# sinamalakouti/CDDMSL

Measured on AMD Instinct MI355X. Metric: images/sec (train step) VOC+Clipart RN50-C4, higher is better.
Workload: dtype bf16

## Files before the change

cddmsl_amd/csrc/conv_fwd256.hip:

```cpp
#include "gemm_common.h"
#include <type_traits>

namespace {

__device__ __forceinline__ unsigned pack4_e4m3(float a, float b, float c, float d) {
  a = __builtin_amdgcn_fmed3f(a, -448.f, 448.f); b = __builtin_amdgcn_fmed3f(b, -448.f, 448.f);
  c = __builtin_amdgcn_fmed3f(c, -448.f, 448.f); d = __builtin_amdgcn_fmed3f(d, -448.f, 448.f);
  int w = __builtin_amdgcn_cvt_pk_fp8_f32(a, b, 0, false);
  w = __builtin_amdgcn_cvt_pk_fp8_f32(c, d, w, true);
  return (unsigned)w;
}

struct fp8e4 { unsigned char v; };
template <> struct Mma<fp8e4> {
  static constexpr int ES = 2;
  __device__ static __forceinline__ void step2(f32x16& acc, const u32x4& a0, const u32x4& a1, const u32x4& b0, const u32x4& b1) {
    const i32x8 a = {(int)a0[0], (int)a0[1], (int)a0[2], (int)a0[3], (int)a1[0], (int)a1[1], (int)a1[2], (int)a1[3]};
    const i32x8 b = {(int)b0[0], (int)b0[1], (int)b0[2], (int)b0[3], (int)b1[0], (int)b1[1], (int)b1[2], (int)b1[3]};
    acc = __builtin_amdgcn_mfma_scale_f32_32x32x64_f8f6f4(a, b, acc, 0, 0, 0, 0x7f7f7f7f, 0, 0x7f7f7f7f);
  }
};
template <typename T> struct MmaQuad {
  __device__ static __forceinline__ void run(f32x16& c0, f32x16& c1, const u32x4 (*fa)[4], const u32x4* fb) {
#pragma unroll
    for (int ks = 0; ks < 4; ++ks) {
      Mma<T>::step(c0, fa[0][ks], fb[ks]);
      Mma<T>::step(c1, fa[1][ks], fb[ks]);
    }
  }
};
template <> struct MmaQuad<fp8e4> {
  __device__ static __forceinline__ void run(f32x16& c0, f32x16& c1, const u32x4 (*fa)[4], const u32x4* fb) {
#pragma unroll
    for (int s = 0; s < 2; ++s) {
      Mma<fp8e4>::step2(c0, fa[0][2 * s], fa[0][2 * s + 1], fb[2 * s], fb[2 * s + 1]);
      Mma<fp8e4>::step2(c1, fa[1][2 * s], fa[1][2 * s + 1], fb[2 * s], fb[2 * s + 1]);
    }
  }
};

__device__ __forceinline__ void blds16(__amdgpu_buffer_rsrc_t r, unsigned voff, unsigned soff, void* l) {
  __builtin_amdgcn_raw_ptr_buffer_load_lds(r, (__attribute__((address_space(3))) void*)l, 16, (int)voff, (int)soff, 0, 0);
}

template <typename T, bool RPOOL, int EPI, bool PRE = false>
__device__ __forceinline__ void tile_epilogue(const ConvArgs& p, f32x16 (&acc)[4][2], float* ep, int wr, int wc, int lane, int m0, int n0,
                                              const u32x4 (*pre)[4] = nullptr, const f32x4* sb = nullptr) {
  constexpr int ES = Mma<T>::ES;
  const int r32 = lane & 31, hh = lane >> 5;
  const int cg = lane & 7, rr = lane >> 3;
  const int n = n0 + wc * 64 + cg * 8;
  float sc[8], bi[8];
#pragma unroll
  for (int j = 0; j < 8; ++j) {
    if (sb) { sc[j] = sb[j >> 2][j & 3]; bi[j] = sb[2 + (j >> 2)][j & 3]; }
    else { sc[j] = p.scale ? p.scale[n + j] : 1.f; bi[j] = p.bias ? p.bias[n + j] : 0.f; }
  }
  const bool has_res = EPI < 0 ? p.residual != nullptr : (EPI & 1) != 0;
  const bool has_msk = EPI < 0 ? p.relu_mask != nullptr : (EPI & 2) != 0;
  const bool f32out = EPI < 0 && (ES == 4 || p.out_f32 != 0);
  const int eso = f32out ? 4 : 2;
  const float relu_floor = p.relu ? 0.f : -__builtin_inff();
  const long rows = p.M - m0;
  auto mk = [&](const char* base, long ld, int es) {
    long bytes = rows * ld * es;
    if (bytes > 0x7fffffffL) bytes = 0x7fffffffL;
    return __builtin_amdgcn_make_buffer_rsrc((void*)(base + (long)m0 * ld * es), 0, base ? (int)bytes : 0, 0x00020000);
  };
  const bool rf32 = EPI < 0 && ES == 2 && p.res_f32;
  const int esr = rf32 ? 4 : ES;
  const __amdgpu_buffer_rsrc_t ry = mk(p.y, p.ldy, eso), rmsk = mk(p.relu_mask, p.ldm, ES);
  const __amdgpu_buffer_rsrc_t rres = RPOOL ? __builtin_amdgcn_make_buffer_rsrc((void*)p.residual, 0, 0x7fffffff, 0x00020000)
                                            : mk(p.residual, p.ldr, esr);
  auto pooled_off = [&](int m) -> unsigned {
    const unsigned tq = fdiv((unsigned)m, p.dWo), ox = m - tq * p.Wo;
    const unsigned img = fdiv(tq, p.dHo), oy = tq - img * p.Ho;
    const unsigned hp = p.Ho >> 1, wp = p.Wo >> 1;
    const bool in = m < p.M && (oy >> 1) < hp && (ox >> 1) < wp;
    return in ? (unsigned)((((img * hp + (oy >> 1)) * wp + (ox >> 1)) * (unsigned)p.ldr + (unsigned)n) * ES) : 0x80000000u;
  };
  const unsigned vy = (unsigned)(((wr * 128 + rr) * p.ldy + n) * eso);
  const unsigned vr = (unsigned)(((wr * 128 + rr) * p.ldr + n) * esr), vm = (unsigned)(((wr * 128 + rr) * p.ldm + n) * ES);
  const bool emit8 = EPI < 0 && ES == 2 && p.y8 != nullptr;
  const __amdgpu_buffer_rsrc_t ry8 = mk(p.y8, p.ldy, 1);
  const unsigned vy8 = (unsigned)((wr * 128 + rr) * p.ldy + n);
  const float q8s = emit8 && p.q8 ? p.q8[0] : 1.f;
  unsigned am8 = 0u;
  constexpr int DEPTH = ES == 2 ? 2 : 1;
  char* wbase[8];
#pragma unroll
  for (int c = 0; c < 8; ++c)
    wbase[c] = (char*)ep + (hh * 4 * 64 + ((((r32 >> 3) ^ (hh << 2)) ^ c) << 3) + (r32 & 7)) * 4;
  u32x4 rresb[DEPTH][4][ES / 2], rmskb[DEPTH][4][ES / 2];
  auto fetch = [&](int a, u32x4 (*rres_)[ES / 2], u32x4 (*rmsk_)[ES / 2]) {
#pragma unroll
    for (int i = 0; i < 4; ++i)
#pragma unroll
      for (int q = 0; q < ES / 2; ++q) {
        if (RPOOL) rres_[i][q] = __builtin_amdgcn_raw_buffer_load_b128(rres, pooled_off(m0 + wr * 128 + a * 32 + rr + 8 * i), q * 16, 0);
        else if (has_res && !rf32) rres_[i][q] = __builtin_amdgcn_raw_buffer_load_b128(rres, vr, (a * 32 + 8 * i) * p.ldr * ES + q * 16, CDDMSL_LOAD_AUX);
        if (has_msk) rmsk_[i][q] = __builtin_amdgcn_raw_buffer_load_b128(rmsk, vm, (a * 32 + 8 * i) * p.ldm * ES + q * 16, CDDMSL_LOAD_AUX);
      }
  };
  if (PRE && DEPTH == 2) {
#pragma unroll
    for (int d = 0; d < 2; ++d)
#pragma unroll
      for (int i = 0; i < 4; ++i) {
        if (EPI & 1) {
          rresb[d % DEPTH][i][0] = pre[d][i];
          if (EPI & 2) rmskb[d % DEPTH][i][0] = __builtin_amdgcn_raw_buffer_load_b128(rmsk, vm, (d * 32 + 8 * i) * p.ldm * ES, CDDMSL_LOAD_AUX);
        } else rmskb[d % DEPTH][i][0] = pre[d][i];
      }
  } else if (DEPTH == 2 && !rf32) { fetch(0, rresb[0], rmskb[0]); fetch(1, rresb[DEPTH - 1], rmskb[DEPTH - 1]); }
  auto put = [&](auto A) {
    constexpr int a = decltype(A)::value;
#pragma unroll
    for (int b = 0; b < 2; ++b)
#pragma unroll
      for (int g = 0; g < 16; ++g)
        *(float*)(wbase[(b << 2) ^ (g & 3)] + ((g & 3) + 8 * (g >> 2)) * 256 + (a & 1) * 8192) = acc[a][b][g];
  };
  auto pass = [&](auto A) {
    constexpr int a = decltype(A)::value;
    if (DEPTH == 1) fetch(a, rresb[0], rmskb[0]);
    if (rf32) {
#pragma unroll
      for (int f = 0; f < 8; ++f)
        rresb[(f >> 2) % DEPTH][f & 3][0] = __builtin_amdgcn_raw_buffer_load_b128(rres, vr, (a * 32 + 8 * (f >> 1)) * p.ldr * 4 + (f & 1) * 16, 0);
    }
    u32x4 (*rres_)[ES / 2] = rresb[a % DEPTH];
    u32x4 (*rmsk_)[ES / 2] = rmskb[a % DEPTH];
    asm volatile("s_waitcnt lgkmcnt(0)" ::: "memory");
    f32x4 val[4][2];
#pragma unroll
    for (int i = 0; i < 4; ++i) {
      const int row = rr + 8 * i;
      const f32x4* src = (const f32x4*)(ep + (a & 1) * 2048 + row * 64 + ((cg ^ (row & 7)) << 3));
      val[i][0] = src[0]; val[i][1] = src[1];
    }
    asm volatile("" ::: "memory");
    if constexpr (a + 1 < 4) put(std::integral_constant<int, a + 1>{});
    asm volatile("" ::: "memory");
#pragma unroll
    for (int i = 0; i < 4; ++i) {
      const f32x4 v0 = val[i][0], v1 = val[i][1];
      float v[8] = {v0[0], v0[1], v0[2], v0[3], v1[0], v1[1], v1[2], v1[3]};
#pragma unroll
      for (int j = 0; j < 8; ++j) v[j] = affine<T>(v[j], sc[j], bi[j]);
      if (rf32) {
#pragma unroll
        for (int j = 0; j < 4; ++j) {
          v[j] += __builtin_bit_cast(f32x4, rresb[((2 * i) >> 2) % DEPTH][(2 * i) & 3][0])[j];
          v[4 + j] += __builtin_bit_cast(f32x4, rresb[((2 * i + 1) >> 2) % DEPTH][(2 * i + 1) & 3][0])[j];
        }
      } else if (RPOOL) {
        if (ES == 2) {
#pragma unroll
          for (int j = 0; j < 4; ++j) { v[2 * j] += 0.25f * bf2f(rres_[i][0][j] & 0xffff); v[2 * j + 1] += 0.25f * bf2f(rres_[i][0][j] >> 16); }
        } else {
#pragma unroll
          for (int j = 0; j < 4; ++j) {
            v[j] += 0.25f * __builtin_bit_cast(f32x4, rres_[i][0])[j]; v[4 + j] += 0.25f * __builtin_bit_cast(f32x4, rres_[i][ES / 2 - 1])[j];
          }
        }
      } else if (has_res) {
        if (ES == 2) {
#pragma unroll
          for (int j = 0; j < 4; ++j) { v[2 * j] += bf2f(rres_[i][0][j] & 0xffff); v[2 * j + 1] += bf2f(rres_[i][0][j] >> 16); }
        } else {
#pragma unroll
          for (int j = 0; j < 4; ++j) {
            v[j] += __builtin_bit_cast(f32x4, rres_[i][0])[j]; v[4 + j] += __builtin_bit_cast(f32x4, rres_[i][ES / 2 - 1])[j];
          }
        }
      }
#pragma unroll
      for (int j = 0; j < 8; ++j) asm("v_max_f32 %0, %1, %2" : "=v"(v[j]) : "v"(v[j]), "s"(relu_floor));
      if (has_msk) {
        float mv[8];
        if (ES == 2) {
#pragma unroll
          for (int j = 0; j < 4; ++j) { mv[2 * j] = bf2f(rmsk_[i][0][j] & 0xffff); mv[2 * j + 1] = bf2f(rmsk_[i][0][j] >> 16); }
        } else {
#pragma unroll
          for (int j = 0; j < 4; ++j) {
            mv[j] = __builtin_bit_cast(f32x4, rmsk_[i][0])[j]; mv[4 + j] = __builtin_bit_cast(f32x4, rmsk_[i][ES / 2 - 1])[j];
          }
        }
#pragma unroll
        for (int j = 0; j < 8; ++j) if (!(mv[j] > 0.f)) v[j] = 0.f;
      }
      const unsigned so = (unsigned)((a * 32 + 8 * i) * p.ldy * eso);
      if (emit8) {
#pragma unroll
        for (int j = 0; j < 8; ++j) am8 = absmax_bits(am8, v[j]);
        const u32x2 o8 = {pack4_e4m3(v[0] * q8s, v[1] * q8s, v[2] * q8s, v[3] * q8s), pack4_e4m3(v[4] * q8s, v[5] * q8s, v[6] * q8s, v[7] * q8s)};
        __builtin_amdgcn_raw_buffer_store_b64(o8, ry8, vy8, (unsigned)((a * 32 + 8 * i) * p.ldy), CDDMSL_STORE_AUX);
        asm volatile("s_nop 4" ::: "memory");
        asm volatile("" :: "v"(o8));
      }
      if (f32out) {
        const u32x4 o0 = {__builtin_bit_cast(unsigned, v[0]), __builtin_bit_cast(unsigned, v[1]), __builtin_bit_cast(unsigned, v[2]), __builtin_bit_cast(unsigned, v[3])};
        const u32x4 o1 = {__builtin_bit_cast(unsigned, v[4]), __builtin_bit_cast(unsigned, v[5]), __builtin_bit_cast(unsigned, v[6]), __builtin_bit_cast(unsigned, v[7])};
        __builtin_amdgcn_raw_buffer_store_b128(o0, ry, vy, so, CDDMSL_STORE_AUX);
        __builtin_amdgcn_raw_buffer_store_b128(o1, ry, vy, so + 16, CDDMSL_STORE_AUX);
        asm volatile("s_nop 4" ::: "memory");
        asm volatile("" :: "v"(o0), "v"(o1));
      } else {
        const u32x4 o = {pack2bf(v[0], v[1]), pack2bf(v[2], v[3]), pack2bf(v[4], v[5]), pack2bf(v[6], v[7])};
        if (p.nt_out) __builtin_amdgcn_raw_buffer_store_b128(o, ry, vy, so, CDDMSL_STORE_AUX);
        else __builtin_amdgcn_raw_buffer_store_b128(o, ry, vy, so, 0);
        asm volatile("s_nop 4" ::: "memory");
        asm volatile("" :: "v"(o));
      }
    }
    if (DEPTH == 2 && a + 2 < 4 && !rf32) fetch(a + 2, rresb[a % DEPTH], rmskb[a % DEPTH]);
  };
  put(std::integral_constant<int, 0>{});
  pass(std::integral_constant<int, 0>{});
  pass(std::integral_constant<int, 1>{});
  pass(std::integral_constant<int, 2>{});
  pass(std::integral_constant<int, 3>{});
  if (emit8 && p.amax8) {
    am8 = wave_max_u(am8);
    if (lane == 0) atomicMax(p.amax8 + (blockIdx.x & 63), am8);
  }
}

template <typename T, bool TAPS, bool RPOOL = false, int EPI = -1, bool PERSIST = false, bool SPLITK = false>
__global__ __launch_bounds__(512) void k_conv_fwd256(ConvArgs p) {
  __shared__ __attribute__((aligned(16))) u32x4 lds[2 * 2 * 2 * 128 * KCH];
  const int t_in = threadIdx.x;
  p.x += (long)blockIdx.y * p.bx; p.w += (long)blockIdx.y * p.bw; p.y += (long)blockIdx.y * p.by;
  const int ntn = p.Cout >> 8;
  const int ntiles = PERSIST ? (p.tile_limit ? p.tile_limit : ntn * ((p.M + 255) >> 8)) : 0;
  int lbid = PERSIST ? (int)((blockIdx.x & 7) * (gridDim.x >> 3) + (blockIdx.x >> 3))
           : SPLITK ? p.tile0 + (int)(blockIdx.x / (unsigned)p.ksplits) : xcd_remap(blockIdx.x, gridDim.x);
  const int kt0 = SPLITK ? (int)(blockIdx.x % (unsigned)p.ksplits) * p.kper : 0;
  if (PERSIST && lbid >= ntiles) return;
  for (;;) {
  int t = t_in;
  if (PERSIST) asm volatile("" : "+v"(t));
  const int lane = t & 63;
#ifdef CDDMSL_TILE_STAMPS
  const unsigned long long ts_entry = __builtin_amdgcn_s_memrealtime();
#endif
  const int wvu = __builtin_amdgcn_readfirstlane(t >> 6);
  const int wr = wvu >> 2, wc = wvu & 3;
  const int tile_n = lbid % ntn, tile_m = lbid / ntn;
  const int m0 = tile_m * 256, n0 = tile_n * 256;
  const int cl = (t & 7) ^ ((t >> 4) & 7);
  const int nkt = SPLITK ? min(p.kper, (p.Kc >> 3) - kt0) : (p.Kc >> 3);
  const int tpt = p.cpp >> 3;

  auto rowoff = [&](int m, int& iy0, int& ix0) {
    const unsigned tq = fdiv((unsigned)m, p.dWo), ox = m - tq * p.Wo;
    const unsigned img = fdiv(tq, p.dHo), oy = tq - img * p.Ho;
    iy0 = (int)oy * p.stride - p.pad; ix0 = (int)ox * p.stride - p.pad;
    return (((long)img * p.Hi + iy0) * p.Wi + ix0) * p.xrs * 16;
  };
  int iyb, ixb;
  const long base_a = rowoff(m0, iyb, ixb);
  const __amdgpu_buffer_rsrc_t ra_rsrc = __builtin_amdgcn_make_buffer_rsrc((void*)(p.x + base_a), 0, 0x7fffffff, 0x00020000);
  const __amdgpu_buffer_rsrc_t rb_rsrc = __builtin_amdgcn_make_buffer_rsrc((void*)(p.w + (long)n0 * p.wrs * 16), 0, 0x7fffffff, 0x00020000);
  unsigned va[2][2], vinv[2][2], vb[2][2];
  int iy0[2][2], ix0[2][2];
#pragma unroll
  for (int h = 0; h < 2; ++h)
#pragma unroll
    for (int i = 0; i < 2; ++i) {
      const int m = m0 + i * 128 + h * 64 + (t >> 3);
      const bool vm = m < p.M;
      const long ro = rowoff(vm ? m : m0, iy0[h][i], ix0[h][i]);
      va[h][i] = (unsigned)(ro - base_a) + cl * 16;
      if (!vm) { iy0[h][i] = -(1 << 20); if (!TAPS) va[h][i] |= 0x80000000u; }
      vinv[h][i] = 0;
      vb[h][i] = (unsigned)(((2 * i + (t >> 8)) * 64 + h * 32 + ((t >> 3) & 31)) * p.wrs + cl) * 16;
    }
  if (TAPS) {
    unsigned xm[2][2] = {{0, 0}, {0, 0}};
    for (int kx = 0; kx < p.KW; ++kx)
#pragma unroll
      for (int h = 0; h < 2; ++h)
#pragma unroll
        for (int i = 0; i < 2; ++i) xm[h][i] |= ((unsigned)(ix0[h][i] + kx) >= (unsigned)p.Wi ? 1u : 0u) << kx;
    const unsigned full = (1u << p.KW) - 1u;
    for (int ky = 0; ky < p.KH; ++ky)
#pragma unroll
      for (int h = 0; h < 2; ++h)
#pragma unroll
        for (int i = 0; i < 2; ++i) vinv[h][i] |= ((unsigned)(iy0[h][i] + ky) >= (unsigned)p.Hi ? full : xm[h][i]) << (ky * p.KW);
  }
  const int step_col = (p.xrs - (p.cpp - KCH)) * 16;
  const int step_row = ((p.Wi - (p.KW - 1)) * p.xrs - (p.cpp - KCH)) * 16;
  int left[2] = {tpt, tpt}, tap[2] = {0, 0}, kxs[2] = {0, 0};
  unsigned soa[2] = {0, 0}, sob[2] = {0, 0};
  if (SPLITK) {
    const int tap0 = TAPS ? kt0 / tpt : 0, within = TAPS ? kt0 - tap0 * tpt : kt0;
    const int ky0 = TAPS ? tap0 / p.KW : 0, kx0 = tap0 - ky0 * p.KW;
#pragma unroll
    for (int h = 0; h < 2; ++h) {
      left[h] = tpt - (TAPS ? within : 0); tap[h] = tap0; kxs[h] = kx0;
      soa[h] = (unsigned)((ky0 * p.Wi + kx0) * p.xrs * 16 + within * KCH * 16);
      sob[h] = (unsigned)(kt0 * KCH * 16);
    }
  }

  char* const L = (char*)lds;
  auto stageA = [&](auto H, int buf) {
    constexpr int h = decltype(H)::value;
    char* dst = L + (buf << 16) + (h << 14) + wvu * 1024;
#pragma unroll
    for (int i = 0; i < 2; ++i) {
      unsigned v = va[h][i];
      if (TAPS) v |= __builtin_amdgcn_ubfe(vinv[h][i], (unsigned)tap[h], 1u) << 31;
      blds16(ra_rsrc, v, soa[h], dst + i * 8192);
    }
    if (TAPS) {
      int step = KCH * 16;
      if (--left[h] == 0) {
        left[h] = tpt; ++tap[h];
        if (++kxs[h] == p.KW) { kxs[h] = 0; step = step_row; } else step = step_col;
      }
      soa[h] += step;
    } else soa[h] += KCH * 16;
  };
  auto stageB = [&](auto J, int buf) {
    constexpr int j = decltype(J)::value;
    char* dst = L + (buf << 16) + (1 << 15) + (j << 14) + wvu * 1024;
#pragma unroll
    for (int i = 0; i < 2; ++i) blds16(rb_rsrc, vb[j][i], sob[j], dst + i * 8192);
    sob[j] += KCH * 16;
  };
  using I0 = std::integral_constant<int, 0>;
  using I1 = std::integral_constant<int, 1>;

  f32x16 acc[4][2];
#pragma unroll
  for (int a = 0; a < 4; ++a)
#pragma unroll
    for (int b = 0; b < 2; ++b)
#pragma unroll
      for (int r = 0; r < 16; ++r) acc[a][b][r] = 0.f;

  const int r32 = lane & 31, hh = lane >> 5, sw = (r32 >> 1) & 7;
  unsigned ada[4], adb[4];
#pragma unroll
  for (int ks = 0; ks < 4; ++ks) {
    ada[ks] = (unsigned)(((wr * 64 + r32) * KCH + ((2 * ks + hh) ^ sw)) * 16);
    adb[ks] = (unsigned)(((wc * 32 + r32) * KCH + ((2 * ks + hh) ^ sw)) * 16 + (1 << 15));
  }
  u32x4 fa0[2][4], fa1[2][4], fb0[4], fb1[4];
  auto readA = [&](auto I, u32x4 (*fa)[4]) {
    constexpr int i = decltype(I)::value;
#pragma unroll
    for (int rt = 0; rt < 2; ++rt)
#pragma unroll
      for (int ks = 0; ks < 4; ++ks) fa[rt][ks] = *(const u32x4*)(L + ada[ks] + ((i << 14) + rt * 32 * KCH * 16));
  };
  auto readB = [&](auto J, u32x4* fb) {
    constexpr int j = decltype(J)::value;
#pragma unroll
    for (int ks = 0; ks < 4; ++ks) fb[ks] = *(const u32x4*)(L + adb[ks] + (j << 14));
  };
  auto flipA = [&]() {
#pragma unroll
    for (int ks = 0; ks < 4; ++ks) ada[ks] ^= 1u << 16;
  };
  auto flipB = [&]() {
#pragma unroll
    for (int ks = 0; ks < 4; ++ks) adb[ks] ^= 1u << 16;
  };
#define CDDMSL_MMA_QUAD(I, J, FA, FB) MmaQuad<T>::run(acc[2 * (I)][J], acc[2 * (I) + 1][J], FA, FB)
#define CDDMSL_PHASE_SYNC_IN()                                                      \
  __builtin_amdgcn_sched_barrier(0);                                                \
  __builtin_amdgcn_s_barrier();                                                     \
  asm volatile("s_waitcnt lgkmcnt(0)" ::: "memory");                                \
  __builtin_amdgcn_sched_barrier(0);                                                \
  __builtin_amdgcn_s_setprio(1);
#define CDDMSL_PHASE_SYNC_OUT(I, J)                                                 \
  asm volatile("" : "+v"(acc[2 * (I)][J]), "+v"(acc[2 * (I) + 1][J]));    \
  __builtin_amdgcn_s_setprio(0);                                                    \
  __builtin_amdgcn_sched_barrier(0);                                                \
  __builtin_amdgcn_s_barrier();                                                     \
  __builtin_amdgcn_sched_barrier(0);

  stageA(I0{}, 0); stageA(I1{}, 0); stageB(I0{}, 0); stageB(I1{}, 0);
  if (nkt > 1) {
    stageA(I0{}, 1); stageB(I0{}, 1); stageB(I1{}, 1);
    asm volatile("s_waitcnt vmcnt(6)" ::: "memory");
  } else {
    asm volatile("s_waitcnt vmcnt(0)" ::: "memory");
  }
  __builtin_amdgcn_s_barrier();
  readA(I0{}, fa0);
  if (wr == 1) __builtin_amdgcn_s_barrier();
  __builtin_amdgcn_sched_barrier(0);
#ifdef CDDMSL_TILE_STAMPS
  const unsigned long long ts_loop = __builtin_amdgcn_s_memrealtime();
#endif

  constexpr bool PREF = EPI > 0 && !RPOOL && Mma<T>::ES == 2 && !SPLITK;
  u32x4 pre[2][4];
  f32x4 sb[4];
  auto ktile = [&](int kt, auto LAST) {
    constexpr bool last = decltype(LAST)::value;
    const int d = kt & 1;
    const bool more1 = !last, more2 = !last && kt + 2 < nkt;
    readB(I0{}, fb0);
    if (more1) stageA(I1{}, d ^ 1);
    CDDMSL_PHASE_SYNC_IN();
    CDDMSL_MMA_QUAD(0, 0, fa0, fb0);
    CDDMSL_PHASE_SYNC_OUT(0, 0);
    readB(I1{}, fb1);
    flipB();
    if (more2) stageA(I0{}, d);
    CDDMSL_PHASE_SYNC_IN();
    CDDMSL_MMA_QUAD(0, 1, fa0, fb1);
    CDDMSL_PHASE_SYNC_OUT(0, 1);
    readA(I1{}, fa1);
    flipA();
    if (more2) {
      stageB(I0{}, d);
      asm volatile("s_waitcnt vmcnt(4)" ::: "memory");
    } else if (more1) {
      asm volatile("s_waitcnt vmcnt(0)" ::: "memory");
    } else if (PREF) {
      const bool is_res = (EPI & 1) != 0;
      const char* base = is_res ? p.residual : p.relu_mask;
      const int ld = is_res ? p.ldr : p.ldm;
      long bytes = ((long)p.M - m0) * ld * 2;
      if (bytes > 0x7fffffffL) bytes = 0x7fffffffL;
      const __amdgpu_buffer_rsrc_t rs = __builtin_amdgcn_make_buffer_rsrc((void*)(base + (long)m0 * ld * 2), 0, (int)bytes, 0x00020000);
      const unsigned vo = (unsigned)(((wr * 128 + (lane >> 3)) * ld + n0 + wc * 64 + (lane & 7) * 8) * 2);
#pragma unroll
      for (int a = 0; a < 2; ++a)
#pragma unroll
        for (int i = 0; i < 4; ++i) pre[a][i] = __builtin_amdgcn_raw_buffer_load_b128(rs, vo, (a * 32 + 8 * i) * ld * 2, 0);
    }
    CDDMSL_PHASE_SYNC_IN();
    CDDMSL_MMA_QUAD(1, 1, fa1, fb1);
    CDDMSL_PHASE_SYNC_OUT(1, 1);
    if (more1) readA(I0{}, fa0);
    if (more2) stageB(I1{}, d);
    if (last && !SPLITK) {
      const int n = n0 + wc * 64 + (lane & 7) * 8;
      const f32x4 one = {1.f, 1.f, 1.f, 1.f}, zero = {0.f, 0.f, 0.f, 0.f};
      sb[0] = p.scale ? *(const f32x4*)(p.scale + n) : one; sb[1] = p.scale ? *(const f32x4*)(p.scale + n + 4) : one;
      sb[2] = p.bias ? *(const f32x4*)(p.bias + n) : zero; sb[3] = p.bias ? *(const f32x4*)(p.bias + n + 4) : zero;
    }
    CDDMSL_PHASE_SYNC_IN();
    CDDMSL_MMA_QUAD(1, 0, fa1, fb0);
    CDDMSL_PHASE_SYNC_OUT(1, 0);
  };
  for (int kt = 0; kt + 1 < nkt; ++kt) ktile(kt, std::false_type{});
  ktile(nkt - 1, std::true_type{});
  if (wr == 0) __builtin_amdgcn_s_barrier();
#ifdef CDDMSL_TILE_STAMPS
  const unsigned long long ts_epi = __builtin_amdgcn_s_memrealtime();
#endif
#undef CDDMSL_MMA_QUAD
#undef CDDMSL_PHASE_SYNC_IN
#undef CDDMSL_PHASE_SYNC_OUT

  if (SPLITK) {
    store_frags((f32x4*)p.partial + (long)blockIdx.x * (8 * 32 * 64) + (wvu * 32) * 64 + lane, acc);
    return;
  }
  tile_epilogue<T, RPOOL, EPI, PREF>(p, acc, (float*)lds + wvu * 4096, wr, wc, lane, m0, n0, pre, sb);
#ifdef CDDMSL_TILE_STAMPS
  if (p.tstamps && lane == 0) {
    if (!PERSIST) asm volatile("s_waitcnt vmcnt(0)" ::: "memory");
    unsigned long long* o = p.tstamps + ((long)(PERSIST ? lbid : (int)blockIdx.x) * 8 + wvu) * 4;
    o[0] = ts_entry; o[1] = ts_loop; o[2] = ts_epi; o[3] = __builtin_amdgcn_s_memrealtime();
  }
#endif
  if (!PERSIST) break;
  lbid += gridDim.x;
  if (lbid >= ntiles) break;
  __builtin_amdgcn_s_barrier();
  }
}

template <typename T, bool TAPS, int EPI>
__global__ __launch_bounds__(256, 2) void k_conv_fwd2(ConvArgs p) {
  constexpr int SA = 256 * 64, SB = 128 * 64, SS = SA + SB, STAGES = 3;
  __shared__ __attribute__((aligned(16))) u32x4 lds[STAGES * SS / 16];
  const int t = threadIdx.x, lane = t & 63;
#ifdef CDDMSL_TILE_STAMPS
  const unsigned long long ts_entry = __builtin_amdgcn_s_memrealtime();
#endif
  p.x += (long)blockIdx.y * p.bx; p.w += (long)blockIdx.y * p.bw; p.y += (long)blockIdx.y * p.by;
  const int wvu = __builtin_amdgcn_readfirstlane(t >> 6);
  const int wr = wvu >> 1, wc = wvu & 1;
  const int ntn = p.Cout >> 7;
  const int lbid = xcd_remap(blockIdx.x, gridDim.x);
  const int tile_n = lbid % ntn, tile_m = lbid / ntn;
  const int m0 = tile_m * 256, n0 = tile_n * 128;
  const int cl = (t & 3) ^ ((t >> 3) & 3);
  const int nkt = p.Kc >> 2;
  const int tpt = p.cpp >> 2;

  auto rowoff = [&](int m, int& iy0, int& ix0) {
    const unsigned tq = fdiv((unsigned)m, p.dWo), ox = m - tq * p.Wo;
    const unsigned img = fdiv(tq, p.dHo), oy = tq - img * p.Ho;
    iy0 = (int)oy * p.stride - p.pad; ix0 = (int)ox * p.stride - p.pad;
    return (((long)img * p.Hi + iy0) * p.Wi + ix0) * p.xrs * 16;
  };
  int iyb, ixb;
  const long base_a = rowoff(m0, iyb, ixb);
  const __amdgpu_buffer_rsrc_t ra_rsrc = __builtin_amdgcn_make_buffer_rsrc((void*)(p.x + base_a), 0, 0x7fffffff, 0x00020000);
  const __amdgpu_buffer_rsrc_t rb_rsrc = __builtin_amdgcn_make_buffer_rsrc((void*)(p.w + (long)n0 * p.wrs * 16), 0, 0x7fffffff, 0x00020000);
  unsigned va[4], vinv[4], vb[2];
  int iy0[4], ix0[4];
#pragma unroll
  for (int i = 0; i < 4; ++i) {
    const int m = m0 + (t >> 2) + 64 * i;
    const bool vm = m < p.M;
    const long ro = rowoff(vm ? m : m0, iy0[i], ix0[i]);
    va[i] = (unsigned)(ro - base_a) + cl * 16;
    if (!vm) { iy0[i] = -(1 << 20); if (!TAPS) va[i] |= 0x80000000u; }
    vinv[i] = 0;
  }
#pragma unroll
  for (int i = 0; i < 2; ++i) vb[i] = (unsigned)((((t >> 2) + 64 * i) * p.wrs + cl) * 16);
  if (TAPS) {
    unsigned xm[4] = {0, 0, 0, 0};
    for (int kx = 0; kx < p.KW; ++kx)
#pragma unroll
      for (int i = 0; i < 4; ++i) xm[i] |= ((unsigned)(ix0[i] + kx) >= (unsigned)p.Wi ? 1u : 0u) << kx;
    const unsigned full = (1u << p.KW) - 1u;
    for (int ky = 0; ky < p.KH; ++ky)
#pragma unroll
      for (int i = 0; i < 4; ++i) vinv[i] |= ((unsigned)(iy0[i] + ky) >= (unsigned)p.Hi ? full : xm[i]) << (ky * p.KW);
  }
  const int step_col = (p.xrs - (p.cpp - 4)) * 16;
  const int step_row = ((p.Wi - (p.KW - 1)) * p.xrs - (p.cpp - 4)) * 16;
  int left = tpt, tap = 0, kxs = 0;
  unsigned soa = 0, sob = 0;

  char* const L = (char*)lds;
  auto stage = [&](int st) {
    char* dst = L + st * SS + wvu * 1024;
#pragma unroll
    for (int i = 0; i < 4; ++i) {
      unsigned v = va[i];
      if (TAPS) v |= __builtin_amdgcn_ubfe(vinv[i], (unsigned)tap, 1u) << 31;
      blds16(ra_rsrc, v, soa, dst + i * 4096);
    }
#pragma unroll
    for (int i = 0; i < 2; ++i) blds16(rb_rsrc, vb[i], sob, dst + SA + i * 4096);
    sob += 64;
    if (TAPS) {
      int step = 64;
      if (--left == 0) {
        left = tpt; ++tap;
        if (++kxs == p.KW) { kxs = 0; step = step_row; } else step = step_col;
      }
      soa += step;
    } else soa += 64;
  };

  f32x16 acc[4][2];
#pragma unroll
  for (int a = 0; a < 4; ++a)
#pragma unroll
    for (int b = 0; b < 2; ++b)
#pragma unroll
      for (int r = 0; r < 16; ++r) acc[a][b][r] = 0.f;

  const int r32 = lane & 31, hh = lane >> 5, sw = (r32 >> 1) & 3;
  unsigned ada[2], adb[2];
#pragma unroll
  for (int ks = 0; ks < 2; ++ks) {
    ada[ks] = (unsigned)(((wr * 128 + r32) * 4 + ((2 * ks + hh) ^ sw)) * 16);
    adb[ks] = (unsigned)(SA + ((wc * 64 + r32) * 4 + ((2 * ks + hh) ^ sw)) * 16);
  }
  u32x4 fa[2][4][2], fb[2][2][2];
  auto readf = [&](auto SET, int st) {
    constexpr int set = decltype(SET)::value;
    const char* base = L + st * SS;
#pragma unroll
    for (int rt = 0; rt < 4; ++rt)
#pragma unroll
      for (int ks = 0; ks < 2; ++ks) fa[set][rt][ks] = *(const u32x4*)(base + ada[ks] + rt * 32 * 64);
#pragma unroll
    for (int ct = 0; ct < 2; ++ct)
#pragma unroll
      for (int ks = 0; ks < 2; ++ks) fb[set][ct][ks] = *(const u32x4*)(base + adb[ks] + ct * 32 * 64);
  };
  using S0 = std::integral_constant<int, 0>;
  using S1 = std::integral_constant<int, 1>;

  stage(0);
  if (nkt > 1) stage(1);
  if (nkt > 2) stage(2);
  if (nkt > 2) asm volatile("s_waitcnt vmcnt(12)" ::: "memory");
  else if (nkt > 1) asm volatile("s_waitcnt vmcnt(6)" ::: "memory");
  else asm volatile("s_waitcnt vmcnt(0)" ::: "memory");
  __builtin_amdgcn_s_barrier();
  readf(S0{}, 0);
#ifdef CDDMSL_TILE_STAMPS
  const unsigned long long ts_loop = __builtin_amdgcn_s_memrealtime();
#endif
  int st_next = 1, st_free = 0;

  auto ktile = [&](int kt, auto SET) {
    constexpr int set = decltype(SET)::value;
    if (kt + 2 < nkt) asm volatile("s_waitcnt vmcnt(6)" ::: "memory");
    else asm volatile("s_waitcnt vmcnt(0)" ::: "memory");
    __builtin_amdgcn_s_waitcnt(0xc07f);
    __builtin_amdgcn_sched_barrier(0);
    __builtin_amdgcn_s_barrier();
    __builtin_amdgcn_sched_barrier(0);
    if (kt + 1 < nkt) readf(std::integral_constant<int, set ^ 1>{}, st_next);
    if (kt + 3 < nkt) stage(st_free);
    st_next = st_next == STAGES - 1 ? 0 : st_next + 1;
    st_free = st_free == STAGES - 1 ? 0 : st_free + 1;
    __builtin_amdgcn_sched_barrier(0);
    __builtin_amdgcn_s_setprio(1);
#pragma unroll
    for (int ks = 0; ks < 2; ++ks)
#pragma unroll
      for (int rt = 0; rt < 4; ++rt)
#pragma unroll
        for (int ct = 0; ct < 2; ++ct) Mma<T>::step(acc[rt][ct], fa[set][rt][ks], fb[set][ct][ks]);
    __builtin_amdgcn_s_setprio(0);
    __builtin_amdgcn_sched_barrier(0);
  };
  for (int kt = 0; kt < nkt; kt += 2) {
    ktile(kt, S0{});
    if (kt + 1 < nkt) ktile(kt + 1, S1{});
  }
#ifdef CDDMSL_TILE_STAMPS
  asm volatile("" : "+v"(acc[3][1]));
  const unsigned long long ts_epi = __builtin_amdgcn_s_memrealtime();
#endif
  tile_epilogue<T, false, EPI>(p, acc, (float*)lds + wvu * 4096, wr, wc, lane, m0, n0);
#ifdef CDDMSL_TILE_STAMPS
  if (p.tstamps && lane == 0) {
    asm volatile("s_waitcnt vmcnt(0)" ::: "memory");
    unsigned long long* o = p.tstamps + ((long)blockIdx.x * 4 + wvu) * 4;
    o[0] = ts_entry; o[1] = ts_loop; o[2] = ts_epi; o[3] = __builtin_amdgcn_s_memrealtime();
  }
#endif
}

__global__ __launch_bounds__(256) void k_conv_split_reduce(ConvArgs p) {
  const int tile_rel = blockIdx.x >> 6, q = (blockIdx.x & 63) * 256 + threadIdx.x;
  const f32x4* src = (const f32x4*)p.partial + (long)tile_rel * p.ksplits * 16384 + q;
  f32x4 sum = src[0];
  for (int s = 1; s < p.ksplits; ++s) sum += src[(long)s * 16384];
  const int wvu = q >> 11, j = (q >> 6) & 31, lane = q & 63, r32 = lane & 31, hh = lane >> 5;
  const int a = j >> 3, b = (j >> 2) & 1, g4 = j & 3, wr = wvu >> 2, wc = wvu & 3;
  const int ntn = p.Cout >> 8, lbid = p.tile0 + tile_rel;
  const int tile_n = lbid % ntn, tile_m = lbid / ntn;
  const int n = tile_n * 256 + wc * 64 + b * 32 + r32;
  const int mrow = tile_m * 256 + wr * 128 + a * 32 + 8 * g4 + 4 * hh;
  const float sc = p.scale ? p.scale[n] : 1.f, bi = p.bias ? p.bias[n] : 0.f;
#pragma unroll
  for (int e = 0; e < 4; ++e) {
    const long m = mrow + e;
    if (m >= p.M) break;
    float v = __builtin_fmaf(sum[e], sc, bi);
    if (p.residual) v += bf2f(*(const unsigned short*)(p.residual + (m * p.ldr + n) * 2));
    if (p.relu) v = fmaxf(v, 0.f);
    if (p.relu_mask && !(bf2f(*(const unsigned short*)(p.relu_mask + (m * p.ldm + n) * 2)) > 0.f)) v = 0.f;
    *(unsigned short*)(p.y + (m * p.ldy + n) * 2) = f2bf(v);
  }
}

static int persistent_blocks() { return env_int("CDDMSL_PERSIST", 1) ? persistent_blocks_raw() : 0; }

static int epi_of(const ConvArgs& a) { return (a.out_f32 || a.res_f32 || a.y8) ? -1 : (a.residual ? 1 : 0) | (a.relu_mask ? 2 : 0); }
template <typename F> void with_epi(int epi, F&& launch) {
  switch (epi) {
    case 0: launch(std::integral_constant<int, 0>()); break;
    case 1: launch(std::integral_constant<int, 1>()); break;
    case 2: launch(std::integral_constant<int, 2>()); break;
    default: launch(std::integral_constant<int, 3>()); break;
  }
}

template <typename T, bool TAPS> void launch_fwd2(const ConvArgs& a, dim3 grid, hipStream_t st) {
  const int epi = epi_of(a);
  if constexpr (sizeof(T) == 2) {
    if (epi >= 0) {
      with_epi(epi, [&](auto e) { hipLaunchKernelGGL((k_conv_fwd2<T, TAPS, decltype(e)::value>), grid, dim3(256), 0, st, a); });
      return;
    }
  }
  hipLaunchKernelGGL((k_conv_fwd2<T, TAPS, -1>), grid, dim3(256), 0, st, a);
}

struct TailSplit { int rem, splits, kper; };
constexpr int TAIL_FRAC_DEFAULT = 8;
static TailSplit plan_tail_split(int tiles, int ncu, int nktot, long ws_bytes) {
  const int rem = ncu > 0 ? tiles % ncu : 0;
  long frac = env_int("CDDMSL_TAIL_FRAC", TAIL_FRAC_DEFAULT);
  if (frac <= 0) frac = 8;
  if (env_int("CDDMSL_TAIL_SPLIT", 1) == 0 || tiles <= ncu || rem <= 0 || rem * frac > ncu || nktot < 16) return {};
  long S = ncu / rem;
  if (S > nktot / 2) S = nktot / 2;
  const long maxs = env_int("CDDMSL_TAIL_MAXS", S);
  if (S > maxs) S = maxs;
  const int kper = (int)((nktot + S - 1) / S);
  S = (nktot + kper - 1) / kper;
  if (S < 2 || rem * S * 65536 * 4 > ws_bytes) return {};
  return {rem, (int)S, kper};
}

template <typename T, bool TAPS> void launch256_main(const ConvArgs& a, dim3 grid, hipStream_t st, int epi) {
  if constexpr (std::is_same<T, __bf16>::value && !TAPS) {
    const int nb = persistent_blocks();
    if (nb > 0 && grid.y == 1 && (int)grid.x > nb && (a.Kc >> 3) <= env_int("CDDMSL_PERSIST_MAXKT", 8)) {
      with_epi(epi, [&](auto e) { hipLaunchKernelGGL((k_conv_fwd256<T, false, false, decltype(e)::value, true>), dim3(nb), dim3(512), 0, st, a); });
      return;
    }
  }
  with_epi(epi, [&](auto e) { hipLaunchKernelGGL((k_conv_fwd256<T, TAPS, false, decltype(e)::value>), grid, dim3(512), 0, st, a); });
}

template <typename T, bool TAPS> void launch256(const ConvArgs& a, dim3 grid, hipStream_t st, void* ws, long ws_bytes) {
  const int epi = epi_of(a);
  if (sizeof(T) == 4 || epi < 0) { hipLaunchKernelGGL((k_conv_fwd256<T, TAPS, false, -1>), grid, dim3(512), 0, st, a); return; }
  if constexpr (sizeof(T) != 4) {
    if constexpr (std::is_same<T, __bf16>::value) {
      const int tiles = (int)grid.x;
      const TailSplit ts = grid.y == 1 ? plan_tail_split(tiles, persistent_blocks_raw(), a.Kc >> 3, ws ? ws_bytes : 0) : TailSplit{};
      if (ts.splits) {
        ConvArgs m = a, t = a;
        m.tile_limit = tiles - ts.rem;
        launch256_main<T, TAPS>(m, dim3((unsigned)(tiles - ts.rem), 1), st, epi);
        t.partial = (float*)ws; t.tile0 = tiles - ts.rem; t.ksplits = ts.splits; t.kper = ts.kper;
        hipLaunchKernelGGL((k_conv_fwd256<T, TAPS, false, -1, false, true>), dim3((unsigned)(ts.rem * ts.splits)), dim3(512), 0, st, t);
        hipLaunchKernelGGL(k_conv_split_reduce, dim3((unsigned)(ts.rem * 64)), dim3(256), 0, st, t);
        return;
      }
    }
    launch256_main<T, TAPS>(a, grid, st, epi);
  }
}

template <typename T> void launch_tile256(const ConvArgs& a, const Plan& p, hipStream_t st, void* ws, long ws_bytes) {
  const dim3 grid(p.gx, p.gy);
  const bool taps = !(a.KH == 1 && a.KW == 1 && a.pad == 0);
  if constexpr (std::is_same<T, fp8e4>::value) {
    if (taps) launch256<T, true>(a, grid, st, ws, ws_bytes);
    else launch256<T, false>(a, grid, st, ws, ws_bytes);
  } else if (p.kernel == 11) {
    if (taps) launch_fwd2<T, true>(a, grid, st);
    else launch_fwd2<T, false>(a, grid, st);
  } else {
    if (a.res_pool) hipLaunchKernelGGL((k_conv_fwd256<T, false, true>), grid, dim3(512), 0, st, a);
    else if (taps) launch256<T, true>(a, grid, st, ws, ws_bytes);
    else launch256<T, false>(a, grid, st, ws, ws_bytes);
  }
}

}

void launch_fwd_tile256(const ConvArgs& a, const Plan& p, Operand op, hipStream_t st, void* ws, long ws_bytes) {
  if (op == OP_BF16) launch_tile256<__bf16>(a, p, st, ws, ws_bytes);
  else if (op == OP_F32) launch_tile256<float>(a, p, st, ws, ws_bytes);
  else launch_tile256<fp8e4>(a, p, st, ws, ws_bytes);
}
```

cddmsl_amd/csrc/gemm_common.h:

```cpp
#pragma once
#include "common.h"
#include <cstdlib>

namespace {

constexpr int BM = 128, BN = 128, KCH = 8;

struct FastDiv {
  unsigned mul, shr, d;
};
static inline FastDiv make_fastdiv(unsigned d) {
  FastDiv f;
  f.d = d;
  unsigned s = 0;
  while ((1ull << s) < d) ++s;
  f.shr = s;
  f.mul = (unsigned)(((1ull << 32) * ((1ull << s) - d)) / d + 1);
  return f;
}
__device__ __forceinline__ unsigned fdiv(unsigned n, const FastDiv& f) { return (__umulhi(n, f.mul) + n) >> f.shr; }

template <typename T> __device__ __forceinline__ float affine(float v, float sc, float bi) {
  return sizeof(T) <= 2 ? __builtin_fmaf(v, sc, bi) : v * sc + bi;
}

#ifndef CDDMSL_STORE_AUX
#define CDDMSL_STORE_AUX 2
#endif
#ifndef CDDMSL_LOAD_AUX
#define CDDMSL_LOAD_AUX 0
#endif

struct ConvArgs {
  const char* x;
  const char* w;
  char* y;
  const float* scale;
  const float* bias;
  const char* residual;
  const char* relu_mask;
  int Nimg, Hi, Wi, Cin, Ho, Wo, Cout, KH, KW, stride, pad;
  int ldy, ldr, ldm;
  int relu, out_f32, pool;
  int res_f32;
  int res_pool;
  int M, Kc, cpp;
  FastDiv dWo, dHo, dcpp, dKW;
  int xrs, wrs;
  long bx, bw, by;
  char* y8 = nullptr;
  const float* q8 = nullptr;
  unsigned* amax8 = nullptr;
  float* partial = nullptr;
  int tile0 = 0, ksplits = 1, kper = 0, tile_limit = 0;
  int pool_out = 0;
  FastDiv dWp = {}, dHp = {};
  int nt_out = 1;
#ifdef CDDMSL_TILE_STAMPS
  unsigned long long* tstamps = nullptr;
#endif
};

template <typename T> struct Mma;
template <> struct Mma<__bf16> {
  static constexpr int ES = 2;
  __device__ static __forceinline__ void step(f32x16& acc, const u32x4& a, const u32x4& b) {
    acc = __builtin_amdgcn_mfma_f32_32x32x16_bf16(__builtin_bit_cast(bf16x8, a), __builtin_bit_cast(bf16x8, b), acc, 0, 0, 0);
  }
  __device__ static __forceinline__ float load(const char* p) { return bf2f(*(const unsigned short*)p); }
  __device__ static __forceinline__ void store(char* p, float v) { *(unsigned short*)p = f2bf(v); }
};
template <> struct Mma<float> {
  static constexpr int ES = 4;
  __device__ static __forceinline__ void step(f32x16& acc, const u32x4& a, const u32x4& b) {
    const f32x4 fa = __builtin_bit_cast(f32x4, a), fb = __builtin_bit_cast(f32x4, b);
    acc = __builtin_amdgcn_mfma_f32_32x32x2f32(fa[0], fb[0], acc, 0, 0, 0);
    acc = __builtin_amdgcn_mfma_f32_32x32x2f32(fa[1], fb[1], acc, 0, 0, 0);
    acc = __builtin_amdgcn_mfma_f32_32x32x2f32(fa[2], fb[2], acc, 0, 0, 0);
    acc = __builtin_amdgcn_mfma_f32_32x32x2f32(fa[3], fb[3], acc, 0, 0, 0);
  }
  __device__ static __forceinline__ float load(const char* p) { return *(const float*)p; }
  __device__ static __forceinline__ void store(char* p, float v) { *(float*)p = v; }
};
typedef __attribute__((ext_vector_type(8))) int i32x8;

__device__ __forceinline__ int xcd_remap(int bid, int nblk) {
  const int q = nblk >> 3, rem = nblk & 7, x = bid & 7, j = bid >> 3;
  return (x < rem ? x * (q + 1) : rem * (q + 1) + (x - rem) * q) + j;
}

template <typename T> __device__ __forceinline__ u32x4 avg4(const u32x4& a, const u32x4& b, const u32x4& c, const u32x4& d);
template <> __device__ __forceinline__ u32x4 avg4<float>(const u32x4& a, const u32x4& b, const u32x4& c, const u32x4& d) {
  const f32x4 fa = __builtin_bit_cast(f32x4, a), fb = __builtin_bit_cast(f32x4, b);
  const f32x4 fc = __builtin_bit_cast(f32x4, c), fd = __builtin_bit_cast(f32x4, d);
  f32x4 r = ((fa + fb) + (fc + fd)) * 0.25f;
  return __builtin_bit_cast(u32x4, r);
}
template <> __device__ __forceinline__ u32x4 avg4<__bf16>(const u32x4& a, const u32x4& b, const u32x4& c, const u32x4& d) {
  u32x4 r;
#pragma unroll
  for (int j = 0; j < 4; ++j) {
    float lo = (bf2f(a[j] & 0xffff) + bf2f(b[j] & 0xffff)) + (bf2f(c[j] & 0xffff) + bf2f(d[j] & 0xffff));
    float hi = (bf2f(a[j] >> 16) + bf2f(b[j] >> 16)) + (bf2f(c[j] >> 16) + bf2f(d[j] >> 16));
    r[j] = pack2bf(lo * 0.25f, hi * 0.25f);
  }
  return r;
}

__device__ __attribute__((aligned(16))) unsigned int g_zero_page[4] = {0u, 0u, 0u, 0u};

__device__ __forceinline__ void glds16(const void* g, void* l) {
  __builtin_amdgcn_global_load_lds((const __attribute__((address_space(1))) void*)g,
                                   (__attribute__((address_space(3))) void*)l, 16, 0, 0);
}

struct WgradArgs {
  const char* x;
  const char* dy;
  float* dw;
  const float* scale;
  int Nimg, Hi, Wi, Cin, Ho, Wo, Cout, KH, KW, stride, pad, ldd, pool;
  int M, Kc, cpp, K, ncc;
  int mtiles_per_split;
  FastDiv dWo, dHo;
  int xrs;
  int ldo;
  int direct;
  long bx, bd, bo;
  const float* g0 = nullptr;
  const unsigned long long* mbits = nullptr;
  float* gpos = nullptr;
  float* ws = nullptr;
#ifdef CDDMSL_TILE_STAMPS
  unsigned long long* tstamps = nullptr;
#endif
};

constexpr int WM = 64;
constexpr int WROW = 16 + 4;

__device__ __forceinline__ int fsw(int row) { return ((row & 3) << 2) | ((row >> 2) & 3); }

__device__ __forceinline__ void store_frags(f32x4* dst, const f32x16 (&acc)[4][2]) {
#pragma unroll
  for (int a = 0; a < 4; ++a)
#pragma unroll
    for (int b = 0; b < 2; ++b)
#pragma unroll
      for (int g4 = 0; g4 < 4; ++g4) {
        const f32x4 v = {acc[a][b][4 * g4], acc[a][b][4 * g4 + 1], acc[a][b][4 * g4 + 2], acc[a][b][4 * g4 + 3]};
        dst[((a * 2 + b) * 4 + g4) * 64] = v;
      }
}

static long env_int(const char* name, long dflt, bool* set = nullptr) {
  const char* e = getenv(name);
  if (set) *set = e != nullptr;
  return e ? atol(e) : dflt;
}

enum Operand { OP_BF16 = 0, OP_F32 = 1, OP_FP8 = 2 };
static int elem_size(Operand op) { return op == OP_BF16 ? 2 : op == OP_F32 ? 4 : 1; }

struct Plan {
  int kernel;
  unsigned gx, gy;
  int splits;
  int mtiles_per_split;
  int bpb;
};

static int persistent_blocks_raw() {
  static int ncu = -1;
  if (ncu < 0) {
    int dev = 0, n = 0;
    if (hipGetDevice(&dev) != hipSuccess || hipDeviceGetAttribute(&n, hipDeviceAttributeMultiprocessorCount, dev) != hipSuccess) n = 0;
    ncu = (n / 8) * 8;
  }
  return ncu;
}

}

extern "C" {
__attribute__((visibility("hidden"))) void launch_fwd_tile128(const ConvArgs& a, const Plan& p, Operand op, hipStream_t st);
__attribute__((visibility("hidden"))) void launch_fwd_tile256(const ConvArgs& a, const Plan& p, Operand op, hipStream_t st, void* ws, long ws_bytes);
__attribute__((visibility("hidden"))) void launch_wgrad(WgradArgs& a, const Plan& p, Operand op, hipStream_t st, void* ws, long ws_bytes);
__attribute__((visibility("hidden"))) void launch_gemm_tn(const WgradArgs& p, Operand op, const Plan& pl, int batch, int mode, hipStream_t st);
__attribute__((visibility("hidden"))) void launch_attnpool_dx(const WgradArgs& p, unsigned gx, unsigned gy, int nbatch, int bpb, hipStream_t st);
__attribute__((visibility("hidden"))) bool record_kernel(int id);
}
```

cddmsl_amd/csrc/gemm_conv.hip:

```cpp
#include "gemm_common.h"

namespace {

template <typename T>
__device__ __forceinline__ void weight_prep_body(const float* w, const float* scale, char* wf, char* wd, int Cout, int KH, int KW, int Cin,
                                                 long first, long stride) {
  __shared__ float tile[32][33];
  const int taps = KH * KW, nit = (Cin + 31) / 32, nct = (Cout + 31) / 32;
  const long ntiles = (long)nct * taps * nit;
  const int tx = threadIdx.x & 31, ty = threadIdx.x >> 5;
  constexpr int ES = Mma<T>::ES;
  for (long tl = first; tl < ntiles; tl += stride) {
    const int it = (int)(tl % nit); const long q = tl / nit;
    const int tap = (int)(q % taps), ct = (int)(q / taps);
    const int ky = tap / KW, kx = tap % KW;
    __syncthreads();
#pragma unroll
    for (int r = 0; r < 4; ++r) {
      const int co = ct * 32 + ty + 8 * r, ci = it * 32 + tx;
      float v = 0.f;
      if (co < Cout && ci < Cin) {
        const long i = ((long)co * taps + tap) * Cin + ci;
        v = w[i];
        if (wf) Mma<T>::store(wf + i * ES, v);
        if (scale) v *= scale[co];
      }
      tile[ty + 8 * r][tx] = v;
    }
    __syncthreads();
    if (wd) {
#pragma unroll
      for (int r = 0; r < 4; ++r) {
        const int ci = it * 32 + ty + 8 * r, co = ct * 32 + tx;
        if (ci < Cin && co < Cout) {
          const long j = (((long)ci * KH + (KH - 1 - ky)) * KW + (KW - 1 - kx)) * Cout + co;
          Mma<T>::store(wd + j * ES, tile[tx][ty + 8 * r]);
        }
      }
    }
  }
}
template <typename T>
__global__ __launch_bounds__(256) void k_weight_prep(const float* w, const float* scale, char* wf, char* wd, int Cout, int KH, int KW, int Cin) {
  weight_prep_body<T>(w, scale, wf, wd, Cout, KH, KW, Cin, (long)blockIdx.x, (long)gridDim.x);
}
template <typename T>
__global__ __launch_bounds__(256) void k_weight_prep_multi(const long long* table) {
  const long long* e = table + 8 * (long)blockIdx.y;
  weight_prep_body<T>((const float*)e[0], (const float*)e[1], (char*)e[2], (char*)e[3], (int)e[4], (int)e[5], (int)e[6], (int)e[7],
                      (long)blockIdx.x, (long)gridDim.x);
}

static thread_local int g_last_kernel = 0;
static thread_local int g_plan_only = 0;


static bool gemm256_legal(const ConvArgs& a) {
  const bool vec_ok = (a.ldy % 8 == 0) && (!a.residual || a.ldr % 8 == 0) && (!a.relu_mask || a.ldm % 8 == 0);
  if (a.pool || (a.cpp & 7) || (a.Cout & 255) || !vec_ok || a.KH * a.KW > 31) return false;
  if (2 * a.pad > a.KH - 1 || 2 * a.pad > a.KW - 1) return false;
  return true;
}

static bool use_gemm256(const ConvArgs& a, int batch) {
  const long mode = env_int("CDDMSL_GEMM256", 1);
  if (mode == 0) return false;
  if (!gemm256_legal(a)) return false;
  if (mode == 2) return true;
  const long tiles = (long)((a.M + 255) / 256) * (a.Cout / 256) * batch;
  return tiles >= 160;
}

static bool fwd2_legal(const ConvArgs& a) {
  const bool vec_ok = (a.ldy % 8 == 0) && (!a.residual || a.ldr % 8 == 0) && (!a.relu_mask || a.ldm % 8 == 0);
  if (a.pool || a.res_pool || (a.cpp & 3) || (a.Cout & 127) || !vec_ok || a.KH * a.KW > 31) return false;
  if (2 * a.pad > a.KH - 1 || 2 * a.pad > a.KW - 1) return false;
  return true;
}
static bool use_fwd2(const ConvArgs& a, int batch) {
  const long mode = env_int("CDDMSL_FWD2", 1);
  if (mode == 0 || !fwd2_legal(a)) return false;
  if (mode == 2) return true;
  if (use_gemm256(a, batch) || batch != 1) return false;
  return (long)(a.Cout / 128) * ((a.M + 255) / 256) >= env_int("CDDMSL_FWD2_MIN", 256);
}

static Plan plan_fwd(const ConvArgs& a, Operand op, int batch) {
  const long tiles256 = (long)(a.Cout / 256) * ((a.M + 255) / 256);
  if (op == OP_FP8) {
    if (!gemm256_legal(a) || tiles256 > 0x7fffffffL) return {};
    return {10, (unsigned)tiles256, 1};
  }
  if (a.y8 && !use_gemm256(a, batch)) return {};
  const long tiles128 = (long)((a.Cout + BN - 1) / BN) * ((a.M + BM - 1) / BM);
  if (tiles128 > 0x7fffffffL) return {};
  const bool packed = batch == 1 && a.xrs == a.cpp && a.wrs == a.Kc;
  if (!a.pool && a.KH == 3 && a.KW == 3 && a.pad == 1 && (a.cpp == 1 || a.cpp == 4 || (a.cpp == 8 && a.Cout == 64)) &&
      (a.Cout == 32 || a.Cout == 64) && !a.residual && !a.out_f32 && packed) {
    return {8, a.cpp > 1 ? 256u * 2 : 256u * 8, 1};
  }
  if (op == OP_BF16 && !a.pool && a.KH == 1 && a.KW == 1 && a.pad == 0 && a.stride == 1 && a.Cout == 64 && (a.cpp == 8 || a.cpp == 32) &&
      !a.residual && !a.out_f32 && !a.y8 && packed && a.ldy == 64 && env_int("CDDMSL_SMALL_1X1", 1) != 0) return {8, 512, 1};
  if (use_fwd2(a, batch)) return {11, (unsigned)((long)(a.Cout / 128) * ((a.M + 255) / 256)), (unsigned)batch};
  if (use_gemm256(a, batch)) return {3, (unsigned)tiles256, (unsigned)batch};
  if (a.pool) return {2, (unsigned)tiles128, 1};
  return {1, (unsigned)tiles128, (unsigned)batch};
}

static void* g_ws = nullptr;
static long g_ws_bytes = 0;

static int run_fwd(const ConvArgs& a, Operand op, const Plan& p, void* stream) {
  if (p.kernel == 0) return CDDMSL_ERR_ARG;
  g_last_kernel = p.kernel;
  if (g_plan_only) return CDDMSL_OK;
  if (p.kernel == 3 || p.kernel == 10 || p.kernel == 11) launch_fwd_tile256(a, p, op, (hipStream_t)stream, g_ws, g_ws_bytes);
  else launch_fwd_tile128(a, p, op, (hipStream_t)stream);
  return launch_status();
}

}

#ifdef CDDMSL_TILE_STAMPS
static unsigned long long* g_tile_stamps = nullptr;
extern "C" void cddmsl_debug_tile_stamps(unsigned long long* p) { g_tile_stamps = p; }
#endif
extern "C" int cddmsl_last_kernel(void) { return g_last_kernel; }
extern "C" int cddmsl_plan_only(int on) { const int was = g_plan_only; g_plan_only = on; return was; }
bool record_kernel(int id) { g_last_kernel = id; return g_plan_only != 0; }

static int nt_out_for(long out_bytes) {
  static const long nt_min_mb = env_int("CDDMSL_NT_MIN_MB", 128);
  return out_bytes > (nt_min_mb << 20) ? 1 : 0;
}

static int fill_conv(ConvArgs& a, Operand op, const void* x, const void* w, void* y, const float* scale, const float* bias,
                     const void* residual, const void* relu_mask, int Nimg, int Hi, int Wi, int Cin, int Cout, int KH, int KW,
                     int stride, int pad, int pool, int ldy, int ldr, int ldm, int relu, int out_f32, void* y8, const float* q8,
                     float* amax8) {
  const int es = elem_size(op);
  if (Nimg < 0 || Hi <= 0 || Wi <= 0 || Cin <= 0 || Cout <= 0 || KH <= 0 || KW <= 0 || stride <= 0) return CDDMSL_ERR_ARG;
  if ((Cin * es) % 16 != 0) return CDDMSL_ERR_ARG;
  if (pool && (KH != 1 || KW != 1 || pad != 0 || stride != 1)) return CDDMSL_ERR_ARG;
  a.x = (const char*)x; a.w = (const char*)w; a.y = (char*)y; a.scale = scale; a.bias = bias;
  a.residual = (const char*)residual; a.relu_mask = (const char*)relu_mask;
  a.Nimg = Nimg; a.Hi = Hi; a.Wi = Wi; a.Cin = Cin; a.Cout = Cout; a.KH = KH; a.KW = KW; a.stride = stride; a.pad = pad;
  if (pool) { a.Ho = Hi / 2; a.Wo = Wi / 2; }
  else { a.Ho = (Hi + 2 * pad - KH) / stride + 1; a.Wo = (Wi + 2 * pad - KW) / stride + 1; }
  if (a.Ho <= 0 || a.Wo <= 0) return CDDMSL_ERR_ARG;
  if ((out_f32 & 2) && (!(out_f32 & 1) || !residual || relu_mask || pool)) return CDDMSL_ERR_ARG;
  a.ldy = ldy; a.ldr = ldr; a.ldm = ldm; a.relu = relu; a.out_f32 = out_f32 & 1; a.pool = pool;
  a.res_f32 = (op == OP_BF16 && (out_f32 & 2)) ? 1 : 0;
  a.res_pool = (out_f32 & 4) ? 1 : 0;
  if (a.res_pool && (!residual || (out_f32 & 2) || pool || KH != 1 || KW != 1 || pad != 0 || (long)Nimg * (a.Ho / 2) * (a.Wo / 2) * ldr * es >= (1L << 31) ||
                     (Cout & 7) || (ldy & 7) || (ldr & 7) || (relu_mask && (ldm & 7)))) return CDDMSL_ERR_ARG;
  if (a.res_f32 && ((Cout & 7) || (ldy & 7) || (ldr & 7))) return CDDMSL_ERR_ARG;
  long M = (long)Nimg * a.Ho * a.Wo;
  if (M > 0x7fffff00L) return CDDMSL_ERR_ARG;
  a.M = (int)M; a.cpp = Cin * es / 16; a.Kc = KH * KW * a.cpp;
  a.dWo = make_fastdiv((unsigned)a.Wo); a.dHo = make_fastdiv((unsigned)a.Ho);
  a.dcpp = make_fastdiv((unsigned)a.cpp); a.dKW = make_fastdiv((unsigned)KW);
  a.xrs = a.cpp; a.wrs = a.Kc; a.bx = a.bw = a.by = 0;
#ifdef CDDMSL_TILE_STAMPS
  a.tstamps = g_tile_stamps;
#endif
  if (a.M == 0) return CDDMSL_OK;
  a.nt_out = nt_out_for((long)a.M * Cout * 2);
  if (y8) {
    if (op == OP_F32 || (out_f32 & 1) || ldy != Cout) return CDDMSL_ERR_ARG;
    a.y8 = (char*)y8; a.q8 = q8; a.amax8 = (unsigned*)amax8;
  }
  return CDDMSL_OK;
}

static int conv_fwd_any(Operand op, const void* x, const void* w, void* y, const float* scale, const float* bias,
                        const void* residual, const void* relu_mask, int Nimg, int Hi, int Wi, int Cin,
                        int Cout, int KH, int KW, int stride, int pad, int pool, int ldy, int ldr, int ldm,
                        int relu, int out_f32, void* y8, const float* q8, float* amax8, void* stream) {
  ConvArgs a;
  const int st = fill_conv(a, op, x, w, y, scale, bias, residual, relu_mask, Nimg, Hi, Wi, Cin, Cout, KH, KW, stride, pad, pool, ldy, ldr, ldm,
                           relu, out_f32, y8, q8, amax8);
  if (st != CDDMSL_OK || a.M == 0) return st;
  return run_fwd(a, op, plan_fwd(a, op, 1), stream);
}

extern "C" int cddmsl_conv_fwd(const void* x, const void* w, void* y, const float* scale, const float* bias,
                               const void* residual, const void* relu_mask, int Nimg, int Hi, int Wi, int Cin,
                               int Cout, int KH, int KW, int stride, int pad, int pool, int ldy, int ldr, int ldm,
                               int relu, int out_f32, int dtype, void* stream) {
  if (dtype != 0 && dtype != 1) return CDDMSL_ERR_ARG;
  return conv_fwd_any((Operand)dtype, x, w, y, scale, bias, residual, relu_mask, Nimg, Hi, Wi, Cin, Cout, KH, KW, stride, pad, pool, ldy, ldr, ldm,
                      relu, out_f32, nullptr, nullptr, nullptr, stream);
}

extern "C" int cddmsl_conv3x3_pool_fwd(const void* x, const void* w, void* y, const float* scale, const float* bias, const void* relu_mask,
                                       int Nimg, int Hi, int Wi, int Cin, int Cout, int stride, int dtype, void* stream) {
  if (dtype != 0 || Cin != 32 || Cout != 64 || stride != 1 || relu_mask || !scale || !bias || Hi < 2 || Wi < 2) return CDDMSL_ERR_ARG;
  ConvArgs a;
  const int st = fill_conv(a, OP_BF16, x, w, y, scale, bias, nullptr, nullptr, Nimg, Hi, Wi, Cin, Cout, 3, 3, 1, 1, 0, Cout, 0, 0, 1, 0,
                           nullptr, nullptr, nullptr);
  if (st != CDDMSL_OK || a.M == 0) return st;
  if ((long)Nimg * Hi * Wi * Cin * 2 >= 0x7ffff000L || (long)Nimg * (a.Ho / 2) * (a.Wo / 2) * Cout * 2 >= 0x7fffffffL) return CDDMSL_ERR_ARG;
  a.pool_out = 1;
  a.dWp = make_fastdiv((unsigned)(a.Wo / 2)); a.dHp = make_fastdiv((unsigned)(a.Ho / 2));
  const Plan pl = plan_fwd(a, OP_BF16, 1);
  if (pl.kernel != 8) return CDDMSL_ERR_ARG;
  return run_fwd(a, OP_BF16, pl, stream);
}

extern "C" int cddmsl_conv_fwd_q8(const void* x, const void* w, void* y, const float* scale, const float* bias,
                                  const void* residual, const void* relu_mask, int Nimg, int Hi, int Wi, int Cin,
                                  int Cout, int KH, int KW, int stride, int pad, int relu, void* y8, const float* q8, float* amax8,
                                  void* stream) {
  if (!y8) return CDDMSL_ERR_ARG;
  return conv_fwd_any(OP_BF16, x, w, y, scale, bias, residual, relu_mask, Nimg, Hi, Wi, Cin, Cout, KH, KW, stride, pad, 0, Cout, Cout, Cout,
                      relu, 0, y8, q8, amax8, stream);
}

extern "C" int cddmsl_conv_fwd_fp8(const void* x, const void* w, void* y, const float* scale, const float* bias,
                                   const void* residual, const void* relu_mask, int Nimg, int Hi, int Wi, int Cin, int Cout, int KH,
                                   int KW, int pad, int relu, int out_f32, void* y8, const float* q8, float* amax8, void* stream) {
  if (Cin % 128 != 0 || (out_f32 & ~1)) return CDDMSL_ERR_ARG;
  return conv_fwd_any(OP_FP8, x, w, y, scale, bias, residual, relu_mask, Nimg, Hi, Wi, Cin, Cout, KH, KW, 1, pad, 0, Cout, Cout, Cout,
                      relu, out_f32, y8, q8, amax8, stream);
}

static bool wgrad256_ok(const WgradArgs& a, int batch) {
  const long mode = env_int("CDDMSL_GEMM256", 1);
  if (mode == 0) return false;
  if ((a.Cout & 255) || (a.K & 255) || (a.cpp & 7) || (a.ldd & 7)) return false;
  if (mode == 2) return true;
  return (long)(a.Cout / 256) * (a.K / 256) * batch * ((a.M + WM - 1) / WM) >= env_int("CDDMSL_WGRAD256_MIN", 4000);
}
static bool wgrad256_span_ok(int mtiles_per_split, int Wi, long row_bytes) {
  return ((long)mtiles_per_split * WM + WM + 2L * Wi + 2) * row_bytes + (1L << 20) < (1L << 31);
}

static int even_split(int total_mt, long* splits) {
  const int mps = (int)((total_mt + *splits - 1) / *splits);
  *splits = (total_mt + mps - 1) / mps;
  return mps;
}

static long split_512_rounds(long tiles, int total_mt, bool taps) {
  bool forced;
  const long target = env_int("CDDMSL_WGRAD_BLOCKS", taps ? 1024 : 512, &forced);
  const long maxs = (total_mt + 7) / 8;
  long splits = 1;
  const long r0 = (target + 511) / 512;
  double best = -1.0;
  for (long r = r0; r <= r0 + 1; ++r) {
    long c = (512 * r) / tiles;
    if (c < 1) c = 1;
    if (c > maxs) c = maxs;
    long real = c;
    even_split(total_mt, &real);
    const long blocks = tiles * real, rounds = (blocks + 511) / 512;
    const double eff = (double)blocks / (512.0 * rounds);
    if (eff > best + 0.03) { best = eff; splits = c; }
    if (c == maxs) break;
  }
  if (forced) { splits = (target + tiles - 1) / tiles; if (splits > maxs) splits = maxs; }
  return splits < 1 ? 1 : splits;
}

static long split_256_rounds(long tiles, int total_mt) {
  const long maxs = (total_mt + 15) / 16;
  long sp = 1;
  double best = -1.0;
  for (int r = 1; r <= 6; ++r) {
    long c = (256L * r) / tiles;
    if (c < 1) continue;
    if (c > maxs) c = maxs;
    const long blocks = tiles * c, rounds = (blocks + 255) / 256;
    const double eff = (double)blocks / (256.0 * rounds);
    if (eff > best + 0.02) { best = eff; sp = c; }
    if (c == maxs) break;
  }
  return sp;
}

static Plan plan_wgrad(const WgradArgs& a, Operand op, int batch) {
  const int es = elem_size(op), total_mt = (a.M + WM - 1) / WM;
  const long tiles256 = (long)(a.Cout / 256) * (a.K / 256);
  const long row_bytes = (long)a.ldd * es > a.xrs * 16L ? (long)a.ldd * es : a.xrs * 16L;
  if (op == OP_FP8) {
    long sp = split_256_rounds(tiles256, total_mt);
    const int mps = even_split(total_mt, &sp);
    if (!wgrad256_span_ok(mps, a.Wi, row_bytes)) return {};
    return {12, (unsigned)(tiles256 * sp), 1, (int)sp, mps};
  }
  const int cols = 256 / es;
  const long tiles = (long)((a.Cout + cols - 1) / cols) * ((a.K + cols - 1) / cols);
  long splits = split_512_rounds(tiles, total_mt, !(a.KH == 1 && a.KW == 1));
  const int mps = even_split(total_mt, &splits);
  if (tiles * splits > 0x7fffffffL) return {};
  const bool same = !a.pool && a.stride == 1 && a.Ho == a.Hi && a.Wo == a.Wi;
  if (same && op == OP_BF16 && wgrad256_ok(a, batch)) {
    bool forced;
    const long want = env_int("CDDMSL_WGRAD256_BLOCKS", 0, &forced);
    const long maxs = (total_mt + 15) / 16;
    long sp = forced ? (want + tiles256 - 1) / tiles256 : split_256_rounds(tiles256, total_mt);
    if (sp > maxs) sp = maxs;
    if (sp < 1) sp = 1;
    const int mps256 = even_split(total_mt, &sp);
    if (wgrad256_span_ok(mps256, a.Wi, row_bytes)) return {6, (unsigned)(tiles256 * sp), 1, (int)sp, mps256};
  }
  return {same ? 5 : 4, (unsigned)(tiles * splits), 1, (int)splits, mps};
}

extern "C" int cddmsl_set_workspace(void* ptr, long bytes) {
  if (bytes < 0 || (ptr == nullptr && bytes != 0) || ((size_t)ptr & 15)) return CDDMSL_ERR_ARG;
  g_ws = ptr; g_ws_bytes = bytes;
  return CDDMSL_OK;
}

static int run_wgrad(WgradArgs& a, Operand op, const Plan& p, void* stream) {
  if (p.kernel == 0) return CDDMSL_ERR_ARG;
  g_last_kernel = p.kernel;
  if (g_plan_only) return CDDMSL_OK;
  a.mtiles_per_split = p.mtiles_per_split;
  launch_wgrad(a, p, op, (hipStream_t)stream, g_ws, g_ws_bytes);
  return launch_status();
}

static int fill_wgrad(WgradArgs& a, Operand op, const void* x, const void* dy, float* dw, const float* scale, int Nimg, int Hi,
                      int Wi, int Cin, int Cout, int KH, int KW, int stride, int pad, int pool, int ldd) {
  const int es = elem_size(op);
  if (Nimg < 0 || Hi <= 0 || Wi <= 0 || Cin <= 0 || Cout <= 0 || KH <= 0 || KW <= 0 || stride <= 0) return CDDMSL_ERR_ARG;
  if ((Cin * es) % 16 != 0 || (Cout * es) % 16 != 0 || (ldd * es) % 16 != 0) return CDDMSL_ERR_ARG;
  if (pool && (KH != 1 || KW != 1 || pad != 0 || stride != 1)) return CDDMSL_ERR_ARG;
  a.x = (const char*)x; a.dy = (const char*)dy; a.dw = dw; a.scale = scale;
  a.Nimg = Nimg; a.Hi = Hi; a.Wi = Wi; a.Cin = Cin; a.Cout = Cout; a.KH = KH; a.KW = KW; a.stride = stride; a.pad = pad;
  a.ldd = ldd; a.pool = pool;
  if (pool) { a.Ho = Hi / 2; a.Wo = Wi / 2; }
  else { a.Ho = (Hi + 2 * pad - KH) / stride + 1; a.Wo = (Wi + 2 * pad - KW) / stride + 1; }
  if (a.Ho <= 0 || a.Wo <= 0) return CDDMSL_ERR_ARG;
  long M = (long)Nimg * a.Ho * a.Wo;
  if (M > 0x7fffff00L) return CDDMSL_ERR_ARG;
  a.M = (int)M; a.cpp = Cin * es / 16; a.Kc = KH * KW * a.cpp; a.K = KH * KW * Cin; a.ncc = Cout * es / 16;
  a.mtiles_per_split = 0;
  a.dWo = make_fastdiv((unsigned)a.Wo); a.dHo = make_fastdiv((unsigned)a.Ho);
  a.xrs = a.cpp; a.ldo = a.K; a.direct = 0; a.bx = a.bd = a.bo = 0;
#ifdef CDDMSL_TILE_STAMPS
  a.tstamps = g_tile_stamps;
#endif
  return CDDMSL_OK;
}

extern "C" int cddmsl_conv_wgrad(const void* x, const void* dy, float* dw, const float* scale, int Nimg, int Hi,
                                 int Wi, int Cin, int Cout, int KH, int KW, int stride, int pad, int pool, int ldd,
                                 int dtype, void* stream) {
  if (dtype != 0 && dtype != 1) return CDDMSL_ERR_ARG;
  WgradArgs a;
  const int st = fill_wgrad(a, (Operand)dtype, x, dy, dw, scale, Nimg, Hi, Wi, Cin, Cout, KH, KW, stride, pad, pool, ldd);
  if (st != CDDMSL_OK || a.M == 0) return st;
  return run_wgrad(a, (Operand)dtype, plan_wgrad(a, (Operand)dtype, 1), stream);
}

extern "C" int cddmsl_conv_wgrad_fp8_ok(int Cin, int Cout, int KH, int KW, int pad, int ldd) {
  return (Cin % 256 == 0 && Cout % 256 == 0 && KH == KW && (KH & 1) && 2 * pad == KH - 1 && ldd % 16 == 0) ? 1 : 0;
}
extern "C" int cddmsl_conv_wgrad_fp8(const void* x8, const void* dy8, float* dw, const float* scale, int Nimg, int Hi, int Wi, int Cin,
                                     int Cout, int KH, int KW, int pad, int ldd, void* stream) {
  if (!cddmsl_conv_wgrad_fp8_ok(Cin, Cout, KH, KW, pad, ldd) || ldd < Cout) return CDDMSL_ERR_ARG;
  WgradArgs a;
  const int st = fill_wgrad(a, OP_FP8, x8, dy8, dw, scale, Nimg, Hi, Wi, Cin, Cout, KH, KW, 1, pad, 0, ldd);
  if (st != CDDMSL_OK || a.M == 0) return st;
  return run_wgrad(a, OP_FP8, plan_wgrad(a, OP_FP8, 1), stream);
}

extern "C" int cddmsl_gemm_nt_batched(const void* a, const void* w, void* c, const float* bias, int M, int N, int K, int lda,
                                      int ldb, int ldc, int batch, long sa, long sw, long sc, int out_f32, int dtype, void* stream) {
  int es = dtype == 0 ? 2 : 4;
  if (dtype != 0 && dtype != 1) return CDDMSL_ERR_ARG;
  if (M < 0 || N <= 0 || K <= 0 || batch < 0 || batch > 65535) return CDDMSL_ERR_ARG;
  if ((K * es) % 16 || (lda * es) % 16 || (ldb * es) % 16 || (sa * es) % 16 || (sw * es) % 16) return CDDMSL_ERR_ARG;
  if (M == 0 || batch == 0) return CDDMSL_OK;
  const Operand op = (Operand)dtype;
  ConvArgs p;
  const int st = fill_conv(p, op, a, w, c, nullptr, bias, nullptr, nullptr, 1, 1, M, K, N, 1, 1, 1, 0, 0, ldc, 0, 0, 0, out_f32 ? 1 : 0,
                           nullptr, nullptr, nullptr);
  if (st != CDDMSL_OK) return st;
  p.xrs = lda * es / 16; p.wrs = ldb * es / 16;
  p.bx = sa * es; p.bw = sw * es; p.by = sc * (out_f32 ? 4 : es);
  p.nt_out = 1;
  return run_fwd(p, op, plan_fwd(p, op, batch), stream);
}

static unsigned tn_small_grid(long kt, long batch, int* bpb) {
  long b = (kt * batch + 4095) / 4096;
  if (b < 8) b = 8;
  if (b > batch) b = batch;
  *bpb = (int)b;
  return (unsigned)((batch + b - 1) / b);
}

static Plan plan_gemm_tn(const WgradArgs& p, Operand op, int batch, int mode) {
  const int cols = 256 / elem_size(op), M = p.M, N = p.Cout, K = p.K;
  const long tiles = (long)((N + cols - 1) / cols) * ((K + cols - 1) / cols);
  const int total_mt = (M + WM - 1) / WM;
  if (op == OP_BF16 && total_mt == 1 && N <= 64 && batch >= 64 && K % 128 == 0 && N % 8 == 0) {
    Plan p = {9, (unsigned)(K / 128), 0};
    p.gy = tn_small_grid(K / 128, batch, &p.bpb);
    return p;
  }
  if (total_mt <= 4 && batch >= 64) {
    long bpb = (tiles * batch + 4095) / 4096, minb = (8 + total_mt - 1) / total_mt;
    if (bpb < minb) bpb = minb;
    if (bpb > batch) bpb = batch;
    return {7, (unsigned)tiles, (unsigned)((batch + bpb - 1) / bpb), 0, 0, (int)bpb};
  }
  long splits = 1;
  if (mode == 0) {
    const long want = (2048 + tiles * batch - 1) / (tiles * batch), maxs = (total_mt + 7) / 8;
    splits = want < 1 ? 1 : (want > maxs ? maxs : want);
    if (splits < 1) splits = 1;
  }
  const int mps = even_split(total_mt, &splits);
  if (tiles * splits > 0x7fffffffL) return {};
  return {5, (unsigned)(tiles * splits), (unsigned)batch, (int)splits, mps};
}

extern "C" int cddmsl_gemm_tn_batched(const void* a, const void* b, void* out, int M, int N, int K, int lda, int ldb, int ldo,
                                      int batch, long sa, long sb, long so, int mode, int dtype, void* stream) {
  int es = dtype == 0 ? 2 : 4;
  if (dtype != 0 && dtype != 1) return CDDMSL_ERR_ARG;
  if (M <= 0 || N <= 0 || K <= 0 || batch <= 0 || batch > 65535 || mode < 0 || mode > 2) return CDDMSL_ERR_ARG;
  if ((K * es) % 16 || (N * es) % 16 || (lda * es) % 16 || (ldb * es) % 16 || (sa * es) % 16 || (sb * es) % 16) return CDDMSL_ERR_ARG;
  const Operand op = (Operand)dtype;
  WgradArgs p;
  const int fs = fill_wgrad(p, op, b, a, (float*)out, nullptr, 1, 1, M, K, N, 1, 1, 1, 0, 0, lda);
  if (fs != CDDMSL_OK) return fs;
  p.xrs = ldb * es / 16; p.ldo = ldo; p.direct = mode;
  p.bx = sb * es; p.bd = sa * es; p.bo = so * (mode == 2 ? es : 4);
  const Plan pl = plan_gemm_tn(p, op, batch, mode);
  if (pl.kernel == 0) return CDDMSL_ERR_ARG;
  g_last_kernel = pl.kernel;
  if (g_plan_only) return CDDMSL_OK;
  p.mtiles_per_split = pl.mtiles_per_split;
  launch_gemm_tn(p, op, pl, batch, mode, (hipStream_t)stream);
  return launch_status();
}

extern "C" int cddmsl_attnpool_dx(const void* pds, const void* zu, const float* g0, const unsigned long long* mbits, void* dx, float* gpos,
                                  int K, int H2, int P, int TP, int C, int dtype, void* stream) {
  if (dtype != 0 || K < 0 || P != 49 || TP != 56 || H2 <= 0 || H2 > 64 || (H2 & 7) || C <= 0 || (C & 127) || !g0 || !mbits || !dx) return CDDMSL_ERR_ARG;
  if (K == 0) return CDDMSL_OK;
  if (K > 65535 * 8) return CDDMSL_ERR_ARG;
  WgradArgs p;
  const int fs = fill_wgrad(p, OP_BF16, zu, pds, (float*)dx, nullptr, 1, 1, H2, C, TP, 1, 1, 1, 0, 0, TP);
  if (fs != CDDMSL_OK) return fs;
  p.direct = 3;
  p.bx = (long)H2 * C * 2; p.bd = (long)H2 * TP * 2; p.bo = (long)P * C * 2;
  p.g0 = g0; p.mbits = mbits; p.gpos = gpos;
  int bpb;
  const unsigned gy = tn_small_grid(C / 128, K, &bpb);
  launch_attnpool_dx(p, (unsigned)(C / 128), gy, K, bpb, (hipStream_t)stream);
  return launch_status();
}

extern "C" int cddmsl_weight_prep_multi(const long long* table, int count, int dtype, void* stream) {
  if ((dtype != 0 && dtype != 1) || count < 0 || count > 65535) return CDDMSL_ERR_ARG;
  if (count == 0) return CDDMSL_OK;
  if (dtype == 0) hipLaunchKernelGGL(k_weight_prep_multi<__bf16>, dim3(256, (unsigned)count), dim3(256), 0, (hipStream_t)stream, table);
  else hipLaunchKernelGGL(k_weight_prep_multi<float>, dim3(256, (unsigned)count), dim3(256), 0, (hipStream_t)stream, table);
  return launch_status();
}

extern "C" int cddmsl_weight_prep(const float* w, const float* scale, void* w_fwd, void* w_dgrad, int Cout, int KH,
                                  int KW, int Cin, int dtype, void* stream) {
  if (dtype != 0 && dtype != 1) return CDDMSL_ERR_ARG;
  long n = (long)Cout * KH * KW * Cin;
  if (n <= 0) return n == 0 ? CDDMSL_OK : CDDMSL_ERR_ARG;
  const long tiles = (long)((Cout + 31) / 32) * KH * KW * ((Cin + 31) / 32);
  unsigned grid = (unsigned)(tiles > 4096 ? 4096 : tiles);
  if (dtype == 0) hipLaunchKernelGGL(k_weight_prep<__bf16>, dim3(grid), dim3(256), 0, (hipStream_t)stream, w, scale, (char*)w_fwd, (char*)w_dgrad, Cout, KH, KW, Cin);
  else hipLaunchKernelGGL(k_weight_prep<float>, dim3(grid), dim3(256), 0, (hipStream_t)stream, w, scale, (char*)w_fwd, (char*)w_dgrad, Cout, KH, KW, Cin);
  return launch_status();
}
```

cddmsl_amd/hip.py:

```python
import ctypes
import math
import os
from ctypes import c_float, c_int, c_long, c_void_p

import torch

from ._lib import check, lib, ptr, require_cuda, stream_ptr

DT = {torch.bfloat16: 0, torch.float32: 1}

_sigs_done = False


def _L():
    global _sigs_done
    L = lib()
    if not _sigs_done:
        vp, ci, cf = c_void_p, c_int, c_float
        L.cddmsl_last_kernel.argtypes = []
        L.cddmsl_plan_only.argtypes = [ci]
        L.cddmsl_conv_fwd.argtypes = [vp] * 7 + [ci] * 16 + [vp]
        L.cddmsl_bottleneck64_ok.argtypes = [ci] * 4
        L.cddmsl_bottleneck64_fwd.argtypes = [vp] * 17 + [ci] * 4 + [vp]
        L.cddmsl_conv_wgrad.argtypes = [vp] * 4 + [ci] * 12 + [vp]
        L.cddmsl_set_workspace.argtypes = [vp, c_long]
        L.cddmsl_weight_prep.argtypes = [vp] * 4 + [ci] * 5 + [vp]
        L.cddmsl_weight_prep_multi.argtypes = [vp, ci, ci, vp]
        L.cddmsl_preprocess.argtypes = [vp, vp] + [ci] * 6 + [vp, vp, ci, ci, vp]
        L.cddmsl_maxpool3s2_fwd.argtypes = [vp, vp] + [ci] * 5 + [vp]
        L.cddmsl_upsample_zero2.argtypes = [vp] * 4 + [ci] * 5 + [vp]
        L.cddmsl_meanpool_fwd.argtypes = [vp, vp, c_long, ci, ci, ci, vp]
        L.cddmsl_meanpool_bwd.argtypes = [vp, vp, c_long, ci, ci, ci, vp]
        L.cddmsl_preprocess224.argtypes = [vp, vp] + [ci] * 11 + [vp, vp, ci, vp]
        L.cddmsl_preprocess_batch.argtypes = [vp, vp, vp, ci, vp, ci, ci, ci, vp, vp, ci, ci, vp]
        L.cddmsl_preprocess224_batch.argtypes = [vp, vp, vp, ci, vp] + [ci] * 8 + [vp, vp, ci, vp]
        L.cddmsl_tta_view.argtypes = [vp] + [ci] * 4 + [vp, vp, vp, ci] * 2 + [vp, ci, ci, ci] * 2 + [ci, vp, vp, ci, ci, vp]
        L.cddmsl_resize_batch_u8.argtypes = [vp, c_long, vp, c_long, vp, c_long, vp, ci, vp]
        L.cddmsl_avgpool2_fwd.argtypes = [vp, vp] + [ci] * 5 + [vp]
        L.cddmsl_avgpool2_bwd.argtypes = [vp] * 4 + [ci] * 5 + [vp]
        L.cddmsl_avgpool2_bwd_q8.argtypes = [vp] * 4 + [ci] * 4 + [vp] * 4
        L.cddmsl_avgpool2_fwd_bits.argtypes = [vp] * 3 + [ci] * 5 + [vp]
        L.cddmsl_avgpool2_bwd_bits.argtypes = [vp] * 3 + [ci] * 5 + [vp]
        L.cddmsl_conv3x3_pool_fwd.argtypes = [vp] * 6 + [ci] * 7 + [vp]
        L.cddmsl_attn_tokens_fwd.argtypes = [vp] * 3 + [ci] * 5 + [vp]
        L.cddmsl_attn_tokens_bwd.argtypes = [vp] * 4 + [ci] * 5 + [vp]
        L.cddmsl_attnpool_softmax_fwd.argtypes = [vp] * 3 + [c_long, ci, ci, ci, cf, ci, vp]
        L.cddmsl_attnpool_softmax_bwd.argtypes = [vp] * 4 + [c_long, ci, ci, ci, cf, ci, vp]
        L.cddmsl_gemm_nt_batched.argtypes = [vp] * 4 + [ci] * 7 + [c_long] * 3 + [ci, ci, vp]
        L.cddmsl_gemm_tn_batched.argtypes = [vp] * 3 + [ci] * 7 + [c_long] * 3 + [ci, ci, vp]
        L.cddmsl_relu_bwd.argtypes = [vp, vp, vp, c_long, ci, ci, vp]
        L.cddmsl_colsum.argtypes = [vp, vp, c_long, ci, ci, ci, vp]
        L.cddmsl_sgd_clip_step.argtypes = [vp] * 4 + [ci, vp] + [cf] * 4 + [ci, vp]
        L.cddmsl_roi_align_forward.argtypes = [vp] * 5 + [ci] * 7 + [cf, ci, ci, ci, vp]
        L.cddmsl_roi_align_backward.argtypes = [vp] * 7 + [ci] * 7 + [cf, ci, ci, ci, vp]
        L.cddmsl_nms_anyorder.argtypes = [vp] * 4 + [ci, cf, vp, vp, vp]
        L.cddmsl_soft_nms.argtypes = [vp] * 6 + [ci, ci, cf, cf, cf, ci, vp, vp, vp]
        L.cddmsl_openset_logits.argtypes = [vp] * 4 + [ci] * 4 + [cf, cf, vp]
        L.cddmsl_openset_select.argtypes = [vp, vp, ci, vp, ci, vp, ci, ci, cf, cf, cf] + [vp] * 6 + [ci, vp, vp, vp]
        L.cddmsl_roi_align_nchw_anyorder.argtypes = [vp] * 3 + [ci] * 7 + [cf, ci, ci, ci, vp, vp, vp]
        L.cddmsl_roi_align_backward_nchw_anyorder.argtypes = [vp] * 3 + [ci] * 7 + [cf, ci, ci, ci, vp, vp, vp]
        L.cddmsl_quantize_fp8.argtypes = [vp] * 4 + [c_long, ci, vp]
        L.cddmsl_conv_fwd_fp8.argtypes = [vp] * 7 + [ci] * 10 + [vp] * 4
        L.cddmsl_conv_wgrad_fp8_ok.argtypes = [ci] * 6
        L.cddmsl_conv_wgrad_fp8.argtypes = [vp] * 4 + [ci] * 9 + [vp]
        L.cddmsl_conv_fwd_q8.argtypes = [vp] * 7 + [ci] * 10 + [vp] * 4
        L.cddmsl_fp8_dot_nt.argtypes = [vp] * 4 + [ci] * 4 + [vp]
        L.cddmsl_roi_align_forward_affine.argtypes = [vp] * 6 + [ci] * 8 + [cf, ci, ci, ci] + [vp] * 4
        L.cddmsl_roi_align_backward_pooled.argtypes = [vp] * 7 + [ci] * 7 + [cf, ci, ci, ci, vp]
        L.cddmsl_anchors.argtypes = [vp, vp, ci, ci, ci, cf, cf, vp]
        L.cddmsl_sort_desc.argtypes = [vp] * 5 + [ci, ci, vp, vp, vp]
        L.cddmsl_rpn_decode.argtypes = [vp] * 6 + [ci] * 5 + [cf] * 8 + [vp]
        L.cddmsl_nms.argtypes = [vp] * 5 + [ci, ci, cf, ci, vp]
        L.cddmsl_iou_match.argtypes = [vp, ci, vp, ci, vp, vp, vp, ci, cf, cf, ci, ci, ci, ci, vp]
        L.cddmsl_iou_match_batched.argtypes = [vp] * 7 + [ci] * 5 + [cf, cf] + [ci] * 4 + [vp]
        L.cddmsl_l2norm_fwd.argtypes = [vp, vp, vp, c_long, ci, cf, vp]
        L.cddmsl_l2norm_bwd.argtypes = [vp, vp, vp, vp, c_long, ci, vp]
        L.cddmsl_cosine_logits_fwd.argtypes = [vp] * 4 + [c_long, ci, ci, cf, cf, vp]
        L.cddmsl_cosine_logits_bwd.argtypes = [vp] * 5 + [c_long, ci, ci, cf, ci, vp]
        L.cddmsl_layernorm_fwd.argtypes = [vp] * 6 + [c_long, ci, cf, ci, vp]
        L.cddmsl_layernorm_bwd.argtypes = [vp] * 6 + [c_long, ci, ci, ci, vp]
        L.cddmsl_layernorm_bwd_emit.argtypes = [vp] * 7 + [c_long, ci, ci, ci, ctypes.POINTER(ci), vp]
        L.cddmsl_focal_ce_fwd.argtypes = [vp] * 4 + [c_long, ci, cf, ci, cf, vp]
        L.cddmsl_focal_ce_bwd.argtypes = [vp] * 5 + [c_long, ci, cf, ci, cf, vp]
        L.cddmsl_attn_small_fwd.argtypes = [vp] * 4 + [ci] * 8 + [cf, ci, vp]
        L.cddmsl_attn_small_bwd.argtypes = [vp] * 7 + [ci] * 8 + [cf, ci, vp]
        L.cddmsl_attn_tokens_fwd_mask.argtypes = [vp] * 4 + [ci] * 5 + [vp]
        L.cddmsl_attnpool_dx.argtypes = [vp] * 6 + [ci] * 6 + [vp]
        L.cddmsl_rpn_losses.argtypes = [vp, vp, vp, ci, vp, ci, vp, vp, vp, vp, c_long, cf, cf, cf, cf, cf, vp, vp, vp, vp, vp]
        L.cddmsl_box_l1.argtypes = [vp, ci, vp, ci, vp, vp, vp, cf, cf, cf, cf, cf, vp, vp, vp, vp]
        L.cddmsl_rpn_losses_reg.argtypes = [vp, vp, vp, ci, vp, ci, vp, vp, vp, vp, c_long, cf, cf, cf, cf, cf, ci, cf, cf, vp, vp, vp, vp, vp]
        L.cddmsl_box_reg_loss.argtypes = [vp, ci, vp, ci, vp, vp, vp, cf, cf, cf, cf, cf, ci, cf, cf, vp, vp, vp, vp]
        L.cddmsl_attn_last_fwd.argtypes = [vp] * 4 + [ci] * 8 + [cf, ci, vp]
        L.cddmsl_attn_last_bwd.argtypes = [vp] * 6 + [ci] * 8 + [cf, ci, vp]
        L.cddmsl_contrastive_fwd.argtypes = [vp] * 4 + [ci, ci, vp]
        L.cddmsl_contrastive_bwd.argtypes = [vp] * 5 + [ci, ci, vp]
        L.cddmsl_instance_boxes.argtypes = [vp] + [ci] * 4 + [vp, ci, vp, vp, vp, vp]
        L.cddmsl_text_embed.argtypes = [vp] * 4 + [c_long, ci, ci, ci, ci, vp]
        L.cddmsl_attn_causal_fwd.argtypes = [vp, vp] + [ci] * 6 + [cf, ci, vp]
        L.cddmsl_quick_gelu.argtypes = [vp, c_long, ci, vp]
        L.cddmsl_text_pool.argtypes = [vp] * 5 + [c_long, ci, ci, ci, cf, ci, vp]
        L.cddmsl_skinny_gemm_workspace.argtypes = [ci] * 3
        L.cddmsl_skinny_gemm.argtypes = [vp] * 6 + [c_long] + [ci] * 4 + [vp]
        L.cddmsl_lm_head_workspace.argtypes = [ci, ci]
        L.cddmsl_lm_head_argmax.argtypes = [vp, vp, vp, ci, vp, vp, c_long, ci, ci, ci, vp]
        L.cddmsl_decode_attn.argtypes = [vp] * 4 + [ci] * 6 + [cf, ci, vp]
        L.cddmsl_pos_embed.argtypes = [vp, ci] + [vp] * 4 + [c_long] + [ci] * 6 + [vp]
        L.cddmsl_gelu_new.argtypes = [vp, c_long, ci, vp]
        L.cddmsl_lm_head_topk_workspace.argtypes = [ci, ci]
        L.cddmsl_lm_head_topk.argtypes = [vp] * 7 + [c_long] + [ci] * 4 + [vp]
        L.cddmsl_beam_step.argtypes = [vp] * 15 + [ci] * 5 + [vp]
        L.cddmsl_decode_attn_beam.argtypes = [vp] * 7 + [ci] * 9 + [cf, ci, vp]
        _sigs_done = True
    return L


class _Profiler:

    def __init__(self):
        self.on = False
        self.only = None
        self.events = []
        self.shapes = []

    def enable(self, only=None):
        self.on, self.only, self.events, self.shapes = True, (set(only) if only else None), [], []

    def begin(self, name=None, plan=None):
        if not self.on:
            return None
        if self.only is not None:
            if name is None and plan is not None:
                L = _L()
                L.cddmsl_plan_only(1)
                try:
                    plan()
                finally:
                    L.cddmsl_plan_only(0)
                name = _CONV_KERNEL.get(L.cddmsl_last_kernel())
            if name not in self.only:
                return None
        e = torch.cuda.Event(enable_timing=True)
        e.record()
        return e

    def end(self, e0, name, flops=0.0, shape=None, nbytes=0.0):
        if e0 is None:
            return
        e1 = torch.cuda.Event(enable_timing=True)
        e1.record()
        self.events.append((name, flops, e0, e1, nbytes))
        if shape is not None:
            self.shapes.append((name, shape, flops, e0, e1, nbytes))

    def by_shape(self):
        torch.cuda.synchronize()
        out = {}
        for name, shape, flops, e0, e1, nbytes in self.shapes:
            d = out.setdefault((name, shape), [0, 0.0, 0.0, 0.0])
            d[0] += 1
            d[1] += e0.elapsed_time(e1)
            d[2] += flops
            d[3] += nbytes
        return out

    def collect(self):
        torch.cuda.synchronize()
        out = {}
        for name, flops, e0, e1, nbytes in self.events:
            d = out.setdefault(name, {"flops": 0.0, "ms": 0.0, "launches": 0, "bytes": 0.0})
            d["flops"] += flops
            d["bytes"] += nbytes
            d["ms"] += e0.elapsed_time(e1)
            d["launches"] += 1
        self.on, self.only, self.events = False, None, []
        return out


PROFILE = _Profiler()
_CONV_KERNEL = {10: "k_conv_fwd256_fp8", 11: "k_conv_fwd2", 1: "k_conv_fwd", 2: "k_conv_fwd_reg", 3: "k_conv_fwd256", 4: "k_conv_wgrad", 5: "k_conv_wgrad_dma", 6: "k_wgrad256", 7: "k_gemm_tn_stream", 8: "k_conv3x3_small", 9: "k_gemm_tn_small", 12: "k_wgrad256_fp8",
                13: "k_bottleneck64"}


def _timed(name):
    def deco(fn):
        def wrapper(*a, **k):
            e0 = PROFILE.begin(name)
            r = fn(*a, **k)
            PROFILE.end(e0, name)
            return r
        wrapper.__name__, wrapper.__doc__ = fn.__name__, fn.__doc__
        return wrapper
    return deco


def _dt(t):
    if t.dtype not in DT:
        raise TypeError(f"unsupported dtype {t.dtype}: the kernels compute in bf16 or f32")
    return DT[t.dtype]


def _conv_input_pixels(N, H, W, Ho, Wo, KH, KW, stride, pool):
    if pool:
        return N * min(H, 2 * Ho) * min(W, 2 * Wo)
    rows = min(H, Ho * min(KH, stride) if stride > KH else (Ho - 1) * stride + KH)
    cols = min(W, Wo * min(KW, stride) if stride > KW else (Wo - 1) * stride + KW)
    return N * rows * cols


class OutSpec:

    def __init__(self):
        self.full, self.used = None, 0


def conv_fwd(x, w, scale=None, bias=None, residual=None, relu=False, relu_mask=None, stride=1, pad=0,
             pool=False, out_f32=False, residual_pooled=False, emit8=None, out_spec=None):
    require_cuda(x, w, scale, bias, residual, relu_mask)
    ensure_workspace(x.device)
    assert x.dim() == 4 and w.dim() == 4 and x.is_contiguous() and w.is_contiguous()
    assert x.dtype == w.dtype
    N, H, W, Cin = x.shape
    Cout, KH, KW, Cin2 = w.shape
    assert Cin == Cin2, (x.shape, w.shape)
    if pool:
        Ho, Wo = H // 2, W // 2
    else:
        Ho, Wo = (H + 2 * pad - KH) // stride + 1, (W + 2 * pad - KW) // stride + 1
    ydt = torch.float32 if out_f32 else x.dtype
    if out_spec is not None and out_spec.full is None:
        out_spec.full = torch.empty((2 * N, Ho, Wo, Cout), device=x.device, dtype=ydt)
        y, out_spec.used = out_spec.full[:N], 1
    elif out_spec is not None and out_spec.used == 1 and tuple(out_spec.full.shape) == (2 * N, Ho, Wo, Cout) and out_spec.full.dtype == ydt:
        y, out_spec.used = out_spec.full[N:], 2
    else:
        y = torch.empty((N, Ho, Wo, Cout), device=x.device, dtype=ydt)
    for v in (scale, bias):
        assert v is None or (v.dtype == torch.float32 and v.numel() == Cout and v.is_contiguous())
    res_f32 = residual is not None and residual.dtype == torch.float32 and x.dtype != torch.float32
    if res_f32:
        assert out_f32 and relu_mask is None and not pool and Cout % 8 == 0
    if residual_pooled:
        assert residual is not None and not res_f32 and residual.dtype == x.dtype and residual.is_contiguous()
        assert tuple(residual.shape) == (N, Ho // 2, Wo // 2, Cout) and pooled_residual_ok(residual), residual.shape
    for v in (residual, relu_mask):
        assert v is None or (v is residual and residual_pooled) or (
            (v.dtype == x.dtype or (v is residual and res_f32)) and v.is_contiguous() and v.numel() == y.numel())
    y8 = None
    if emit8 is not None:
        assert x.dtype == torch.bfloat16 and not out_f32 and not pool and not residual_pooled and not res_f32
        y8 = torch.empty(y.shape, device=x.device, dtype=torch.uint8)

    def launch():
        if y8 is not None:
            return _L().cddmsl_conv_fwd_q8(ptr(x), ptr(w), ptr(y), ptr(scale), ptr(bias), ptr(residual), ptr(relu_mask),
                                           N, H, W, Cin, Cout, KH, KW, stride, pad, int(relu), ptr(y8), ptr(emit8[0]), ptr(emit8[1]), stream_ptr())
        return _L().cddmsl_conv_fwd(ptr(x), ptr(w), ptr(y), ptr(scale), ptr(bias), ptr(residual), ptr(relu_mask),
                                    N, H, W, Cin, Cout, KH, KW, stride, pad, int(pool), Cout, Cout, Cout,
                                    int(relu), int(out_f32) | (2 if res_f32 else 0) | (4 if residual_pooled else 0), _dt(x), stream_ptr())
    e0 = PROFILE.begin(plan=launch) if PROFILE.on else None
    st = launch()
    check(st, "cddmsl_conv_fwd")
    PROFILE.end(e0, _CONV_KERNEL.get(_L().cddmsl_last_kernel(), "conv_fwd") if e0 is not None else "conv_fwd",
                2.0 * N * Ho * Wo * Cout * KH * KW * Cin,
                (N * Ho * Wo, Cout, KH * KW * Cin, KH, int(pool), stride),
                nbytes=float(_conv_input_pixels(N, H, W, Ho, Wo, KH, KW, stride, bool(pool)) * Cin * x.element_size()
                             + w.numel() * w.element_size() + y.numel() * y.element_size()
                             + (residual.numel() * residual.element_size() if residual is not None else 0)
                             + (relu_mask.numel() * relu_mask.element_size() if relu_mask is not None else 0)))
    if y8 is not None:
        y._fp8 = (y8, emit8[0].data_ptr())
    return y


def conv3x3_pool_fwd(x, w, scale, bias, relu_mask=None, stride=1):
    require_cuda(x, w, scale, bias, relu_mask)
    assert x.dim() == 4 and w.dim() == 4 and x.is_contiguous() and w.is_contiguous() and x.dtype == w.dtype
    N, H, W, Cin = x.shape
    Cout, KH, KW, Cin2 = w.shape
    assert (KH, KW, Cin2) == (3, 3, Cin), (x.shape, w.shape)
    for v in (scale, bias):
        assert v is not None and v.dtype == torch.float32 and v.numel() == Cout and v.is_contiguous()
    assert relu_mask is None or (relu_mask.dtype == x.dtype and relu_mask.is_contiguous())
    y = torch.empty((N, H // 2, W // 2, Cout), device=x.device, dtype=x.dtype)

    def launch():
        return _L().cddmsl_conv3x3_pool_fwd(ptr(x), ptr(w), ptr(y), ptr(scale), ptr(bias), ptr(relu_mask), N, H, W, Cin, Cout, stride,
                                            _dt(x), stream_ptr())
    e0 = PROFILE.begin(plan=launch) if PROFILE.on else None
    check(launch(), "cddmsl_conv3x3_pool_fwd")
    Mc = N * (H // 2) * (W // 2) * 4
    PROFILE.end(e0, "k_conv3x3_small", 2.0 * Mc * Cout * 9 * Cin, (Mc, Cout, 9 * Cin, 3, 2, 1),
                nbytes=float(x.numel() * x.element_size() + w.numel() * w.element_size() + y.numel() * y.element_size()))
    return y


def bottleneck64_ok(o1, w2, w3, wd=None, w1n=None):
    if not (o1.is_cuda and o1.dtype == torch.bfloat16 and o1.dim() == 4 and o1.is_contiguous() and o1.shape[3] == 64):
        return False
    want = ((w2, (64, 3, 3, 64)), (w3, (256, 1, 1, 64)), (wd, (256, 1, 1, 64)), (w1n, (64, 1, 1, 256)))
    if any(w is not None and (tuple(w.shape) != s or w.dtype != torch.bfloat16 or not w.is_contiguous()) for w, s in want):
        return False
    N, H, W, _ = o1.shape
    return N > 0 and bool(_L().cddmsl_bottleneck64_ok(N, H, W, 0))


def bottleneck64_fwd(o1, w2, bn2, w3, bn3, residual=None, x0=None, wd=None, bnd=None, w1n=None, bn1n=None):
    require_cuda(o1, w2, w3, residual, x0, wd, w1n)
    assert bottleneck64_ok(o1, w2, w3, wd, w1n) and (residual is None) != (wd is None)
    N, H, W, _ = o1.shape
    for t, c in ((residual, 256), (x0 if wd is not None else None, 64)):
        assert t is None or (t.dtype == torch.bfloat16 and t.is_contiguous() and tuple(t.shape) == (N, H, W, c))
    for bn, c in ((bn2, 64), (bn3, 256), (bnd, 256), (bn1n, 64)):
        assert bn is None or all(v.dtype == torch.float32 and v.numel() == c and v.is_contiguous() and v.is_cuda for v in bn)
    assert (wd is None) == (bnd is None) and (w1n is None) == (bn1n is None) and (wd is None or x0 is not None)
    out = torch.empty((N, H, W, 256), device=o1.device, dtype=o1.dtype)
    o1n = torch.empty((N, H, W, 64), device=o1.device, dtype=o1.dtype) if w1n is not None else None
    sd, bd = bnd if bnd is not None else (None, None)
    s1n, b1n = bn1n if bn1n is not None else (None, None)
    e0 = PROFILE.begin(name="k_bottleneck64") if PROFILE.on else None
    check(_L().cddmsl_bottleneck64_fwd(ptr(o1), ptr(w2), ptr(bn2[0]), ptr(bn2[1]), ptr(w3), ptr(bn3[0]), ptr(bn3[1]), ptr(residual),
                                       ptr(x0 if wd is not None else None), ptr(wd), ptr(sd), ptr(bd), ptr(w1n), ptr(s1n), ptr(b1n),
                                       ptr(out), ptr(o1n), N, H, W, 0, stream_ptr()), "cddmsl_bottleneck64_fwd")
    M = N * H * W
    kn = 576 * 64 + 64 * 256 + (64 * 256 if wd is not None else 0) + (256 * 64 if w1n is not None else 0)
    PROFILE.end(e0, "k_bottleneck64", 2.0 * M * kn, (M, 256, 576, 3, int(wd is not None), int(w1n is not None)),
                nbytes=float(2 * M * (64 + (64 if wd is not None else 256) + 256 + (64 if w1n is not None else 0)) + 2 * kn))
    return out, o1n


def conv_emit8_ok(M, Cout, KH, KW, Cin_chunks_ok=True):
    return Cout % 256 == 0 and KH * KW <= 31 and ((M + 255) // 256) * (Cout // 256) >= 160 and Cin_chunks_ok and os.environ.get("CDDMSL_GEMM256", "1") != "0"


FP8_MAX = 448.0


@_timed("quantize_fp8")
def quantize_fp8(x, scale=None, amax=None):
    require_cuda(x, scale, amax)
    assert x.is_contiguous() and x.dtype in (torch.bfloat16, torch.float32) and x.numel() % 8 == 0
    y = torch.empty(x.shape, device=x.device, dtype=torch.uint8)
    check(_L().cddmsl_quantize_fp8(ptr(x), ptr(y), ptr(scale), ptr(amax), x.numel(), 0 if x.dtype == torch.bfloat16 else 1, stream_ptr()),
          "cddmsl_quantize_fp8")
    return y


def conv_fwd_fp8_ok(M, Cin, Cout, KH, KW, pad):
    min_tiles = int(os.environ.get("CDDMSL_FP8_MIN_TILES", "160"))
    min_k = int(os.environ.get("CDDMSL_FP8_MIN_K", "2048"))
    return Cin % 128 == 0 and Cout % 256 == 0 and KH * KW <= 31 and 2 * pad <= KH - 1 and ((M + 255) // 256) * (Cout // 256) >= min_tiles \
        and KH * KW * Cin >= min_k


def conv_fwd_fp8(x8, w8, scale=None, bias=None, residual=None, relu=False, relu_mask=None, pad=0, out_f32=False, emit8=None):
    require_cuda(x8, w8, scale, bias, residual, relu_mask)
    assert x8.dtype == torch.uint8 and w8.dtype == torch.uint8 and x8.is_contiguous() and w8.is_contiguous()
    N, H, W, Cin = x8.shape
    Cout, KH, KW, Cin2 = w8.shape
    assert Cin == Cin2
    Ho, Wo = H + 2 * pad - KH + 1, W + 2 * pad - KW + 1
    y = torch.empty((N, Ho, Wo, Cout), device=x8.device, dtype=torch.float32 if out_f32 else torch.bfloat16)
    for v in (scale, bias):
        assert v is None or (v.dtype == torch.float32 and v.numel() == Cout and v.is_contiguous())
    for v in (residual, relu_mask):
        assert v is None or (v.dtype == torch.bfloat16 and v.is_contiguous() and v.numel() == y.numel())

    y8 = torch.empty(y.shape, device=x8.device, dtype=torch.uint8) if emit8 is not None else None
    assert emit8 is None or not out_f32

    def launch():
        return _L().cddmsl_conv_fwd_fp8(ptr(x8), ptr(w8), ptr(y), ptr(scale), ptr(bias), ptr(residual), ptr(relu_mask),
                                        N, H, W, Cin, Cout, KH, KW, pad, int(relu), int(out_f32), ptr(y8),
                                        ptr(emit8[0]) if emit8 else c_void_p(0), ptr(emit8[1]) if emit8 else c_void_p(0), stream_ptr())
    e0 = PROFILE.begin(name="k_conv_fwd256_fp8") if PROFILE.on else None
    check(launch(), "cddmsl_conv_fwd_fp8")
    PROFILE.end(e0, "k_conv_fwd256_fp8", 2.0 * N * Ho * Wo * Cout * KH * KW * Cin, (N * Ho * Wo, Cout, KH * KW * Cin, KH, 0, 1),
                nbytes=float(x8.numel() + w8.numel() + y.numel() * y.element_size() + (residual.numel() * 2 if residual is not None else 0)
                             + (relu_mask.numel() * 2 if relu_mask is not None else 0)))
    if y8 is not None:
        y._fp8 = (y8, emit8[0].data_ptr())
    return y


@_timed("fp8_dot_nt")
def fp8_dot_nt(a8, b8, alpha=None):
    require_cuda(a8, b8, alpha)
    R, K = a8.shape
    N = b8.shape[0]
    assert a8.dtype == torch.uint8 and b8.dtype == torch.uint8 and a8.is_contiguous() and b8.is_contiguous() and b8.shape[1] == K
    c = torch.empty((R, N), device=a8.device, dtype=torch.float32)
    check(_L().cddmsl_fp8_dot_nt(ptr(a8), ptr(b8), ptr(c), ptr(alpha), R, N, K, N, stream_ptr()), "cddmsl_fp8_dot_nt")
    return c


def pooled_residual_ok(t):
    return t.numel() * t.element_size() < 2 ** 31 and t.shape[-1] % 8 == 0


def linear_fwd(x, w, scale=None, bias=None, residual=None, relu=False, relu_mask=None, out_f32=False):
    M, K = x.shape
    y = conv_fwd(x.view(1, 1, M, K), w.view(w.shape[0], 1, 1, K), scale, bias,
                 None if residual is None else residual.view(1, 1, M, -1), relu,
                 None if relu_mask is None else relu_mask.view(1, 1, M, -1), out_f32=out_f32)
    return y.view(M, w.shape[0])


_WORKSPACE = {}
WORKSPACE_BYTES = 288 << 20


def ensure_workspace(device):
    key = torch.device(device).index or 0
    if key not in _WORKSPACE:
        ws = torch.empty(WORKSPACE_BYTES, dtype=torch.uint8, device=device)
        check(_L().cddmsl_set_workspace(ptr(ws), ctypes.c_long(ws.numel())), "cddmsl_set_workspace")
        _WORKSPACE[key] = ws
    return _WORKSPACE[key]


def conv_wgrad(x, dy, w_shape, scale=None, stride=1, pad=0, pool=False, out=None):
    require_cuda(x, dy, scale, out)
    Cout, KH, KW, Cin = w_shape
    N, H, W, Cin2 = x.shape
    assert Cin == Cin2 and x.dtype == dy.dtype and x.is_contiguous() and dy.is_contiguous()
    assert dy.shape[-1] == Cout and dy.numel() // Cout == (N * (H // 2) * (W // 2) if pool else
                                                          N * ((H + 2 * pad - KH) // stride + 1) * ((W + 2 * pad - KW) // stride + 1))
    if out is None:
        out = torch.zeros(w_shape, device=x.device, dtype=torch.float32)
    assert out.dtype == torch.float32 and out.is_contiguous() and tuple(out.shape) == tuple(w_shape)
    ensure_workspace(x.device)
    def launch():
        return _L().cddmsl_conv_wgrad(ptr(x), ptr(dy), ptr(out), ptr(scale), N, H, W, Cin, Cout, KH, KW, stride, pad,
                                      int(pool), Cout, _dt(x), stream_ptr())
    e0 = PROFILE.begin(plan=launch) if PROFILE.on else None
    st = launch()
    check(st, "cddmsl_conv_wgrad")
    PROFILE.end(e0, _CONV_KERNEL.get(_L().cddmsl_last_kernel(), "conv_wgrad") if e0 is not None else "conv_wgrad",
                2.0 * (dy.numel() // Cout) * Cout * KH * KW * Cin,
                (dy.numel() // Cout, Cout, KH * KW * Cin, KH, int(pool), stride),
                nbytes=float(_conv_input_pixels(N, H, W, (H // 2) if pool else (H + 2 * pad - KH) // stride + 1,
                                                 (W // 2) if pool else (W + 2 * pad - KW) // stride + 1, KH, KW, stride, bool(pool)) * Cin * x.element_size()
                             + dy.numel() * dy.element_size() + out.numel() * 4))
    return out


def conv_wgrad_fp8_ok(M, Cin, Cout, KH, KW, pad, min_m=None, taps_only=True):
    min_m = int(os.environ.get("CDDMSL_FP8_WGRAD_MIN_M", "300000" if min_m is None else str(min_m)))
    return os.environ.get("CDDMSL_FP8_WGRAD", "1") != "0" and (KH * KW > 1 or not taps_only) and M >= min_m \
        and bool(_L().cddmsl_conv_wgrad_fp8_ok(Cin, Cout, KH, KW, pad, Cout))


def conv_wgrad_fp8(x8, dy8, w_shape, scale, pad=0, out=None):
    require_cuda(x8, dy8, scale, out)
    Cout, KH, KW, Cin = w_shape
    N, H, W, Cin2 = x8.shape
    assert Cin == Cin2 and x8.dtype == torch.uint8 and dy8.dtype == torch.uint8 and x8.is_contiguous() and dy8.is_contiguous()
    assert dy8.shape[-1] == Cout and dy8.numel() // Cout == N * H * W and 2 * pad == KH - 1
    assert scale is not None and scale.dtype == torch.float32 and scale.numel() == Cout and scale.is_contiguous()
    if out is None:
        out = torch.zeros(w_shape, device=x8.device, dtype=torch.float32)
    assert out.dtype == torch.float32 and out.is_contiguous() and tuple(out.shape) == tuple(w_shape)
    ensure_workspace(x8.device)
    def launch():
        return _L().cddmsl_conv_wgrad_fp8(ptr(x8), ptr(dy8), ptr(out), ptr(scale), N, H, W, Cin, Cout, KH, KW, pad, Cout, stream_ptr())
    e0 = PROFILE.begin(name="k_wgrad256_fp8") if PROFILE.on else None
    check(launch(), "cddmsl_conv_wgrad_fp8")
    PROFILE.end(e0, "k_wgrad256_fp8", 2.0 * (N * H * W) * Cout * KH * KW * Cin, (N * H * W, Cout, KH * KW * Cin, KH, 0, 1),
                nbytes=float(x8.numel() + dy8.numel() + out.numel() * 4))
    return out


@_timed("weight_prep")
def weight_prep(w_master, scale, dtype, want_fwd=True, want_dgrad=True):
    require_cuda(w_master, scale)
    assert w_master.dtype == torch.float32 and w_master.is_contiguous() and w_master.dim() == 4
    Cout, KH, KW, Cin = w_master.shape
    wf = torch.empty((Cout, KH, KW, Cin), device=w_master.device, dtype=dtype) if want_fwd else None
    wd = torch.empty((Cin, KH, KW, Cout), device=w_master.device, dtype=dtype) if want_dgrad else None
    st = _L().cddmsl_weight_prep(ptr(w_master), ptr(scale), ptr(wf), ptr(wd), Cout, KH, KW, Cin, DT[dtype], stream_ptr())
    check(st, "cddmsl_weight_prep")
    return wf, wd


@_timed("weight_prep")
def weight_prep_multi(table, count, dtype):
    require_cuda(table)
    assert table.dtype == torch.int64 and table.is_contiguous() and table.shape == (count, 8)
    check(_L().cddmsl_weight_prep_multi(ptr(table), count, DT[dtype], stream_ptr()), "cddmsl_weight_prep_multi")


def _f3(v):
    return (c_float * 3)(*[float(x) for x in v])


def _image_table(images_u8):
    import ctypes
    n = len(images_u8)
    ptrs = (ctypes.c_void_p * n)(*[im.data_ptr() for im in images_u8])
    hs = (ctypes.c_int * n)(*[int(im.shape[1]) for im in images_u8])
    ws = (ctypes.c_int * n)(*[int(im.shape[2]) for im in images_u8])
    return ptrs, hs, ws


@_timed("preprocess")
def preprocess(images_u8, Hp, Wp, mean, std, dtype, Cp=None, div255=True):
    require_cuda(*images_u8)
    Cp = Cp or (8 if dtype == torch.bfloat16 else 4)
    out = torch.empty((len(images_u8), Hp, Wp, Cp), device=images_u8[0].device, dtype=dtype)
    m, s = _f3(mean), _f3(std)
    for im in images_u8:
        assert im.dtype == torch.uint8 and im.dim() == 3 and im.shape[0] == 3 and im.is_contiguous()
    ptrs, hs, ws = _image_table(images_u8)
    check(_L().cddmsl_preprocess_batch(ptrs, hs, ws, len(images_u8), ptr(out), Hp, Wp, Cp, m, s, int(div255), DT[dtype], stream_ptr()),
          "cddmsl_preprocess_batch")
    return out


@_timed("preprocess224")
def preprocess224(images_u8, Hp, Wp, mean, std, dtype, size=224, Cp=None):
    require_cuda(*images_u8)
    Cp = Cp or (8 if dtype == torch.bfloat16 else 4)
    if Wp <= Hp:
        RW, RH = size, int(size * Hp / Wp)
    else:
        RH, RW = size, int(size * Wp / Hp)
    top, left = int(round((RH - size) / 2.0)), int(round((RW - size) / 2.0))
    out = torch.empty((len(images_u8), size, size, Cp), device=images_u8[0].device, dtype=dtype)
    m, s = _f3(mean), _f3(std)
    for im in images_u8:
        assert im.dtype == torch.uint8 and im.dim() == 3 and im.is_contiguous()
    ptrs, hs, ws = _image_table(images_u8)
    check(_L().cddmsl_preprocess224_batch(ptrs, hs, ws, len(images_u8), ptr(out), Hp, Wp, RH, RW, top, left, size, Cp,
                                           m, s, DT[dtype], stream_ptr()), "cddmsl_preprocess224_batch")
    return out


from .resample import resample_table as _resample_table


def tta_view_list(sizes, flip):
    return [(int(nh), int(nw), f) for nh, nw in sizes for f in ((False, True) if flip else (False,))]


@_timed("tta_views")
def tta_views(image_u8, sizes, flip, mean, std, dtype, batch_size=3, div255=True):
    import numpy as np
    require_cuda(image_u8)
    assert image_u8.dtype == torch.uint8 and image_u8.dim() == 3 and image_u8.shape[0] == 3 and image_u8.is_contiguous()
    assert batch_size >= 1
    h, w = int(image_u8.shape[1]), int(image_u8.shape[2])
    Cp = 8 if dtype == torch.bfloat16 else 4
    sizes = [(int(a), int(b)) for a, b in sizes]
    views = tta_view_list(sizes, flip)
    groups = []
    for g0 in range(0, len(views), batch_size):
        vs = views[g0:g0 + batch_size]
        Hp, Wp = max(v[0] for v in vs), max(v[1] for v in vs)
        groups.append((torch.empty((len(vs), Hp, Wp, Cp), device=image_u8.device, dtype=dtype), [(v[0], v[1]) for v in vs]))
    parts, where, off = [], {}, 0
    for insize, outsize in sorted({(w, nw) for _, nw in sizes if nw != w} | {(h, nh) for nh, _ in sizes if nh != h}):
        lo, n, k, ks = _resample_table(insize, outsize)
        where[(insize, outsize)] = (off, off + outsize, off + 2 * outsize, ks)
        parts += [lo, n, k.reshape(-1)]
        off += 2 * outsize + outsize * ks
    tab = None
    if parts:
        from ._lib import to_device_async
        tab = to_device_async(torch.from_numpy(np.concatenate(parts)), image_u8.device)

    def axis(insize, outsize):
        if insize == outsize:
            return c_void_p(0), c_void_p(0), c_void_p(0), 0
        a, b, c, ks = where[(insize, outsize)]
        base = tab.data_ptr()
        return c_void_p(base + 4 * a), c_void_p(base + 4 * b), c_void_p(base + 4 * c), ks

    m, s = _f3(mean), _f3(std)
    per = 2 if flip else 1
    for i, (nh, nw) in enumerate(sizes):
        v0 = i * per
        t0, t1 = groups[v0 // batch_size][0], (groups[(v0 + 1) // batch_size][0] if flip else None)
        check(_L().cddmsl_tta_view(ptr(image_u8), h, w, nh, nw, *axis(w, nw), *axis(h, nh),
                                   ptr(t0), v0 % batch_size, t0.shape[1], t0.shape[2],
                                   ptr(t1), (v0 + 1) % batch_size if flip else 0, t1.shape[1] if flip else 0, t1.shape[2] if flip else 0,
                                   Cp, m, s, int(div255), DT[dtype], stream_ptr()), "cddmsl_tta_view")
    return groups


class ResizeItem(ctypes.Structure):
    _fields_ = [("src_off", c_long), ("dst_off", c_long)] + [(k, c_int) for k in (
        "h", "w", "newh", "neww", "flip", "reverse_channels", "xtab", "xks", "ytab", "yks")]


def resize_batch_u8(src, dst, tab, items):
    require_cuda(src, dst, tab)
    assert src.dtype == torch.uint8 and dst.dtype == torch.uint8 and src.is_contiguous() and dst.is_contiguous()
    assert tab is None or (tab.dtype == torch.int32 and tab.is_contiguous())
    arr = (ResizeItem * max(len(items), 1))(*[ResizeItem(*(int(v) for v in it)) for it in items])
# ... 1045 lines not shown
```

cddmsl_amd/layers.py:

```python
import os
import weakref

import torch

from . import hip

_STEP = [0]


def bump_weight_version():
    _STEP[0] += 1


_LOAD_GEN = [0]


def note_weights_loaded(*_):
    _LOAD_GEN[0] += 1
    _STEP[0] += 1


def load_generation():
    return _LOAD_GEN[0]

# ... 156 lines not shown

def _fp8_eligible(pw, in_shape, pad=0):
    Cout, KH, KW, Cin = _ohwi(pw.param).shape
    N, H, W, _ = in_shape
    M = N * (H + 2 * pad - KH + 1) * (W + 2 * pad - KW + 1)
    return hip.conv_fwd_fp8_ok(M, Cin, Cout, KH, KW, pad)


def fp8_emit_for(consumer_pw, out_shape, pad, fp8, producer_cout=None, producer_taps=1):
    if not fp8 or consumer_pw is None or not _fp8_eligible(consumer_pw, out_shape, pad):
        return None
    M = out_shape[0] * out_shape[1] * out_shape[2]
    if producer_cout is not None and not hip.conv_emit8_ok(M, producer_cout, producer_taps, 1):
        return None
    return fp8_act_slot(consumer_pw).emit()


def fp8_copy(t, slot):
    made = getattr(t, "_fp8", None)
    if made is not None and made[1] == slot.scale.data_ptr():
        return made[0]
    slot.calibrate(t)
    t8 = hip.quantize_fp8(t, slot.scale, slot.amax)
    t._fp8 = (t8, slot.scale.data_ptr())
    return t8


def wgrad_auto(x, dy, pw, scale, pad, out, fp8=False, x8=None, dy_slot=None, min_m=None, taps_only=True):
    Cout, KH, KW, Cin = _ohwi(pw.param).shape
    if fp8 and x8 is not None and dy_slot is not None and dy.dtype == torch.bfloat16 \
            and hip.conv_wgrad_fp8_ok(dy.numel() // Cout, Cin, Cout, KH, KW, pad, min_m, taps_only):
        d8 = fp8_copy(dy, dy_slot)
        deq = fp8_act_slot(pw).deq * dy_slot.deq
        eff = deq * scale if scale is not None else deq.expand(Cout).contiguous()
        return hip.conv_wgrad_fp8(x8, d8, (Cout, KH, KW, Cin), eff, pad=pad, out=out)
    return hip.conv_wgrad(x, dy, (Cout, KH, KW, Cin), scale, pad=pad, out=out)


def _fp8_wgrad1x1_wanted(pw, M, fp8):
    if not fp8 or os.environ.get("CDDMSL_FP8_WGRAD_1X1", "1") == "0":
        return False
    Cout, KH, KW, Cin = _ohwi(pw.param).shape
    return KH == 1 and KW == 1 and hip.conv_wgrad_fp8_ok(M, Cin, Cout, 1, 1, 0, None, False)


def _fp8_made_for(t, pw):
    made = getattr(t, "_fp8", None)
    sl = getattr(pw, "_fp8_slot", None)
    return made[0] if made is not None and sl is not None and made[1] == sl.scale.data_ptr() else None


def conv_fwd_auto(x, pw, scale=None, bias=None, fp8=False, emit8=None, **kw):
    T = x.dtype
    if fp8 and T == torch.bfloat16 and kw.get("stride", 1) == 1 and not kw.get("out_f32", False) and kw.get("out_spec") is None:
        Cout = _ohwi(pw.param).shape[0]
        pad = kw.get("pad", 0)
        if _fp8_eligible(pw, x.shape, pad):
            sl = fp8_act_slot(pw)
            x8 = fp8_copy(x, sl)
            w8, d_w = fp8_weight(pw)
            eff = (sl.deq * d_w) * scale if scale is not None else (sl.deq * d_w).expand(Cout).contiguous()
            return hip.conv_fwd_fp8(x8, w8, eff, bias, kw.get("residual"), kw.get("relu", False), kw.get("relu_mask"), pad, emit8=emit8)
    wf, _ = pw.get(T, need_dgrad=False)
    if emit8 is not None:
        Cout, KH, KW, Cin = _ohwi(pw.param).shape
        N, H, W, _ = x.shape
        pad = kw.get("pad", 0)
        M = N * (H + 2 * pad - KH + 1) * (W + 2 * pad - KW + 1)
        if not (T == torch.bfloat16 and hip.conv_emit8_ok(M, Cout, KH, KW, (Cin * 2 // 16) % 8 == 0) and kw.get("stride", 1) == 1):
            emit8 = None
    return hip.conv_fwd(x, wf, scale, bias, emit8=emit8, **kw)


def fp8_weight_d(pw, wd):
    key = (-1 if pw.frozen else _STEP[0], wd.data_ptr(), pw.param._version, _LOAD_GEN[0])
    c = getattr(pw, "_fp8d", None)
    if c is None or c[0] != key:
        amax = wd.abs().amax().float().clamp_min(1e-20).view(1)
        pw._fp8d = c = (key, hip.quantize_fp8(wd, hip.FP8_MAX / amax), amax / hip.FP8_MAX)
    return c[1], c[2]


def fp8_slot_of(owner, name):
    sl = getattr(owner, name, None)
    dev = (owner.param if hasattr(owner, "param") else owner.w[0]).device
    if sl is None or sl.scale.device != dev:
        sl = FP8_SCALES.slot(dev)
        setattr(owner, name, sl)
    return sl


def dgrad_auto(g, pw, fp8=False, slot=None, emit8=None, **kw):
    T = g.dtype
    _, wd = pw.get(T, True)
    if fp8 and T == torch.bfloat16 and slot is not None and not kw.get("residual_pooled", False):
        Cout_d, KH, KW, Cin_d = wd.shape
        pad = kw.get("pad", 0)
        N, H, W, _ = g.shape
        M = N * (H + 2 * pad - KH + 1) * (W + 2 * pad - KW + 1)
        if hip.conv_fwd_fp8_ok(M, Cin_d, Cout_d, KH, KW, pad):
            g8 = fp8_copy(g, slot)
            wd8, d_w = fp8_weight_d(pw, wd)
            return hip.conv_fwd_fp8(g8, wd8, (slot.deq * d_w).expand(Cout_d).contiguous(), None, kw.get("residual"), False, kw.get("relu_mask"),
                                    pad, emit8=emit8)
    if emit8 is not None:
        Cout_d, KH, KW, Cin_d = wd.shape
        N, H, W, _ = g.shape
        pad = kw.get("pad", 0)
        M = N * (H + 2 * pad - KH + 1) * (W + 2 * pad - KW + 1)
        if not (T == torch.bfloat16 and hip.conv_emit8_ok(M, Cout_d, KH, KW, (Cin_d * 2 // 16) % 8 == 0) and not kw.get("residual_pooled", False)):
            emit8 = None
    return hip.conv_fwd(g, wd, emit8=emit8, **kw)


def _fp8_dgrad_wanted(pw, g_shape, pad, fp8):
    if not fp8:
        return False
    Cout, KH, KW, Cin = _ohwi(pw.param).shape
    N, H, W, _ = g_shape
    M = N * (H + 2 * pad - KH + 1) * (W + 2 * pad - KW + 1)
    return hip.conv_fwd_fp8_ok(M, Cout, Cin, KH, KW, pad)


def cat_prepared(weights, dtype):
    return torch.cat([hip.weight_prep(_ohwi(w.detach()), None, dtype, True, False)[0] for w in weights], dim=0)


_BF16_OF = {}


def _bf16_key(g):
    return (g.data_ptr(), g.numel(), g.device)


def _register_bf16(g, gb):
    _BF16_OF.clear()
    if gb is not None:
        _BF16_OF[_bf16_key(g)] = (g, g._version, gb)


def bf16_of(g):
    if _BF16_OF and g.dtype == torch.float32 and g.is_contiguous():
        e = _BF16_OF.pop(_bf16_key(g), None)
        if e is not None and e[0]._version == e[1] and g._version == e[1]:
            return e[2].view(g.shape)
    return g.to(torch.bfloat16)


class ConvFn(torch.autograd.Function):

    @staticmethod
    def forward(ctx, x, anchor, pw, bias, stride, pad, relu, out_f32, train_w, residual=None, fp8=False):
        y = conv_fwd_auto(x, pw, None, None if bias is None else bias.detach(), fp8, residual=None if residual is None else residual.detach(),
                          relu=relu, stride=stride, pad=pad, out_f32=out_f32)
        ctx.pw, ctx.bias, ctx.cfg = pw, bias, (stride, pad, relu, out_f32, train_w)
        ctx.fp8 = bool(fp8)
        ctx.save_for_backward(x, y if relu else None, _fp8_made_for(x, pw) if fp8 else None)
        return y

    @staticmethod
    def backward(ctx, dy):
        x, y, x8 = ctx.saved_tensors
        stride, pad, relu, out_f32, train_w = ctx.cfg
        f8 = ctx.fp8 and x8 is not None and stride == 1
        g_slot = fp8_slot_of(ctx.pw, "_fp8_g") if f8 else None
        T = x.dtype
        dy_in = dy
        dy = dy.contiguous()
        if relu:
            dy = hip.relu_bwd(dy, y if y.dtype == T else y.to(T))
        elif dy.dtype != T:
            dy = bf16_of(dy) if T == torch.bfloat16 else dy.to(T)
        w = ctx.pw.param
        if train_w:
            if f8:
                wgrad_auto(x, dy, ctx.pw, None, pad, _ohwi(_grad_buf(w)), True, x8, g_slot, min_m=65536)
            else:
                hip.conv_wgrad(x, dy, _ohwi(w).shape, None, stride=stride, pad=pad, out=_ohwi(_grad_buf(w)))
            if ctx.bias is not None:
                hip.colsum(dy.view(-1, dy.shape[-1]), out=_grad_buf(ctx.bias))
        dx = None
        if ctx.needs_input_grad[0]:
            assert stride == 1, "input gradient of a strided conv is not on the hot path"
            _, wd = ctx.pw.get(T, need_dgrad=True)
            KH = _ohwi(w).shape[1]
            Kd, rows = dy.shape[-1], dy.numel() // dy.shape[-1]
            if KH == 1 and _ohwi(w).shape[2] == 1 and pad == 0 and rows <= 1024 and Kd >= 8192 and Kd % (16 * 64) == 0:
                S, N = 16, x.shape[-1]
                part = torch.empty(S, rows, N, device=dy.device, dtype=torch.float32)
                hip.gemm_nt_batched(dy, wd, part, rows, N, Kd // S, Kd, Kd, N, S, Kd // S, Kd // S, rows * N)
                dx = part.sum(0).to(T).view(x.shape)
            elif f8:
                dx = dgrad_auto(dy, ctx.pw, True, g_slot, pad=KH - 1 - pad)
            else:
                dx = hip.conv_fwd(dy, wd, stride=1, pad=KH - 1 - pad)
        return dx, None, None, None, None, None, None, None, None, (dy_in if ctx.needs_input_grad[9] else None), None


class FrozenMlpFn(torch.autograd.Function):

    @staticmethod
    def forward(ctx, x, pw1, b1, pw2, b2, residual):
        T = x.dtype
        w1, _ = pw1.get(T, need_dgrad=False)
        w2, _ = pw2.get(T, need_dgrad=False)
        M, K = x.shape
        h = hip.conv_fwd(x.view(1, 1, M, K), w1, None, b1.detach(), relu=True)
        y = hip.conv_fwd(h, w2, None, b2.detach(), residual.detach().view(1, 1, M, -1), out_f32=True)
        ctx.pw = (pw1, pw2)
        ctx.save_for_backward(h)
        return y.view(M, -1)

    @staticmethod
    def backward(ctx, dy):
        (h,) = ctx.saved_tensors
        T = h.dtype
        M = h.shape[2]
        g = dy.contiguous()
        if g.dtype != T:
            g = bf16_of(g) if T == torch.bfloat16 else g.to(T)
        _, w2d = ctx.pw[1].get(T, need_dgrad=True)
        _, w1d = ctx.pw[0].get(T, need_dgrad=True)
        dh = hip.conv_fwd(g.view(1, 1, M, -1), w2d, relu_mask=h)
        dx = hip.conv_fwd(dh, w1d).view(M, -1) if ctx.needs_input_grad[0] else None
        return dx, None, None, None, None, (dy if ctx.needs_input_grad[5] else None)


def frozen_mlp(x2d, pw1, b1, pw2, b2, residual):
    return FrozenMlpFn.apply(x2d.contiguous(), pw1, b1, pw2, b2, residual.contiguous())


def conv(x, pw, bias=None, stride=1, pad=0, relu=False, out_f32=False, train_w=True, residual=None, fp8=False):
    anchor = pw.param if train_w else None
    assert residual is None or not relu
    return ConvFn.apply(x, anchor, pw, bias, stride, pad, relu, out_f32, train_w, residual, fp8)


def linear(x2d, pw, bias=None, relu=False, out_f32=False, train_w=True, residual=None):
    M, K = x2d.shape
    y = conv(x2d.contiguous().view(1, 1, M, K), pw, bias, 1, 0, relu, out_f32, train_w,
             None if residual is None else residual.contiguous().view(1, 1, M, -1))
    return y.view(M, -1)


class FusedHeadsFn(torch.autograd.Function):

    @staticmethod
    def forward(ctx, x, anchor, heads, out_f32):
        T = x.dtype
        K = heads[0][0].shape[1] if heads[0][0].dim() == 2 else heads[0][0].shape[1]
        ws = [w.detach().reshape(w.shape[0], -1) for w, _ in heads]
        n = sum(w.shape[0] for w in ws)
        npad = (n + 7) // 8 * 8
        wcat = torch.zeros(npad, 1, 1, ws[0].shape[1], device=x.device, dtype=torch.float32)
        wcat[:n, 0, 0] = torch.cat(ws, dim=0)
        bcat = torch.zeros(npad, device=x.device, dtype=torch.float32)
        bcat[:n] = torch.cat([b.detach() for _, b in heads])
        wf, wd = hip.weight_prep(wcat, None, T, True, True)
        y = hip.conv_fwd(x, wf, None, bcat, out_f32=out_f32)
        ctx.heads, ctx.wd, ctx.npad = heads, wd, npad
        ctx.save_for_backward(x)
        return y

    @staticmethod
    def backward(ctx, dy):
        (x,) = ctx.saved_tensors
        T = x.dtype
        dy = dy.contiguous()
        if dy.dtype != T:
            dy = dy.to(T)
        K = x.shape[-1]
        dw = hip.conv_wgrad(x, dy, (ctx.npad, 1, 1, K))
        db = hip.colsum(dy.view(-1, ctx.npad))
        off = 0
        for w, b in ctx.heads:
            n = w.shape[0]
            _grad_buf(w).view(n, -1).add_(dw[off:off + n].view(n, -1)) if w.dim() == 2 else \
                _ohwi(_grad_buf(w)).add_(dw[off:off + n])
            _grad_buf(b).add_(db[off:off + n])
            off += n
        dx = hip.conv_fwd(dy, ctx.wd) if ctx.needs_input_grad[0] else None
        return dx, None, None, None


def fused_heads(x, heads, out_f32=True):
    return FusedHeadsFn.apply(x, heads[0][0], heads, out_f32)


class BlockParams:

    def __init__(self, w1, w2, w3, wd, bn1, bn2, bn3, bnd, stride, frozen, fp8=False):
        self.stride, self.frozen, self.fp8 = stride, frozen, fp8
        self.bn = (bn1, bn2, bn3, bnd)
        self.w = (w1, w2, w3, wd)
        self.pw = tuple(None if w is None else PreparedWeight(w, b[0], frozen) for w, b in zip(self.w, self.bn))


def _pool_bits_wanted(bp, o2):
    if os.environ.get("CDDMSL_POOL_MASK_BITS", "1") == "0" or o2.dtype != torch.bfloat16 or o2.shape[-1] % 8:
        return False
    return not (bp.fp8 and _fp8_dgrad_wanted(bp.pw[1], o2.shape, 1, True))


def _block_forward(x, bp, save, px_given=None, next_pw=None, out_spec=None):
    (s1, b1), (s2, b2), (s3, b3), bnd = bp.bn
    pool = bp.stride > 1
    f8 = bp.fp8
    o1_shape = (x.shape[0], x.shape[1], x.shape[2], _ohwi(bp.w[0]).shape[0])
    o1 = conv_fwd_auto(x, bp.pw[0], s1, b1, f8, emit8=fp8_emit_for(bp.pw[1], o1_shape, 1, f8), relu=True)
    x8 = _fp8_made_for(x, bp.pw[0]) if f8 and save else None
    M2 = x.shape[0] * x.shape[1] * x.shape[2]
    e8o2 = fp8_act_slot(bp.pw[2]).emit() if save and not pool and _fp8_wgrad1x1_wanted(bp.pw[2], M2, f8) else None
    o2 = conv_fwd_auto(o1, bp.pw[1], s2, b2, f8, emit8=e8o2, relu=True, pad=1)
    o2_8 = _fp8_made_for(o2, bp.pw[2]) if e8o2 is not None else None
    o2_shape, bits = tuple(o2.shape), None
    if pool and save and _pool_bits_wanted(bp, o2):
        p2, bits = hip.avgpool2_fwd_bits(o2)
    else:
        p2 = hip.avgpool2_fwd(o2) if pool else o2
    if pool and px_given is not None and tuple(px_given.shape) == (x.shape[0], x.shape[1] // 2, x.shape[2] // 2, x.shape[3]):
        px = px_given
    else:
        px = hip.avgpool2_fwd(x) if pool else x
    if bp.pw[3] is not None:
        idn = conv_fwd_auto(px, bp.pw[3], bnd[0], bnd[1], f8)
    else:
        idn = x
    out_shape = (p2.shape[0], p2.shape[1], p2.shape[2], _ohwi(bp.w[2]).shape[0])
    out = conv_fwd_auto(p2, bp.pw[2], s3, b3, f8, emit8=fp8_emit_for(next_pw, out_shape, 0, f8), residual=idn, relu=True, out_spec=out_spec)
    return out, ((o1, o2 if bits is None else bits, p2 if pool else None, px if pool else None,
                  (x8, _fp8_made_for(o1, bp.pw[1]) if f8 else None, o2_8), o2_shape) if save else None)


def _block_backward(gs, x, o1, o2, p2, px, bp, need_dx, mask_x, prev_bp=None, c8=(None, None, None), o2_shape=None):
    T = x.dtype
    (s1, _), (s2, _), (s3, _), bnd = bp.bn
    pool = bp.stride > 1
    f8 = bp.fp8 and T == torch.bfloat16
    w1p, w2p, w3p, wdp = bp.w
    shp = lambda w: _ohwi(w).shape
    gs_slot = fp8_slot_of(bp, "_fp8_gs") if f8 else None
    d2_slot = fp8_slot_of(bp.pw[1], "_fp8_g") if f8 else None
    x8, o1_8, o2_8 = c8
    o2_bits = o2.dtype == torch.int32
    o2_shape = tuple(o2.shape) if o2_shape is None else tuple(o2_shape)
    M2 = o2_shape[0] * o2_shape[1] * o2_shape[2]
    if o2_8 is not None and not pool:
        wgrad_auto(o2, gs, bp.pw[2], s3, 0, _ohwi(_grad_buf(w3p)), f8, o2_8, gs_slot, taps_only=False)
    else:
        hip.conv_wgrad(p2 if pool else o2, gs, shp(w3p), s3, out=_ohwi(_grad_buf(w3p)))
    d1_slot = fp8_slot_of(bp.pw[0], "_fp8_g") if f8 and x8 is not None and _fp8_wgrad1x1_wanted(bp.pw[0], M2, f8) else None
    if pool:
        dp2 = dgrad_auto(gs, bp.pw[2], f8, gs_slot)
        if o2_bits:
            dpre2 = hip.avgpool2_bwd_bits(dp2, o2_shape, o2)
        else:
            dpre2 = hip.avgpool2_bwd(dp2, o2_shape, mask=o2, emit8=d2_slot.emit() if f8 and _fp8_dgrad_wanted(bp.pw[1], o2_shape, 1, f8) else None)
    else:
        e8 = d2_slot.emit() if f8 and _fp8_dgrad_wanted(bp.pw[1], o2_shape, 1, f8) else None
        dpre2 = dgrad_auto(gs, bp.pw[2], f8, gs_slot, emit8=e8, relu_mask=o2)
    dpre1 = dgrad_auto(dpre2, bp.pw[1], f8, d2_slot, pad=1, relu_mask=o1, emit8=d1_slot.emit() if d1_slot is not None else None)
    wgrad_auto(o1, dpre2, bp.pw[1], s2, 1, _ohwi(_grad_buf(w2p)), f8, o1_8, d2_slot)
    if d1_slot is not None:
        wgrad_auto(x, dpre1, bp.pw[0], s1, 0, _ohwi(_grad_buf(w1p)), f8, x8, d1_slot, taps_only=False)
    else:
        hip.conv_wgrad(x, dpre1, shp(w1p), s1, out=_ohwi(_grad_buf(w1p)))
    if wdp is not None:
        hip.conv_wgrad(px if pool else x, gs, shp(wdp), bnd[0], out=_ohwi(_grad_buf(wdp)))
    if not need_dx:
        return None
    pooled = False
    if wdp is not None:
        dxb = dgrad_auto(gs, bp.pw[3], f8, gs_slot)
        if pool:
            pooled = x.shape[1] % 2 == 0 and x.shape[2] % 2 == 0 and hip.pooled_residual_ok(dxb)
            if not pooled:
                dxb = hip.avgpool2_bwd(dxb, tuple(x.shape))
    else:
        dxb = gs
    e8 = None
    if f8 and prev_bp is not None and prev_bp.fp8 and not pooled and _fp8_dgrad_wanted(prev_bp.pw[2], x.shape, 0, True):
        e8 = fp8_slot_of(prev_bp, "_fp8_gs").emit()
    return dgrad_auto(dpre1, bp.pw[0], False, None, emit8=e8, residual=dxb, relu_mask=x if mask_x else None, residual_pooled=pooled)


class ResStageFn(torch.autograd.Function):
    @staticmethod
    def forward(ctx, x, anchor, blocks, out_grad_premasked=False, px0=None, out_spec=None):
        ctx.out_grad_premasked = out_grad_premasked
        saved, o1_8s, o2_shapes = [x], [], []
        cur = x
        for bi, bp in enumerate(blocks):
            cur, mids = _block_forward(cur, bp, True, px0 if bi == 0 else None, blocks[bi + 1].pw[0] if bi + 1 < len(blocks) else None,
                                       out_spec if bi + 1 == len(blocks) else None)
            saved += [mids[0], mids[1], mids[2], mids[3], cur]
            o1_8s += list(mids[4])
            o2_shapes.append(mids[5])
        ctx.blocks, ctx.o2_shapes = blocks, o2_shapes
        ctx.save_for_backward(*saved, *o1_8s)
        return cur

    @staticmethod
    def backward(ctx, g):
        blocks = ctx.blocks
        saved, o1_8s = ctx.saved_tensors[:-3 * len(blocks)], ctx.saved_tensors[-3 * len(blocks):]
        need_dx = ctx.needs_input_grad[0]
        gs = g.contiguous() if ctx.out_grad_premasked else hip.relu_bwd(g.contiguous(), saved[-1])
        for i in range(len(blocks) - 1, -1, -1):
            x, o1, o2, p2, px = saved[5 * i: 5 * i + 5]
            gs = _block_backward(gs, x, o1, o2, p2, px, blocks[i], need_dx or i > 0, mask_x=i > 0, prev_bp=blocks[i - 1] if i > 0 else None,
                                 c8=tuple(o1_8s[3 * i: 3 * i + 3]), o2_shape=ctx.o2_shapes[i])
        return gs, None, None, None, None, None


def _fused_stage_ok(x, blocks, out_spec):
    if os.environ.get("CDDMSL_FUSED_BOTTLENECK", "1") == "0" or out_spec is not None:
        return False
    if not (x.is_cuda and x.dtype == torch.bfloat16 and x.dim() == 4 and x.is_contiguous()):
        return False
    cin = x.shape[3]
    for bi, bp in enumerate(blocks):
        if bp.fp8 or bp.stride != 1 or any(v is None for b in bp.bn[:3] for v in b):
            return False
        if tuple(_ohwi(bp.w[0]).shape) != (64, 1, 1, cin) or tuple(_ohwi(bp.w[1]).shape) != (64, 3, 3, 64) or tuple(_ohwi(bp.w[2]).shape) != (256, 1, 1, 64):
            return False
        if bp.w[3] is not None:
            if bi > 0 or cin != 64 or tuple(_ohwi(bp.w[3]).shape) != (256, 1, 1, 64) or any(v is None for v in bp.bn[3]):
                return False
        elif cin != 256:
            return False
        cin = 256
    return bool(blocks) and bool(hip._L().cddmsl_bottleneck64_ok(x.shape[0], x.shape[1], x.shape[2], 0))


def _fused_stage_forward(x, blocks):
    T = x.dtype
    wf = lambda pw: pw.get(T, need_dgrad=False)[0]
    o1 = conv_fwd_auto(x, blocks[0].pw[0], blocks[0].bn[0][0], blocks[0].bn[0][1], False, relu=True)
    cur = x
    for bi, bp in enumerate(blocks):
        nxt = blocks[bi + 1] if bi + 1 < len(blocks) else None
        kw = dict(x0=cur, wd=wf(bp.pw[3]), bnd=bp.bn[3]) if bp.pw[3] is not None else dict(residual=cur)
        if nxt is not None:
            kw.update(w1n=wf(nxt.pw[0]), bn1n=nxt.bn[0])
        cur, o1 = hip.bottleneck64_fwd(o1, wf(bp.pw[1]), bp.bn[1], wf(bp.pw[2]), bp.bn[2], **kw)
    return cur


def res_stage(x, blocks, frozen, out_grad_premasked=False, out_spec=None):
    px0 = getattr(x, "_pooled2", None)
    if frozen or not torch.is_grad_enabled():
        if _fused_stage_ok(x, blocks, out_spec):
            return _fused_stage_forward(x, blocks)
        cur = x
        for bi, bp in enumerate(blocks):
            cur, _ = _block_forward(cur, bp, False, px0 if bi == 0 else None, blocks[bi + 1].pw[0] if bi + 1 < len(blocks) else None,
                                    out_spec if bi + 1 == len(blocks) else None)
        return cur
    return ResStageFn.apply(x, blocks[0].w[0], blocks, out_grad_premasked, px0, out_spec)


class StackHalvesFn(torch.autograd.Function):

    @staticmethod
    def forward(ctx, a, b, full):
        n = a.shape[0]
        assert a.data_ptr() == full.data_ptr() and b.data_ptr() == full[n:].data_ptr() and full.shape[0] == 2 * n and a.shape == b.shape
        ctx.n = n
        return full.view(full.shape)

    @staticmethod
    def backward(ctx, g):
        return g[:ctx.n], g[ctx.n:], None


def stack_halves(a, b, full):
    return StackHalvesFn.apply(a, b, full)


def res_stage_attnpool(x, blocks, frozen, ap):
    fuse = not frozen and torch.is_grad_enabled()
    y = res_stage(x, blocks, frozen, out_grad_premasked=fuse)
    return AttnPoolFn.apply(y, None if ap.frozen else ap.q_w, ap, fuse)


def roi_downsample_on_map(K, out_size, N, H, W):
    if os.environ.get("CDDMSL_ROI_COMMUTE", "1") == "0":
        return False
    v = os.environ.get("CDDMSL_ROI_COMMUTE_DOWN", "")
    if v in ("0", "1"):
        return v == "1"
    return K * (out_size // 2) ** 2 > N * H * W


def _roi_block0_forward(feat, rois, bp, out_size, scale, sr, extra, next_pw=None, on_map=None, save=False):
    T = feat.dtype
    (s1, b1), (s2, b2), (s3, b3), bnd = bp.bn
    w1, _ = bp.pw[0].get(T, False)
    f8 = bp.fp8
    K, E = rois.shape[0], (0 if extra is None else extra.shape[0])
    N, H, W, _ = feat.shape
    z = hip.conv_fwd(feat, w1)
    o1_shape = (K + E, out_size, out_size, z.shape[-1])
    e8 = fp8_emit_for(bp.pw[1], o1_shape, 1, f8) if E == 0 else None
    o1 = hip.roi_align_forward_affine(z, rois, out_size, out_size, scale, sr, True, s1, b1, relu=True, extra_rows=E, emit8=e8)
    del z
    if on_map is None:
        on_map = roi_downsample_on_map(K, out_size, N, H, W)
    if on_map:
        wd, _ = bp.pw[3].get(T, False)
        zd = hip.conv_fwd(feat, wd)
        idn = hip.roi_align_forward_affine(zd, rois, out_size, out_size, scale, sr, True, bnd[0], bnd[1], pooled_only=True, extra_rows=E)
        del zd
        px = None
        if E:
            px = hip.avgpool2_fwd(extra)
            idn[K:].copy_(hip.conv_fwd(px, wd, bnd[0], bnd[1]))
    else:
        px = hip.roi_align_forward_affine(feat, rois, out_size, out_size, scale, sr, True, pooled_only=True, extra_rows=E)
        idn = None
    if E:
        o1[K:].copy_(hip.conv_fwd(extra, w1, s1, b1, relu=True))
        if idn is None:
            px[K:].copy_(hip.avgpool2_fwd(extra))
    o2 = conv_fwd_auto(o1, bp.pw[1], s2, b2, f8, relu=True, pad=1)
    o2_shape = tuple(o2.shape)
    if save and _pool_bits_wanted(bp, o2):
        p2, o2 = hip.avgpool2_fwd_bits(o2)
    else:
        p2 = hip.avgpool2_fwd(o2)
    if idn is None:
        idn = conv_fwd_auto(px, bp.pw[3], bnd[0], bnd[1], f8)
    out_shape = (p2.shape[0], p2.shape[1], p2.shape[2], _ohwi(bp.w[2]).shape[0])
    out = conv_fwd_auto(p2, bp.pw[2], s3, b3, f8, emit8=fp8_emit_for(next_pw, out_shape, 0, f8), residual=idn, relu=True)
    return o1, o2, p2, px, out, (_fp8_made_for(o1, bp.pw[1]) if f8 else None), o2_shape


class RoIStageFn(torch.autograd.Function):

    @staticmethod
    def forward(ctx, feat, anchor, rois, roi_start, blocks, out_size, scale, sr, out_grad_premasked, extra):
        feat = feat.contiguous()
        nxt = lambda i: blocks[i + 1].pw[0] if i + 1 < len(blocks) else None
        on_map = roi_downsample_on_map(rois.shape[0], out_size, feat.shape[0], feat.shape[1], feat.shape[2])
        o1, o2, p2, px, cur, o1_8, o2_shape = _roi_block0_forward(feat, rois, blocks[0], out_size, scale, sr, extra, nxt(0), on_map, save=True)
        saved, o1_8s, o2_shapes = [feat, rois, roi_start, extra, o1, o2, p2, px, cur], [None, o1_8, None], [o2_shape]
        for bi, bp in enumerate(blocks[1:], start=1):
            cur, mids = _block_forward(cur, bp, True, None, nxt(bi))
            saved += [mids[0], mids[1], mids[2], mids[3], cur]
            o1_8s += list(mids[4])
            o2_shapes.append(mids[5])
        ctx.o2_shapes = o2_shapes
        ctx.blocks, ctx.meta = blocks, (out_size, scale, sr, out_grad_premasked, on_map)
        ctx.save_for_backward(*saved, *o1_8s)
        return cur

    @staticmethod
    def backward(ctx, g):
        blocks = ctx.blocks
        saved, o1_8s = ctx.saved_tensors[:-3 * len(blocks)], ctx.saved_tensors[-3 * len(blocks):]
        out_size, scale, sr, premasked, on_map = ctx.meta
        feat, rois, roi_start, extra = saved[:4]
        st = saved[4:]
        gs = g.contiguous() if premasked else hip.relu_bwd(g.contiguous(), st[-1])
        for i in range(len(blocks) - 1, 0, -1):
            o1, o2, p2, px = st[5 * i: 5 * i + 4]
            gs = _block_backward(gs, st[5 * i - 1], o1, o2, p2, px, blocks[i], True, mask_x=True, prev_bp=blocks[i - 1], c8=tuple(o1_8s[3 * i: 3 * i + 3]),
                                 o2_shape=ctx.o2_shapes[i])
        bp = blocks[0]
        o1, o2, p2, px = st[0:4]
        o2_shape = ctx.o2_shapes[0]
        T = o1.dtype
        (s1, _), (s2, _), (s3, _), bnd = bp.bn
        w1p, w2p, w3p, wdp = bp.w
        shp = lambda w: _ohwi(w).shape
        K, E = rois.shape[0], (0 if extra is None else extra.shape[0])
        f8 = bp.fp8 and T == torch.bfloat16
        gs_slot = fp8_slot_of(bp, "_fp8_gs") if f8 else None
        d2_slot = fp8_slot_of(bp.pw[1], "_fp8_g") if f8 else None
        hip.conv_wgrad(p2, gs, shp(w3p), s3, out=_ohwi(_grad_buf(w3p)))
        if o2.dtype == torch.int32:
            dpre2 = hip.avgpool2_bwd_bits(dgrad_auto(gs, bp.pw[2], f8, gs_slot), o2_shape, o2)
        else:
            e8 = d2_slot.emit() if f8 and _fp8_dgrad_wanted(bp.pw[1], o2_shape, 1, f8) else None
            dpre2 = hip.avgpool2_bwd(dgrad_auto(gs, bp.pw[2], f8, gs_slot), o2_shape, mask=o2, emit8=e8)
        dpre1 = dgrad_auto(dpre2, bp.pw[1], f8, d2_slot, pad=1, relu_mask=o1)
        wgrad_auto(o1, dpre2, bp.pw[1], s2, 1, _ohwi(_grad_buf(w2p)), f8, o1_8s[1], d2_slot)
        N, H, W, C = feat.shape
        _, w1d = bp.pw[0].get(T, True)
        dfeat = dextra = dzd = wdd = None
        if on_map:
            _, wdd = bp.pw[3].get(T, True)
            dzd = hip.roi_align_backward(gs[:K], rois, roi_start, (N, H, W, gs.shape[-1]), scale, sr, True, pooled=True)
            hip.conv_wgrad(feat, dzd, shp(wdp), bnd[0], out=_ohwi(_grad_buf(wdp)))
            if E:
                hip.conv_wgrad(px, gs[K:], shp(wdp), bnd[0], out=_ohwi(_grad_buf(wdp)))
        else:
            hip.conv_wgrad(px, gs, shp(wdp), bnd[0], out=_ohwi(_grad_buf(wdp)))
            dxb = dgrad_auto(gs, bp.pw[3], f8, gs_slot)
        dz = hip.roi_align_backward(dpre1[:K], rois, roi_start, (N, H, W, dpre1.shape[-1]), scale, sr, True)
        hip.conv_wgrad(feat, dz, shp(w1p), s1, out=_ohwi(_grad_buf(w1p)))
        if E:
            hip.conv_wgrad(extra, dpre1[K:], shp(w1p), s1, out=_ohwi(_grad_buf(w1p)))
            if ctx.needs_input_grad[9]:
                dxe = hip.conv_fwd(gs[K:], wdd) if on_map else dxb[K:].contiguous()
                dextra = hip.conv_fwd(dpre1[K:], w1d, residual=hip.avgpool2_bwd(dxe, tuple(extra.shape)))
        if ctx.needs_input_grad[0]:
            r = hip.conv_fwd(dzd, wdd) if on_map else hip.roi_align_backward(dxb[:K], rois, roi_start, (N, H, W, C), scale, sr, True, pooled=True)
            dfeat = hip.conv_fwd(dz, w1d, residual=r)
        return dfeat, None, None, None, None, None, None, None, None, dextra


def roi_stage_supported(blocks):
    bp = blocks[0]
    return bp.stride == 2 and bp.w[3] is not None and tuple(bp.w[0].shape[2:]) == (1, 1) and tuple(bp.w[3].shape[2:]) == (1, 1)


def roi_stage(feat, rois, roi_start, blocks, frozen, out_size, scale, sr, extra=None, out_grad_premasked=False):
    assert rois.dim() == 2 and rois.size(1) == 5 and out_size % 2 == 0
    assert extra is None or tuple(extra.shape[1:]) == (out_size, out_size, feat.shape[3])
    if frozen or not torch.is_grad_enabled():
        nxt = lambda i: blocks[i + 1].pw[0] if i + 1 < len(blocks) else None
        cur = _roi_block0_forward(feat.contiguous(), rois, blocks[0], out_size, scale, sr, extra, nxt(0))[4]
        for bi, bp in enumerate(blocks[1:], start=1):
            cur, _ = _block_forward(cur, bp, False, None, nxt(bi))
        return cur
    return RoIStageFn.apply(feat, blocks[0].w[0], rois, roi_start, blocks, out_size, scale, sr, out_grad_premasked, extra)


def roi_stage_attnpool(feat, rois, roi_start, blocks, frozen, ap, out_size, scale, sr, extra=None):
    fuse = not frozen and torch.is_grad_enabled()
    y = roi_stage(feat, rois, roi_start, blocks, frozen, out_size, scale, sr, extra, out_grad_premasked=fuse)
    return AttnPoolFn.apply(y, None if ap.frozen else ap.q_w, ap, fuse)


class RoIAlignFn(torch.autograd.Function):
    @staticmethod
    def forward(ctx, x, rois, roi_start, out_size, scale, sampling_ratio, aligned, with_pooled=False, extra=None):
        K, E = rois.shape[0], (0 if extra is None else extra.shape[0])
        out = hip.roi_align_forward(x, rois, out_size, out_size, scale, sampling_ratio, aligned, with_pooled=with_pooled, extra_rows=E)
        ctx.save_for_backward(rois, roi_start)
        ctx.meta = (tuple(x.shape), scale, sampling_ratio, aligned, K)
        y = out[0] if with_pooled else out
        if E:
            y[K:].copy_(extra)
            if with_pooled:
                out[1][K:].copy_(hip.avgpool2_fwd(extra.contiguous()))
        if with_pooled:
            ctx.mark_non_differentiable(out[1])
        return out

    @staticmethod
    def backward(ctx, dy, *unused):
        rois, roi_start = ctx.saved_tensors
        shape, scale, sr, aligned, K = ctx.meta
        dy = dy.contiguous()
        dx = hip.roi_align_backward(dy[:K], rois, roi_start, shape, scale, sr, aligned)
        dextra = dy[K:] if (dy.shape[0] > K and ctx.needs_input_grad[8]) else None
        return dx, None, None, None, None, None, None, None, dextra


def roi_align(x, rois, roi_start, out_size, scale, sampling_ratio, aligned=True, with_pooled=False, extra=None):
    assert rois.dim() == 2 and rois.size(1) == 5
    assert extra is None or tuple(extra.shape[1:]) == (out_size, out_size, x.shape[3])
    if with_pooled and out_size % 2 == 0:
        y, yp = RoIAlignFn.apply(x, rois, roi_start, out_size, scale, sampling_ratio, aligned, True, extra)
        y._pooled2 = yp
        return y
    return RoIAlignFn.apply(x, rois, roi_start, out_size, scale, sampling_ratio, aligned, False, extra)


class AttnPoolParams:
    def __init__(self, pos, q_w, q_b, k_w, k_b, v_w, v_b, c_w, c_b, heads, frozen=False):
        self.pos, self.heads, self.frozen = pos, heads, frozen
        self.q_w, self.q_b, self.k_w, self.k_b, self.v_w, self.v_b, self.c_w, self.c_b = q_w, q_b, k_w, k_b, v_w, v_b, c_w, c_b
        self.pq = PreparedWeight(q_w, None, frozen)
        self.pk = PreparedWeight(k_w, None, frozen)
        self.pv = PreparedWeight(v_w, None, frozen)
        self.pc = PreparedWeight(c_w, None, frozen)


class AttnPoolFn(torch.autograd.Function):

    TP = 56

    @staticmethod
    def forward(ctx, x, anchor, ap, premask_input_grad=False):
        ctx.relu_src = x if premask_input_grad else None
        T = x.dtype
        K, h, w, C = x.shape
        P, TP, H = h * w, AttnPoolFn.TP, ap.heads
        D = C // H
        assert ap.pos.shape[0] == P + 1 <= TP, "attention pool needs a 7x7 map (clip_backbone.py:86)"
        dev = x.device
        fused_dx = hip.attnpool_dx_ok(K, H, P, TP, C, T) and bool(ctx.needs_input_grad[0]) and os.environ.get("CDDMSL_ATTNPOOL_DX", "1") != "0"
        mbits = None
        if fused_dx and premask_input_grad:
            tok, mbits = hip.attn_tokens_fwd_mask(x.view(K, P, C), ap.pos.detach(), TP)
        else:
            tok = hip.attn_tokens_fwd(x.view(K, P, C), ap.pos.detach(), TP)
        wq, _ = ap.pq.get(T, False)
        wk, wkT = ap.pk.get(T, True)
        wv, wvT = ap.pv.get(T, True)
        wc, _ = ap.pc.get(T, False)
        q0 = hip.conv_fwd(tok.view(K, 1, TP, C), wq, None, ap.q_b.detach(), stride=TP).view(K, C)
        zu = torch.empty((K, 2 * H, C), device=dev, dtype=T)
        hip.gemm_nt_batched(q0, wkT, zu, K, C, D, C, C, 2 * H * C, H, D, D, C, c_off=H * C)
        S = torch.empty((K, H, TP), device=dev, dtype=torch.float32)
        hip.gemm_nt_batched(zu, tok, S, H, TP, C, C, C, TP, K, 2 * H * C, TP * C, H * TP, a_off=H * C)
        p, pT = hip.attnpool_softmax_fwd(S, P + 1, D ** -0.5, T)
        z = torch.empty((K, H, C), device=dev, dtype=T)
        hip.gemm_tn_batched(pT, tok, z, TP, H, C, H, C, C, K, TP * H, TP * C, H * C)
        o = torch.empty((K, C), device=dev, dtype=T)
        hip.gemm_nt_batched(z, wv, o, K, D, C, H * C, C, C, H, C, D * C, D)
        o = o + ap.v_b.detach().to(T)
        out = hip.conv_fwd(o.view(1, 1, K, C), wc, None, ap.c_b.detach(), out_f32=True).view(K, -1)
        ctx.ap = ap
        ctx.fused_dx = fused_dx
        ctx.save_for_backward(tok, q0, zu, p, z, o, mbits)
        ctx.shape = (K, h, w, C)
        return out

    @staticmethod
    def backward(ctx, dout):
        ap = ctx.ap
        tok, q0, zu, p, z, o, mbits = ctx.saved_tensors
        K, h, w, C = ctx.shape
        P, TP, H = h * w, AttnPoolFn.TP, ap.heads
        D = C // H
        T = tok.dtype
        dev = tok.device
        train = not ap.frozen
        dout_t = dout.contiguous().to(T)
        if train:
            hip.conv_wgrad(o.view(1, 1, K, C), dout_t.view(1, 1, K, -1), _ohwi(ap.c_w).shape, out=_ohwi(_grad_buf(ap.c_w)))
            hip.colsum(dout_t, out=_grad_buf(ap.c_b))
        _, wcd = ap.pc.get(T, True)
        wk, wkT = ap.pk.get(T, True)
        wv, wvT = ap.pv.get(T, True)
        do = hip.conv_fwd(dout_t.view(1, 1, K, -1), wcd).view(K, C)
        if train:
            hip.colsum(do, out=_grad_buf(ap.v_b))
            hip.gemm_tn_batched(do, z, _grad_buf(ap.v_w), K, D, C, C, H * C, C, H, D, C, D * C, accumulate=True)
        hip.gemm_nt_batched(do, wvT, zu, K, C, D, C, C, 2 * H * C, H, D, D, C)
        dP = torch.empty((K, H, TP), device=dev, dtype=torch.float32)
        hip.gemm_nt_batched(zu, tok, dP, H, TP, C, C, C, TP, K, 2 * H * C, TP * C, H * TP)
        dsT, pds = hip.attnpool_softmax_bwd(p, dP, D ** -0.5, T)
        du = torch.empty((K, H, C), device=dev, dtype=T)
        hip.gemm_tn_batched(dsT, tok, du, TP, H, C, H, C, C, K, TP * H, TP * C, H * C)
        dq0 = torch.empty((K, C), device=dev, dtype=T)
        hip.gemm_nt_batched(du, wk, dq0, K, D, C, H * C, C, C, H, C, D * C, D)
        if train:
            hip.gemm_tn_batched(q0, du, _grad_buf(ap.k_w), K, D, C, C, H * C, C, H, D, C, D * C, accumulate=True)
            _grad_buf(ap.k_b)
            hip.conv_wgrad(tok.view(K, 1, TP, C), dq0.view(K, 1, 1, C), _ohwi(ap.q_w).shape, stride=TP, out=_ohwi(_grad_buf(ap.q_w)))
            hip.colsum(dq0, out=_grad_buf(ap.q_b))
        _, wqd = ap.pq.get(T, True)
        gpos = _grad_buf(ap.pos) if train else None
        want_dx = ctx.needs_input_grad[0]
        if ctx.fused_dx and want_dx:
            g0 = hip.conv_fwd(dq0.view(1, 1, K, C), wqd, out_f32=True).view(K, C)
            if mbits is None:
                mbits = torch.full((K, C), -1, device=dev, dtype=torch.int64)
            dx = hip.attnpool_dx(pds, zu, g0, mbits, P, gpos)
            return dx.view(K, h, w, C), None, None, None
        dtok = torch.empty((K, TP, C), device=dev, dtype=T)
        hip.gemm_tn_batched(pds, zu, dtok, 2 * H, TP, C, TP, C, C, K, 2 * H * TP, 2 * H * C, TP * C)
        dtok[:, 0, :] += hip.conv_fwd(dq0.view(1, 1, K, C), wqd).view(K, C)
        dx = None
        if want_dx or train:
            dx = hip.attn_tokens_bwd(dtok, P, ctx.relu_src if want_dx else None, gpos, want_dx)
        return (dx.view(K, h, w, C) if want_dx else None), None, None, None


def attnpool(x, ap):
    return AttnPoolFn.apply(x, None if ap.frozen else ap.q_w, ap)


_FP8_CONST = {}


def _fp8_const(value, device):
    k = (float(value), str(device))
    if k not in _FP8_CONST:
        _FP8_CONST[k] = torch.tensor([float(value)], device=device, dtype=torch.float32)
    return _FP8_CONST[k]


def fp8_unit_rows(wn):
    return hip.quantize_fp8(wn.contiguous(), _fp8_const(hip.FP8_MAX, wn.device))


class CosineLogitsFn(torch.autograd.Function):
    @staticmethod
    def forward(ctx, x, wn, temperature, fp8=False, wn8=None):
        x = x.contiguous()
        if fp8 and x.shape[1] % 64 == 0 and wn.shape[0] <= 32:
            xn, inv = hip.l2norm_fwd(x, 1e-12)
            unit = _fp8_const(hip.FP8_MAX, x.device)
            if wn8 is None:
                wn8 = fp8_unit_rows(wn)
            dot = hip.fp8_dot_nt(hip.quantize_fp8(xn, unit), wn8, _fp8_const(1.0 / (hip.FP8_MAX * hip.FP8_MAX * temperature), x.device))
            scores = torch.cat([dot, torch.zeros(x.shape[0], 1, device=x.device, dtype=torch.float32)], dim=1)
        else:
            scores, inv = hip.cosine_logits_fwd(x, wn, temperature)
        ctx.save_for_backward(x, wn, inv)
        ctx.t = temperature
        return scores

    @staticmethod
    def backward(ctx, ds):
        x, wn, inv = ctx.saved_tensors
        return hip.cosine_logits_bwd(ds, x.contiguous(), wn, inv, ctx.t), None, None, None, None


def cosine_logits(x, wn, temperature, fp8=False, wn8=None):
    return CosineLogitsFn.apply(x, wn, temperature, fp8, wn8)


class ContrastiveFn(torch.autograd.Function):

    @staticmethod
    def forward(ctx, a, b):
        an, ia = hip.l2norm_fwd(a.contiguous(), 0.0)
        bn, ib = hip.l2norm_fwd(b.contiguous(), 0.0)
        S = hip.linear_fwd(an, bn)
        loss, rl, cl = hip.contrastive_fwd(S)
        ctx.save_for_backward(an, ia, bn, ib, S, rl, cl)
        return loss.view(())

    @staticmethod
    def backward(ctx, g):
        an, ia, bn, ib, S, rl, cl = ctx.saved_tensors
        dS = hip.contrastive_bwd(S, rl, cl, g)
        n = dS.shape[0]
        pad = (-n) % 4
        P = (lambda t: torch.nn.functional.pad(t, (0, pad))) if pad else (lambda t: t)
        dan = hip.linear_fwd(P(dS).contiguous(), P(bn.t()).contiguous())
        dbn = hip.linear_fwd(P(dS.t()).contiguous(), P(an.t()).contiguous())
        return hip.l2norm_bwd(dan, an, ia), hip.l2norm_bwd(dbn, bn, ib)


def contrastive_loss(a, b):
    return ContrastiveFn.apply(a, b)


class LayerNormFn(torch.autograd.Function):

    @staticmethod
    def forward(ctx, x, gamma, beta, out_dtype):
        y, mean, rstd = hip.layernorm_fwd(x.contiguous(), gamma, beta, out_dtype)
        ctx.save_for_backward(x, gamma, mean, rstd)
        return y

    @staticmethod
    def backward(ctx, dy):
        x, gamma, mean, rstd = ctx.saved_tensors
        return hip.layernorm_bwd(dy, x.contiguous(), gamma, mean, rstd), None, None, None


def layer_norm(x2d, gamma, beta, out_dtype):
    return LayerNormFn.apply(x2d, gamma.detach(), beta.detach(), out_dtype)


class LayerNormSkipFn(torch.autograd.Function):

    @staticmethod
    def forward(ctx, x, gamma, beta, out_dtype):
        x = x.contiguous()
        y, mean, rstd = hip.layernorm_fwd(x, gamma, beta, out_dtype)
        ctx.save_for_backward(x, gamma, mean, rstd)
        ctx.emit = out_dtype == torch.bfloat16
        return y, x.view_as(x)

    @staticmethod
    def backward(ctx, dy, dskip):
        x, gamma, mean, rstd = ctx.saved_tensors
        emit = ctx.emit and os.environ.get("CDDMSL_LN_EMIT_BF16", "1") != "0"
        if dskip is None:
            if emit and dy is not None:
                dx, dxb = hip.layernorm_bwd(dy, x, gamma, mean, rstd, emit_bf16=True)
                _register_bf16(dx, dxb)
                return dx, None, None, None
            return hip.layernorm_bwd(dy, x, gamma, mean, rstd), None, None, None
        acc = dskip.contiguous()
# ... 222 lines not shown
```

include/cddmsl_hip.h:

```cpp
#ifndef CDDMSL_HIP_H
#define CDDMSL_HIP_H
#include <stddef.h>

#ifdef __cplusplus
extern "C" {
#endif

int cddmsl_abi_version(void);

int cddmsl_conv_fwd(const void* x, const void* w, void* y, const float* scale, const float* bias, const void* residual,
                    const void* relu_mask, int Nimg, int Hi, int Wi, int Cin, int Cout, int KH, int KW, int stride, int pad,
                    int pool, int ldy, int ldr, int ldm, int relu, int out_f32, int dtype, void* stream);
int cddmsl_conv3x3_pool_fwd(const void* x, const void* w, void* y, const float* scale, const float* bias, const void* relu_mask,
                            int Nimg, int Hi, int Wi, int Cin, int Cout, int stride, int dtype, void* stream);
int cddmsl_bottleneck64_ok(int Nimg, int H, int W, int dtype);
int cddmsl_bottleneck64_fwd(const void* o1, const void* w2, const float* s2, const float* b2, const void* w3, const float* s3,
                            const float* b3, const void* residual, const void* x0, const void* wd, const float* sd,
                            const float* bd, const void* w1n, const float* s1n, const float* b1n, void* out, void* o1n,
                            int Nimg, int H, int W, int dtype, void* stream);
int cddmsl_set_workspace(void* ptr, long bytes);
int cddmsl_conv_wgrad(const void* x, const void* dy, float* dw, const float* scale, int Nimg, int Hi, int Wi, int Cin,
                      int Cout, int KH, int KW, int stride, int pad, int pool, int ldd, int dtype, void* stream);
int cddmsl_gemm_nt_batched(const void* a, const void* w, void* c, const float* bias, int M, int N, int K, int lda, int ldb, int ldc,
                           int batch, long sa, long sw, long sc, int out_f32, int dtype, void* stream);
int cddmsl_gemm_tn_batched(const void* a, const void* b, void* out, int M, int N, int K, int lda, int ldb, int ldo, int batch, long sa,
                           long sb, long so, int mode, int dtype, void* stream);
int cddmsl_last_kernel(void);
int cddmsl_plan_only(int on);
int cddmsl_weight_prep(const float* w, const float* scale, void* w_fwd, void* w_dgrad, int Cout, int KH, int KW, int Cin,
                       int dtype, void* stream);
int cddmsl_weight_prep_multi(const long long* table, int count, int dtype, void* stream);

int cddmsl_quantize_fp8(const void* x, void* y, const float* scale, float* amax, long numel, int src_dtype, void* stream);
int cddmsl_conv_fwd_fp8(const void* x, const void* w, void* y, const float* scale, const float* bias, const void* residual,
                        const void* relu_mask, int Nimg, int Hi, int Wi, int Cin, int Cout, int KH, int KW, int pad, int relu,
                        int out_f32, void* y8, const float* q8, float* amax8, void* stream);
int cddmsl_conv_fwd_q8(const void* x, const void* w, void* y, const float* scale, const float* bias, const void* residual,
                       const void* relu_mask, int Nimg, int Hi, int Wi, int Cin, int Cout, int KH, int KW, int stride, int pad,
                       int relu, void* y8, const float* q8, float* amax8, void* stream);
int cddmsl_fp8_dot_nt(const void* a, const void* b, float* c, const float* alpha, int R, int N, int K, int ldc, void* stream);
int cddmsl_conv_wgrad_fp8_ok(int Cin, int Cout, int KH, int KW, int pad, int ldd);
int cddmsl_conv_wgrad_fp8(const void* x8, const void* dy8, float* dw, const float* scale, int Nimg, int Hi, int Wi, int Cin, int Cout,
                          int KH, int KW, int pad, int ldd, void* stream);

int cddmsl_roi_align_forward(const void* x, const float* rois, void* y, void* y_pooled, int* dbg_grid, int N, int C, int H, int W,
                             int K, int ph, int pw, float spatial_scale, int sampling_ratio, int aligned, int dtype, void* stream);
int cddmsl_roi_align_backward(const void* dy, const float* rois, const int* roi_start, void* dx, float* ws_ay, float* ws_ax,
                              int* ws_fp, int N, int C, int H, int W, int K, int ph, int pw, float spatial_scale,
                              int sampling_ratio, int aligned, int dtype, void* stream);
int cddmsl_roi_align_forward_affine(const void* x, const float* rois, void* y, void* y_pooled, const float* scale,
                                    const float* bias, int relu, int N, int C, int H, int W, int K, int ph, int pw,
                                    float spatial_scale, int sampling_ratio, int aligned, int dtype, void* y8, const float* q8,
                                    float* amax8, void* stream);
int cddmsl_roi_align_backward_pooled(const void* dy, const float* rois, const int* roi_start, void* dx, float* ws_ay,
                                     float* ws_ax, int* ws_fp, int N, int C, int H, int W, int K, int ph, int pw,
                                     float spatial_scale, int sampling_ratio, int aligned, int dtype, void* stream);
int cddmsl_roi_align_nchw_anyorder(const void* input, const float* rois, void* output, int N, int C, int H, int W, int K, int ph, int pw,
                                   float spatial_scale, int sampling_ratio, int aligned, int dtype, void* temp, size_t* temp_bytes,
                                   void* stream);
int cddmsl_roi_align_backward_nchw_anyorder(const void* grad, const float* rois, void* grad_input, int N, int C, int H, int W, int K,
                                            int ph, int pw, float spatial_scale, int sampling_ratio, int aligned, int dtype, void* temp,
                                            size_t* temp_bytes, void* stream);

int cddmsl_anchors(const float* cell, float* out, int Hf, int Wf, int A, float stride, float offset, void* stream);
int cddmsl_sort_desc(const float* keys_in, float* keys_out, int* idx_scratch, int* order_out, const int* offsets, int N,
                     int total, void* temp, size_t* temp_bytes, void* stream);
int cddmsl_rpn_decode(const int* order, const float* deltas, const float* cell, const int* img_hw, float* boxes,
                      unsigned char* valid, int N, int Hf, int Wf, int A, int topk, float stride, float offset, float wx,
                      float wy, float ww, float wh, float scale_clamp, float min_size, void* stream);
int cddmsl_nms(const float* boxes, const unsigned char* valid, unsigned long long* mask_ws, int* keep, int* nkeep, int N,
               int n, float thr, int max_keep, void* stream);
int cddmsl_nms_anyorder(const float* boxes, const float* scores, long* keep, int* nkeep, int K, float iou_threshold, void* temp,
                        size_t* temp_bytes, void* stream);
int cddmsl_soft_nms(const float* boxes, const float* scores, const long* idxs, long* keep, float* keep_scores, int* nkeep, int K,
                    int method, float sigma, float iou_threshold, float prune_threshold, int max_keep, void* temp,
                    size_t* temp_bytes, void* stream);
int cddmsl_openset_logits(const float* x, const float* wn, float* logits, float* stats, int R, int D, int K, int ld,
                          float temperature, float eps, void* stream);
int cddmsl_openset_select(const float* logits, const float* stats, int ld, const float* boxes, int ldb, const float* objectness,
                          int R, int K, float img_h, float img_w, float score_thresh, int* cand_row, int* cand_cls,
                          float* cand_score, float* cand_box, unsigned char* valid, int* count, int cap, void* temp,
                          size_t* temp_bytes, void* stream);
int cddmsl_iou_match(const float* gt, int G, const float* preds, int P, long* matches, signed char* labels,
                     unsigned int* best_ws, int nthr, float t0, float t1, int l0, int l1, int l2, int allow_low_quality,
                     void* stream);

int cddmsl_iou_match_batched(const float* gt, const int* gt_off, const float* preds, const int* pred_off, long* matches,
                             signed char* labels, unsigned int* best_ws, int N, int P, int maxG, int totalG, int nthr, float t0,
                             float t1, int l0, int l1, int l2, int allow_low_quality, void* stream);

int cddmsl_attn_tokens_fwd(const void* x, const float* pos, void* tok, int K, int P, int TP, int C, int dtype, void* stream);
int cddmsl_attn_tokens_fwd_mask(const void* x, const float* pos, void* tok, unsigned long long* mbits, int K, int P, int TP, int C,
                                int dtype, void* stream);
int cddmsl_attnpool_dx(const void* pds, const void* zu, const float* g0, const unsigned long long* mbits, void* dx, float* gpos, int K,
                       int H2, int P, int TP, int C, int dtype, void* stream);
int cddmsl_attn_tokens_bwd(const void* dtok, const void* relu_mask, void* dx, float* gpos, int K, int P, int TP, int C, int dtype,
                           void* stream);
int cddmsl_attnpool_softmax_fwd(const float* S, float* p, void* pT, long K, int H, int P1, int TP, float scale, int dtype, void* stream);
int cddmsl_attnpool_softmax_bwd(const float* p, const float* dP, void* dsT, void* pds, long K, int H, int P1, int TP, float scale,
                                int dtype, void* stream);

int cddmsl_attn_small_fwd(const void* q, const void* k, const void* v, void* o, int nseq, int t, int heads, int dh, int ldq,
                          int ldk, int ldv, int ldo, float scale, int dtype, void* stream);
int cddmsl_attn_small_bwd(const void* q, const void* k, const void* v, const void* dout, void* dq, void* dk, void* dv, int nseq,
                          int t, int heads, int dh, int ldq, int ldk, int ldv, int ldo, float scale, int dtype, void* stream);
int cddmsl_attn_last_fwd(const void* q, const void* kv, void* o, float* p, int n, int t, int heads, int dh, int ldq, int ldkv, int voff,
                         int ldo, float scale, int dtype, void* stream);
int cddmsl_attn_last_bwd(const void* q, const void* kv, const void* dout, const float* p, void* dq, void* dkv, int n, int t, int heads,
                         int dh, int ldq, int ldkv, int voff, int ldo, float scale, int dtype, void* stream);

int cddmsl_text_embed(const long* ids, const void* tok, const float* pos, float* x, long rows, int t, int W, int vocab, int dtype,
                      void* stream);
int cddmsl_attn_causal_fwd(const void* qkv, void* o, int nseq, int t, int heads, int dh, int ldqkv, int ldo, float scale, int dtype,
                           void* stream);
int cddmsl_quick_gelu(void* x, long numel, int dtype, void* stream);
int cddmsl_text_pool(const float* x, const long* rows, const float* gamma, const float* beta, void* y, long R, int nout, int group,
                     int W, float eps, int dtype, void* stream);

int cddmsl_skinny_gemm_workspace(int M, int N, int K);
int cddmsl_skinny_gemm(const void* x, const void* w, const float* bias, const float* residual, void* y, float* ws, long ws_bytes, int M,
                       int N, int K, int epi, void* stream);
int cddmsl_lm_head_workspace(int M, int V);
int cddmsl_lm_head_argmax(const void* h, const void* wte, long* ids, int ld_ids, float* logits, void* ws, long ws_bytes, int M, int V,
                          int K, void* stream);
int cddmsl_decode_attn(const void* qkv, void* kc, void* vc, void* o, int nseq, int heads, int dh, int L, int Lmax, int ldqkv, float scale,
                       int dtype, void* stream);
int cddmsl_pos_embed(const long* ids, int ld_ids, const void* tab, const float* src, const float* wpe, float* x, long rows, int t, int pos0,
                     int W, int vocab, int npos, int dtype, void* stream);
int cddmsl_gelu_new(void* x, long numel, int dtype, void* stream);
int cddmsl_lm_head_topk_workspace(int M, int V);
int cddmsl_lm_head_topk(const void* h, const void* wte, float* vals, int* idx, float* logZ, float* logits, void* ws, long ws_bytes, int M,
                        int V, int K, int B, void* stream);
int cddmsl_beam_step(const float* vals, const int* idx, const float* logZ, const float* sum_in, const int* len_in,
                     const unsigned char* stop_in, const int* hist_in, const unsigned char* anc_in, float* sum_out, int* len_out,
                     unsigned char* stop_out, int* hist_out, unsigned char* anc_out, int* src, long* next_tok, int n, int B, int T, int step,
                     int stop_id, void* stream);
int cddmsl_decode_attn_beam(const void* qkv, const void* pk, const void* pv, void* gk, void* gv, const unsigned char* anc, void* o, int rows,
                            int B, int heads, int dh, int P, int L, int Tg, int ldanc, int ldqkv, float scale, int dtype, void* stream);

int cddmsl_l2norm_fwd(const float* x, float* y, float* inv, long R, int D, float eps, void* stream);
int cddmsl_l2norm_bwd(const float* dy, const float* y, const float* inv, float* dx, long R, int D, void* stream);
int cddmsl_cosine_logits_fwd(const float* x, const float* wn, float* scores, float* inv, long R, int D, int Kc,
                             float temperature, float eps, void* stream);
int cddmsl_cosine_logits_bwd(const float* ds, const float* x, const float* wn, const float* inv, float* dx, long R, int D,
                             int Kc, float temperature, int accumulate, void* stream);
int cddmsl_layernorm_fwd(const float* x, const float* gamma, const float* beta, void* y, float* mean, float* rstd, long R, int D,
                         float eps, int dtype, void* stream);
int cddmsl_layernorm_bwd(const void* dy, const float* x, const float* gamma, const float* mean, const float* rstd, float* dx,
                         long R, int D, int accumulate, int dtype, void* stream);
int cddmsl_layernorm_bwd_emit(const void* dy, const float* x, const float* gamma, const float* mean, const float* rstd, float* dx,
                              void* dx_bf16, long R, int D, int accumulate, int dtype, int* emitted, void* stream);
int cddmsl_focal_ce_fwd(const float* logits, const long* target, float* row_loss, float* probs, long R, int C, float gamma,
                        int bg_class, float bg_weight, void* stream);
int cddmsl_focal_ce_bwd(const float* logits, const long* target, const float* probs, const float* gscale, float* dlogits, long R,
                        int C, float gamma, int bg_class, float bg_weight, void* stream);
int cddmsl_contrastive_fwd(const float* S, float* rlse, float* clse, float* loss, int n, int ld, void* stream);
int cddmsl_contrastive_bwd(const float* S, const float* rlse, const float* clse, const float* gloss, float* dS, int n, int ld,
                           void* stream);
int cddmsl_rpn_losses(const float* logits, const float* deltas, const long* pos, int npos, const long* neg, int nneg, const long* midx,
                      const float* gt, const long* gt_off, const float* anchors, long A, float wx, float wy, float ww, float wh, float inv_norm,
                      float* out2, const float* gout2, float* dlogits, float* ddeltas, void* stream);
int cddmsl_box_l1(const float* deltas, int ld, const long* fg, int nfg, const long* cls, const float* src, const float* tgt, float wx, float wy,
                  float ww, float wh, float inv_norm, float* out1, const float* gout1, float* ddeltas, void* stream);
int cddmsl_rpn_losses_reg(const float* logits, const float* deltas, const long* pos, int npos, const long* neg, int nneg, const long* midx,
                          const float* gt, const long* gt_off, const float* anchors, long A, float wx, float wy, float ww, float wh, float inv_norm,
                          int loc_type, float beta, float scale_clamp, float* out2, const float* gout2, float* dlogits, float* ddeltas, void* stream);
int cddmsl_box_reg_loss(const float* deltas, int ld, const long* fg, int nfg, const long* cls, const float* src, const float* tgt, float wx, float wy,
                        float ww, float wh, float inv_norm, int loc_type, float beta, float scale_clamp, float* out1, const float* gout1, float* ddeltas,
                        void* stream);

int cddmsl_preprocess(const unsigned char* img, void* out, int n, int h, int w, int Hp, int Wp, int Cp, const float* mean3,
                      const float* std3, int div255, int dtype, void* stream);
int cddmsl_preprocess224(const unsigned char* img, void* out, int n, int h, int w, int Hp, int Wp, int RH, int RW, int top,
                         int left, int S, int Cp, const float* mean3, const float* std3, int dtype, void* stream);
int cddmsl_preprocess_batch(const unsigned char* const* imgs, const int* hs, const int* ws, int N, void* out, int Hp, int Wp, int Cp,
                            const float* mean3, const float* std3, int div255, int dtype, void* stream);
int cddmsl_preprocess224_batch(const unsigned char* const* imgs, const int* hs, const int* ws, int N, void* out, int Hp, int Wp, int RH,
                               int RW, int top, int left, int S, int Cp, const float* mean3, const float* std3, int dtype, void* stream);
int cddmsl_tta_view(const unsigned char* img, int h, int w, int newh, int neww, const int* xlo, const int* xn, const int* xk, int xks,
                    const int* ylo, const int* yn, const int* yk, int yks, void* out0, int n0, int Hp0, int Wp0, void* out1, int n1,
                    int Hp1, int Wp1, int Cp, const float* mean3, const float* std3, int div255, int dtype, void* stream);
typedef struct cddmsl_resize_item {
  long src_off, dst_off;
  int h, w, newh, neww, flip, reverse_channels, xtab, xks, ytab, yks;
} cddmsl_resize_item;
int cddmsl_resize_batch_u8(const unsigned char* src, long src_bytes, unsigned char* dst, long dst_bytes, const int* tab, long tab_len,
                           const cddmsl_resize_item* items, int count, void* stream);
int cddmsl_avgpool2_fwd(const void* x, void* y, int N, int H, int W, int C, int dtype, void* stream);
int cddmsl_avgpool2_bwd(const void* dy, const void* mask, const void* add, void* dx, int N, int H, int W, int C, int dtype,
                        void* stream);
int cddmsl_avgpool2_fwd_bits(const void* x, void* y, void* bits, int N, int H, int W, int C, int dtype, void* stream);
int cddmsl_avgpool2_bwd_bits(const void* dy, const void* bits, void* dx, int N, int H, int W, int C, int dtype, void* stream);
int cddmsl_avgpool2_bwd_q8(const void* dy, const void* mask, const void* add, void* dx, int N, int H, int W, int C, void* y8,
                           const float* q8, float* amax8, void* stream);
int cddmsl_maxpool3s2_fwd(const void* x, void* y, int N, int H, int W, int C, int dtype, void* stream);
int cddmsl_upsample_zero2(const void* t, const void* mask, const void* add, void* dx, int N, int H, int W, int C, int dtype,
                          void* stream);
int cddmsl_meanpool_fwd(const void* x, float* y, long K, int P, int C, int dtype, void* stream);
int cddmsl_meanpool_bwd(const float* dy, void* dx, long K, int P, int C, int dtype, void* stream);
int cddmsl_relu_bwd(const void* g, const void* y, void* dx, long numel, int g_f32, int dtype, void* stream);
int cddmsl_colsum(const void* x, float* out, long rows, int cols, int period, int dtype, void* stream);
int cddmsl_sgd_clip_step(float** params, const float** grads, float** moms, const long* sizes, int count, float* norm_ws,
                         float lr, float momentum, float wd, float clip, int first_step, void* stream);

int cddmsl_instance_boxes(const void* maps, int B, int H, int W, int dtype, int* records, int max_records, int* counts, void* ws,
                          size_t* ws_bytes, void* stream);

#ifdef __cplusplus
}
#endif
#endif
```

Baseline: 173.3.

## Fuse 2x2 avgpool with mask bits into conv3x3 epilogue and unpool into conv3 dgrad

Adds two new epilogue modes to the 256-tile conv kernel. In the first, the 3x3 conv reorders its output rows so each 2x2 pool window lands in one thread, then writes the pooled result and relu-mask bits directly. In the second, the 1x1 dgrad applies the pool backward (scatter ×0.25 gated by the bits) in its epilogue. This removes the full-resolution o2 and dp2 round trips through memory and two separate pooling kernels in stride-2 bottlenecks. The cost is extra epilogue work, a row-remapped im2col index, and fallback paths when tail-split planning or shapes don't fit.

Result: faster. 175.2 (median of 6 runs) (+1.1%).

```diff
diff --git a/cddmsl_amd/csrc/conv_fwd256.hip b/cddmsl_amd/csrc/conv_fwd256.hip
--- a/cddmsl_amd/csrc/conv_fwd256.hip
+++ b/cddmsl_amd/csrc/conv_fwd256.hip
@@ -56,20 +56,28 @@
     if (sb) { sc[j] = sb[j >> 2][j & 3]; bi[j] = sb[2 + (j >> 2)][j & 3]; }
     else { sc[j] = p.scale ? p.scale[n + j] : 1.f; bi[j] = p.bias ? p.bias[n + j] : 0.f; }
   }
-  const bool has_res = EPI < 0 ? p.residual != nullptr : (EPI & 1) != 0;
-  const bool has_msk = EPI < 0 ? p.relu_mask != nullptr : (EPI & 2) != 0;
+  constexpr bool POOLO = EPI == 4, POOLB = EPI == 5;
+  constexpr int EOPS = EPI >= 4 ? 0 : EPI;
+  const bool has_res = EPI < 0 ? p.residual != nullptr : (EOPS & 1) != 0;
+  const bool has_msk = EPI < 0 ? p.relu_mask != nullptr : (EOPS & 2) != 0;
   const bool f32out = EPI < 0 && (ES == 4 || p.out_f32 != 0);
   const int eso = f32out ? 4 : 2;
   const float relu_floor = p.relu ? 0.f : -__builtin_inff();
-  const long rows = p.M - m0;
+  const long rows = POOLO ? (p.M - m0) >> 2 : p.M - m0;
+  const int mb = POOLO ? m0 >> 2 : m0;
   auto mk = [&](const char* base, long ld, int es) {
     long bytes = rows * ld * es;
     if (bytes > 0x7fffffffL) bytes = 0x7fffffffL;
-    return __builtin_amdgcn_make_buffer_rsrc((void*)(base + (long)m0 * ld * es), 0, base ? (int)bytes : 0, 0x00020000);
+    return __builtin_amdgcn_make_buffer_rsrc((void*)(base + (long)mb * ld * es), 0, base ? (int)bytes : 0, 0x00020000);
   };
   const bool rf32 = EPI < 0 && ES == 2 && p.res_f32;
   const int esr = rf32 ? 4 : ES;
-  const __amdgpu_buffer_rsrc_t ry = mk(p.y, p.ldy, eso), rmsk = mk(p.relu_mask, p.ldm, ES);
+  const unsigned tq0 = POOLB ? fdiv((unsigned)m0, p.dWo) : 0u;
+  long ybytes = (4L * p.M - 4L * tq0 * p.Wo) * p.ldy * 2;
+  if (ybytes > 0x7fffffffL) ybytes = 0x7fffffffL;
+  const __amdgpu_buffer_rsrc_t ry = POOLB ? __builtin_amdgcn_make_buffer_rsrc((void*)(p.y + 4L * tq0 * p.Wo * p.ldy * 2), 0, (int)ybytes, 0x00020000)
+                                          : mk(p.y, p.ldy, eso);
+  const __amdgpu_buffer_rsrc_t rmsk = mk(p.relu_mask, p.ldm, ES);
   const __amdgpu_buffer_rsrc_t rres = RPOOL ? __builtin_amdgcn_make_buffer_rsrc((void*)p.residual, 0, 0x7fffffff, 0x00020000)
                                             : mk(p.residual, p.ldr, esr);
   auto pooled_off = [&](int m) -> unsigned {
@@ -79,7 +87,16 @@
     const bool in = m < p.M && (oy >> 1) < hp && (ox >> 1) < wp;
     return in ? (unsigned)((((img * hp + (oy >> 1)) * wp + (ox >> 1)) * (unsigned)p.ldr + (unsigned)n) * ES) : 0x80000000u;
   };
-  const unsigned vy = (unsigned)(((wr * 128 + rr) * p.ldy + n) * eso);
+  const unsigned vy = (unsigned)(((wr * (POOLO ? 32 : 128) + rr) * p.ldy + n) * eso);
+  const __amdgpu_buffer_rsrc_t rbits = mk(POOLO || POOLB ? (const char*)p.pool_bits : nullptr, p.Cout >> 3, 4);
+  const unsigned vbits = (unsigned)(((wr * (POOLB ? 128 : 32) + rr) * (p.Cout >> 3) + (n >> 3)) * 4);
+  unsigned bw[4][4];
+  if constexpr (POOLB) {
+#pragma unroll
+    for (int a = 0; a < 4; ++a)
+#pragma unroll
+      for (int i = 0; i < 4; ++i) bw[a][i] = __builtin_amdgcn_raw_buffer_load_b32(rbits, vbits, (a * 32 + 8 * i) * (p.Cout >> 3) * 4, 0);
+  }
   const unsigned vr = (unsigned)(((wr * 128 + rr) * p.ldr + n) * esr), vm = (unsigned)(((wr * 128 + rr) * p.ldm + n) * ES);
   const bool emit8 = EPI < 0 && ES == 2 && p.y8 != nullptr;
   const __amdgpu_buffer_rsrc_t ry8 = mk(p.y8, p.ldy, 1);
@@ -133,6 +150,7 @@
     u32x4 (*rmsk_)[ES / 2] = rmskb[a % DEPTH];
     asm volatile("s_waitcnt lgkmcnt(0)" ::: "memory");
     f32x4 val[4][2];
+    u32x4 ob[4];
 #pragma unroll
     for (int i = 0; i < 4; ++i) {
       const int row = rr + 8 * i;
@@ -190,6 +208,33 @@
         }
 #pragma unroll
         for (int j = 0; j < 8; ++j) if (!(mv[j] > 0.f)) v[j] = 0.f;
+      }
+      if constexpr (POOLO) {
+        ob[i] = u32x4{pack2bf(v[0], v[1]), pack2bf(v[2], v[3]), pack2bf(v[4], v[5]), pack2bf(v[6], v[7])};
+        continue;
+      }
+      if constexpr (POOLB) {
+        const unsigned m = (unsigned)(m0 + wr * 128 + a * 32 + 8 * i + rr);
+        const unsigned tq = fdiv(m, p.dWo), pox = m - tq * p.Wo;
+        const unsigned vo = m < (unsigned)p.M ? (unsigned)(((4 * p.Wo * (tq - tq0) + 2 * pox) * p.ldy + n) * 2) : 0x80000000u;
+        const u32x4 g = {pack2bf(v[0], v[1]), pack2bf(v[2], v[3]), pack2bf(v[4], v[5]), pack2bf(v[6], v[7])};
+        const unsigned word = bw[a][i];
+#pragma unroll
+        for (int e = 0; e < 4; ++e) {
+          u32x4 o;
+#pragma unroll
+          for (int j = 0; j < 4; ++j) {
+            const float lo = (word >> (8 * e + 2 * j)) & 1u ? bf2f(g[j] & 0xffff) * 0.25f : 0.f;
+            const float hi = (word >> (8 * e + 2 * j + 1)) & 1u ? bf2f(g[j] >> 16) * 0.25f : 0.f;
+            o[j] = pack2bf(lo, hi);
+          }
+          const unsigned so = (unsigned)((((e >> 1) * 2 * p.Wo + (e & 1)) * p.ldy) * 2);
+          if (p.nt_out) __builtin_amdgcn_raw_buffer_store_b128(o, ry, vo, so, CDDMSL_STORE_AUX);
+          else __builtin_amdgcn_raw_buffer_store_b128(o, ry, vo, so, 0);
+          asm volatile("s_nop 4" ::: "memory");
+          asm volatile("" :: "v"(o));
+        }
+        continue;
       }
       const unsigned so = (unsigned)((a * 32 + 8 * i) * p.ldy * eso);
       if (emit8) {
@@ -214,6 +259,26 @@
         asm volatile("s_nop 4" ::: "memory");
         asm volatile("" :: "v"(o));
       }
+    }
+    if constexpr (POOLO) {
+      u32x4 o;
+      unsigned mw = 0u;
+#pragma unroll
+      for (int j = 0; j < 4; ++j) {
+        float lo[4], hi[4];
+#pragma unroll
+        for (int e = 0; e < 4; ++e) {
+          lo[e] = bf2f(ob[e][j] & 0xffff); hi[e] = bf2f(ob[e][j] >> 16);
+          mw |= (lo[e] > 0.f ? 1u : 0u) << (8 * e + 2 * j) | (hi[e] > 0.f ? 1u : 0u) << (8 * e + 2 * j + 1);
+        }
+        o[j] = pack2bf(((lo[0] + lo[1]) + (lo[2] + lo[3])) * 0.25f, ((hi[0] + hi[1]) + (hi[2] + hi[3])) * 0.25f);
+      }
+      if (p.nt_out) __builtin_amdgcn_raw_buffer_store_b128(o, ry, vy, (unsigned)(a * 8 * p.ldy * 2), CDDMSL_STORE_AUX);
+      else __builtin_amdgcn_raw_buffer_store_b128(o, ry, vy, (unsigned)(a * 8 * p.ldy * 2), 0);
+      asm volatile("s_nop 4" ::: "memory");
+      __builtin_amdgcn_raw_buffer_store_b32(mw, rbits, vbits, (unsigned)(a * 8 * (p.Cout >> 3) * 4), 0);
+      asm volatile("s_nop 4" ::: "memory");
+      asm volatile("" :: "v"(o), "v"(mw));
     }
     if (DEPTH == 2 && a + 2 < 4 && !rf32) fetch(a + 2, rresb[a % DEPTH], rmskb[a % DEPTH]);
   };
@@ -254,9 +319,20 @@
   const int nkt = SPLITK ? min(p.kper, (p.Kc >> 3) - kt0) : (p.Kc >> 3);
   const int tpt = p.cpp >> 3;
 
+  constexpr bool POOLO = EPI == 4;
+  auto pooled_px = [&](int m) { const int R = m - m0; return (m0 >> 2) + (R >> 5) * 8 + (R & 7); };
   auto rowoff = [&](int m, int& iy0, int& ix0) {
-    const unsigned tq = fdiv((unsigned)m, p.dWo), ox = m - tq * p.Wo;
-    const unsigned img = fdiv(tq, p.dHo), oy = tq - img * p.Ho;
+    unsigned img, oy, ox;
+    if (POOLO) {
+      const unsigned pp = (unsigned)pooled_px(m), e = ((unsigned)(m - m0) >> 3) & 3u, wp = (unsigned)p.Wo >> 1, hp = (unsigned)p.Ho >> 1;
+      const unsigned tq = fdiv(pp, p.dWp), pox = pp - tq * wp;
+      img = fdiv(tq, p.dHp);
+      oy = 2 * (tq - img * hp) + (e >> 1); ox = 2 * pox + (e & 1);
+    } else {
+      const unsigned tq = fdiv((unsigned)m, p.dWo);
+      ox = m - tq * p.Wo;
+      img = fdiv(tq, p.dHo); oy = tq - img * p.Ho;
+    }
     iy0 = (int)oy * p.stride - p.pad; ix0 = (int)ox * p.stride - p.pad;
     return (((long)img * p.Hi + iy0) * p.Wi + ix0) * p.xrs * 16;
   };
@@ -271,7 +347,7 @@
 #pragma unroll
     for (int i = 0; i < 2; ++i) {
       const int m = m0 + i * 128 + h * 64 + (t >> 3);
-      const bool vm = m < p.M;
+      const bool vm = POOLO ? pooled_px(m) < (p.M >> 2) : m < p.M;
       const long ro = rowoff(vm ? m : m0, iy0[h][i], ix0[h][i]);
       va[h][i] = (unsigned)(ro - base_a) + cl * 16;
       if (!vm) { iy0[h][i] = -(1 << 20); if (!TAPS) va[h][i] |= 0x80000000u; }
@@ -401,7 +477,7 @@
   const unsigned long long ts_loop = __builtin_amdgcn_s_memrealtime();
 #endif
 
-  constexpr bool PREF = EPI > 0 && !RPOOL && Mma<T>::ES == 2 && !SPLITK;
+  constexpr bool PREF = EPI > 0 && EPI < 4 && !RPOOL && Mma<T>::ES == 2 && !SPLITK;
   u32x4 pre[2][4];
   f32x4 sb[4];
   auto ktile = [&](int kt, auto LAST) {
@@ -754,11 +830,22 @@
     else launch_fwd2<T, false>(a, grid, st);
   } else {
     if (a.res_pool) hipLaunchKernelGGL((k_conv_fwd256<T, false, true>), grid, dim3(512), 0, st, a);
+    else if (a.pool_bits) {
+      if constexpr (std::is_same<T, __bf16>::value) {
+        if (a.pool_bwd) hipLaunchKernelGGL((k_conv_fwd256<T, false, false, 5>), grid, dim3(512), 0, st, a);
+        else hipLaunchKernelGGL((k_conv_fwd256<T, true, false, 4>), grid, dim3(512), 0, st, a);
+      }
+    }
     else if (taps) launch256<T, true>(a, grid, st, ws, ws_bytes);
     else launch256<T, false>(a, grid, st, ws, ws_bytes);
   }
 }
 
+}
+
+bool fwd256_tail_split_planned(long tiles, int nktot, void* ws, long ws_bytes) {
+  if (tiles > 0x7fffffffL) return false;
+  return plan_tail_split((int)tiles, persistent_blocks_raw(), nktot, ws ? ws_bytes : 0).splits != 0;
 }
 
 void launch_fwd_tile256(const ConvArgs& a, const Plan& p, Operand op, hipStream_t st, void* ws, long ws_bytes) {
diff --git a/cddmsl_amd/csrc/gemm_common.h b/cddmsl_amd/csrc/gemm_common.h
--- a/cddmsl_amd/csrc/gemm_common.h
+++ b/cddmsl_amd/csrc/gemm_common.h
@@ -55,6 +55,8 @@
   int tile0 = 0, ksplits = 1, kper = 0, tile_limit = 0;
   int pool_out = 0;
   FastDiv dWp = {}, dHp = {};
+  unsigned* pool_bits = nullptr;
+  int pool_bwd = 0;
   int nt_out = 1;
 #ifdef CDDMSL_TILE_STAMPS
   unsigned long long* tstamps = nullptr;
@@ -188,5 +190,6 @@
 __attribute__((visibility("hidden"))) void launch_wgrad(WgradArgs& a, const Plan& p, Operand op, hipStream_t st, void* ws, long ws_bytes);
 __attribute__((visibility("hidden"))) void launch_gemm_tn(const WgradArgs& p, Operand op, const Plan& pl, int batch, int mode, hipStream_t st);
 __attribute__((visibility("hidden"))) void launch_attnpool_dx(const WgradArgs& p, unsigned gx, unsigned gy, int nbatch, int bpb, hipStream_t st);
+__attribute__((visibility("hidden"))) bool fwd256_tail_split_planned(long tiles, int nktot, void* ws, long ws_bytes);
 __attribute__((visibility("hidden"))) bool record_kernel(int id);
 }
diff --git a/cddmsl_amd/csrc/gemm_conv.hip b/cddmsl_amd/csrc/gemm_conv.hip
--- a/cddmsl_amd/csrc/gemm_conv.hip
+++ b/cddmsl_amd/csrc/gemm_conv.hip
@@ -208,6 +208,40 @@
   return run_fwd(a, OP_BF16, pl, stream);
 }
 
+extern "C" int cddmsl_conv_pool2_fwd(const void* x, const void* w, void* p2, void* bits, const float* scale, const float* bias,
+                                     const void* residual, const void* relu_mask, int Nimg, int Hi, int Wi, int Cin, int Cout, int relu,
+                                     int dtype, void* stream) {
+  if (dtype != 0 || residual || relu_mask || !p2 || !bits || Hi < 2 || Wi < 2) return CDDMSL_ERR_ARG;
+  ConvArgs a;
+  const int st = fill_conv(a, OP_BF16, x, w, p2, scale, bias, nullptr, nullptr, Nimg, Hi, Wi, Cin, Cout, 3, 3, 1, 1, 0, Cout, 0, 0, relu, 0,
+                           nullptr, nullptr, nullptr);
+  if (st != CDDMSL_OK || a.M == 0) return st;
+  if (plan_fwd(a, OP_BF16, 1).kernel != 3) return CDDMSL_ERR_ARG;
+  if (fwd256_tail_split_planned((long)(Cout / 256) * ((a.M + 255) / 256), a.Kc >> 3, g_ws, g_ws_bytes)) return CDDMSL_ERR_ARG;
+  const long np = (long)Nimg * (Hi / 2) * (Wi / 2);
+  a.M = (int)(4 * np);
+  a.pool_bits = (unsigned*)bits;
+  a.dWp = make_fastdiv((unsigned)(Wi / 2)); a.dHp = make_fastdiv((unsigned)(Hi / 2));
+  a.nt_out = nt_out_for(np * Cout * 2);
+  const Plan pl = {3, (unsigned)((long)(Cout / 256) * ((a.M + 255) / 256)), 1};
+  return run_fwd(a, OP_BF16, pl, stream);
+}
+
+extern "C" int cddmsl_conv_unpool2_fwd(const void* x, const void* w, void* dx, const void* bits, const void* residual, const void* relu_mask,
+                                       int Nimg, int H, int W, int Cin, int Cout, int dtype, void* stream) {
+  if (dtype != 0 || residual || relu_mask || !dx || !bits || H < 2 || W < 2 || (H & 1) || (W & 1)) return CDDMSL_ERR_ARG;
+  ConvArgs a;
+  const int st = fill_conv(a, OP_BF16, x, w, dx, nullptr, nullptr, nullptr, nullptr, Nimg, H / 2, W / 2, Cin, Cout, 1, 1, 1, 0, 0, Cout, 0, 0, 0, 0,
+                           nullptr, nullptr, nullptr);
+  if (st != CDDMSL_OK || a.M == 0) return st;
+  const Plan pl = plan_fwd(a, OP_BF16, 1);
+  if (pl.kernel != 3) return CDDMSL_ERR_ARG;
+  if (fwd256_tail_split_planned((long)pl.gx, a.Kc >> 3, g_ws, g_ws_bytes)) return CDDMSL_ERR_ARG;
+  a.pool_bits = (unsigned*)bits; a.pool_bwd = 1;
+  a.nt_out = nt_out_for(4L * a.M * Cout * 2);
+  return run_fwd(a, OP_BF16, pl, stream);
+}
+
 extern "C" int cddmsl_conv_fwd_q8(const void* x, const void* w, void* y, const float* scale, const float* bias,
                                   const void* residual, const void* relu_mask, int Nimg, int Hi, int Wi, int Cin,
                                   int Cout, int KH, int KW, int stride, int pad, int relu, void* y8, const float* q8, float* amax8,
diff --git a/cddmsl_amd/hip.py b/cddmsl_amd/hip.py
--- a/cddmsl_amd/hip.py
+++ b/cddmsl_amd/hip.py
@@ -42,6 +42,8 @@
         L.cddmsl_avgpool2_fwd_bits.argtypes = [vp] * 3 + [ci] * 5 + [vp]
         L.cddmsl_avgpool2_bwd_bits.argtypes = [vp] * 3 + [ci] * 5 + [vp]
         L.cddmsl_conv3x3_pool_fwd.argtypes = [vp] * 6 + [ci] * 7 + [vp]
+        L.cddmsl_conv_pool2_fwd.argtypes = [vp] * 8 + [ci] * 7 + [vp]
+        L.cddmsl_conv_unpool2_fwd.argtypes = [vp] * 6 + [ci] * 6 + [vp]
         L.cddmsl_attn_tokens_fwd.argtypes = [vp] * 3 + [ci] * 5 + [vp]
         L.cddmsl_attn_tokens_bwd.argtypes = [vp] * 4 + [ci] * 5 + [vp]
         L.cddmsl_attnpool_softmax_fwd.argtypes = [vp] * 3 + [c_long, ci, ci, ci, cf, ci, vp]
@@ -294,6 +296,77 @@
     return y
 
 
+def _conv_pool2_call(x, w, p2, bits, scale, bias, relu):
+    N, H, W, Cin = x.shape
+    return _L().cddmsl_conv_pool2_fwd(ptr(x), ptr(w), ptr(p2), ptr(bits), ptr(scale), ptr(bias), c_void_p(0), c_void_p(0), N, H, W, Cin,
+                                      w.shape[0], int(relu), _dt(x), stream_ptr())
+
+
+def conv_pool2_ok(x, w):
+    if not (x.is_cuda and x.dtype == torch.bfloat16 and w.dtype == x.dtype and x.dim() == 4 and w.dim() == 4 and x.is_contiguous()
+            and w.is_contiguous() and tuple(w.shape[1:]) == (3, 3, x.shape[3]) and x.shape[1] >= 2 and x.shape[2] >= 2 and x.shape[0] > 0):
+        return False
+    L = _L()
+    was = L.cddmsl_plan_only(1)
+    try:
+        return _conv_pool2_call(x, w, x, x, None, None, True) == 0
+    finally:
+        L.cddmsl_plan_only(was)
+
+
+def conv_pool2_fwd(x, w, scale=None, bias=None, relu=True):
+    require_cuda(x, w, scale, bias)
+    ensure_workspace(x.device)
+    assert x.dim() == 4 and w.dim() == 4 and x.is_contiguous() and w.is_contiguous() and x.dtype == w.dtype
+    N, H, W, Cin = x.shape
+    Cout, KH, KW, Cin2 = w.shape
+    assert (KH, KW, Cin2) == (3, 3, Cin) and Cout % 8 == 0, (x.shape, w.shape)
+    for v in (scale, bias):
+        assert v is None or (v.dtype == torch.float32 and v.numel() == Cout and v.is_contiguous())
+    p2 = torch.empty((N, H // 2, W // 2, Cout), device=x.device, dtype=x.dtype)
+    bits = torch.empty((N, H // 2, W // 2, Cout // 8), device=x.device, dtype=torch.int32)
+    e0 = PROFILE.begin(name="k_conv_fwd256") if PROFILE.on else None
+    check(_conv_pool2_call(x, w, p2, bits, scale, bias, relu), "cddmsl_conv_pool2_fwd")
+    PROFILE.end(e0, "k_conv_fwd256", 2.0 * N * H * W * Cout * 9 * Cin, (N * H * W, Cout, 9 * Cin, 3, 2, 1),
+                nbytes=float(x.numel() * 2 + w.numel() * 2 + p2.numel() * 2 + bits.numel() * 4))
+    return p2, bits
+
+
+def _conv_unpool2_call(g, w, dx, bits, H, W):
+    return _L().cddmsl_conv_unpool2_fwd(ptr(g), ptr(w), ptr(dx), ptr(bits), c_void_p(0), c_void_p(0), g.shape[0], H, W, g.shape[3], w.shape[0],
+                                        _dt(g), stream_ptr())
+
+
+def conv_unpool2_ok(g, w, out_shape):
+    N, H, W, C = out_shape
+    if not (g.is_cuda and g.dtype == torch.bfloat16 and w.dtype == g.dtype and g.dim() == 4 and w.dim() == 4 and g.is_contiguous()
+            and w.is_contiguous() and tuple(w.shape) == (C, 1, 1, g.shape[3]) and tuple(g.shape[:3]) == (N, H // 2, W // 2) and N > 0
+            and H >= 2 and W >= 2 and H % 2 == 0 and W % 2 == 0):
+        return False
+    L = _L()
+    was = L.cddmsl_plan_only(1)
+    try:
+        return _conv_unpool2_call(g, w, g, g, H, W) == 0
+    finally:
+        L.cddmsl_plan_only(was)
+
+
+def conv_unpool2_fwd(g, w, bits, out_shape):
+    require_cuda(g, w, bits)
+    ensure_workspace(g.device)
+    N, H, W, C = out_shape
+    assert g.dim() == 4 and g.is_contiguous() and w.is_contiguous() and g.dtype == w.dtype and tuple(w.shape) == (C, 1, 1, g.shape[3])
+    assert tuple(g.shape[:3]) == (N, H // 2, W // 2) and H % 2 == 0 and W % 2 == 0 and C % 8 == 0, (g.shape, out_shape)
+    assert bits.dtype == torch.int32 and bits.is_contiguous() and tuple(bits.shape) == (N, H // 2, W // 2, C // 8), bits.shape
+    dx = torch.empty((N, H, W, C), device=g.device, dtype=g.dtype)
+    e0 = PROFILE.begin(name="k_conv_fwd256") if PROFILE.on else None
+    check(_conv_unpool2_call(g, w, dx, bits, H, W), "cddmsl_conv_unpool2_fwd")
+    M = N * (H // 2) * (W // 2)
+    PROFILE.end(e0, "k_conv_fwd256", 2.0 * M * C * g.shape[3], (M, C, g.shape[3], 1, 3, 1),
+                nbytes=float(g.numel() * 2 + w.numel() * 2 + dx.numel() * 2 + bits.numel() * 4))
+    return dx
+
+
 def bottleneck64_ok(o1, w2, w3, wd=None, w1n=None):
     if not (o1.is_cuda and o1.dtype == torch.bfloat16 and o1.dim() == 4 and o1.is_contiguous() and o1.shape[3] == 64):
         return False
diff --git a/cddmsl_amd/layers.py b/cddmsl_amd/layers.py
--- a/cddmsl_amd/layers.py
+++ b/cddmsl_amd/layers.py
@@ -482,6 +482,23 @@
     return not (bp.fp8 and _fp8_dgrad_wanted(bp.pw[1], o2.shape, 1, True))
 
 
+def _conv2_pool_fused(o1, bp, save):
+    if not save or bp.fp8 or os.environ.get("CDDMSL_CONV_POOL", "1") == "0" or o1.dtype != torch.bfloat16:
+        return False
+    if os.environ.get("CDDMSL_POOL_MASK_BITS", "1") == "0":
+        return False
+    return hip.conv_pool2_ok(o1, bp.pw[1].get(o1.dtype, need_dgrad=False)[0])
+
+
+def _conv3_dgrad_unpooled(gs, bp, bits, o2_shape):
+    if bp.fp8 or bits.dtype != torch.int32 or gs.dtype != torch.bfloat16 or os.environ.get("CDDMSL_CONV_UNPOOL", "1") == "0":
+        return None
+    wd = bp.pw[2].get(gs.dtype, True)[1]
+    if not hip.conv_unpool2_ok(gs, wd, o2_shape):
+        return None
+    return hip.conv_unpool2_fwd(gs, wd, bits, o2_shape)
+
+
 def _block_forward(x, bp, save, px_given=None, next_pw=None, out_spec=None):
     (s1, b1), (s2, b2), (s3, b3), bnd = bp.bn
     pool = bp.stride > 1
@@ -491,13 +508,18 @@
     x8 = _fp8_made_for(x, bp.pw[0]) if f8 and save else None
     M2 = x.shape[0] * x.shape[1] * x.shape[2]
     e8o2 = fp8_act_slot(bp.pw[2]).emit() if save and not pool and _fp8_wgrad1x1_wanted(bp.pw[2], M2, f8) else None
-    o2 = conv_fwd_auto(o1, bp.pw[1], s2, b2, f8, emit8=e8o2, relu=True, pad=1)
-    o2_8 = _fp8_made_for(o2, bp.pw[2]) if e8o2 is not None else None
-    o2_shape, bits = tuple(o2.shape), None
-    if pool and save and _pool_bits_wanted(bp, o2):
-        p2, bits = hip.avgpool2_fwd_bits(o2)
+    if pool and _conv2_pool_fused(o1, bp, save):
+        w2 = bp.pw[1].get(o1.dtype, need_dgrad=False)[0]
+        p2, bits = hip.conv_pool2_fwd(o1, w2, s2, b2, relu=True)
+        o2, o2_8, o2_shape = None, None, (o1.shape[0], o1.shape[1], o1.shape[2], w2.shape[0])
     else:
-        p2 = hip.avgpool2_fwd(o2) if pool else o2
+        o2 = conv_fwd_auto(o1, bp.pw[1], s2, b2, f8, emit8=e8o2, relu=True, pad=1)
+        o2_8 = _fp8_made_for(o2, bp.pw[2]) if e8o2 is not None else None
+        o2_shape, bits = tuple(o2.shape), None
+        if pool and save and _pool_bits_wanted(bp, o2):
+            p2, bits = hip.avgpool2_fwd_bits(o2)
+        else:
+            p2 = hip.avgpool2_fwd(o2) if pool else o2
     if pool and px_given is not None and tuple(px_given.shape) == (x.shape[0], x.shape[1] // 2, x.shape[2] // 2, x.shape[3]):
         px = px_given
     else:
@@ -531,11 +553,13 @@
         hip.conv_wgrad(p2 if pool else o2, gs, shp(w3p), s3, out=_ohwi(_grad_buf(w3p)))
     d1_slot = fp8_slot_of(bp.pw[0], "_fp8_g") if f8 and x8 is not None and _fp8_wgrad1x1_wanted(bp.pw[0], M2, f8) else None
     if pool:
-        dp2 = dgrad_auto(gs, bp.pw[2], f8, gs_slot)
-        if o2_bits:
-            dpre2 = hip.avgpool2_bwd_bits(dp2, o2_shape, o2)
-        else:
-            dpre2 = hip.avgpool2_bwd(dp2, o2_shape, mask=o2, emit8=d2_slot.emit() if f8 and _fp8_dgrad_wanted(bp.pw[1], o2_shape, 1, f8) else None)
+        dpre2 = _conv3_dgrad_unpooled(gs, bp, o2, o2_shape) if o2_bits else None
+        if dpre2 is None:
+            dp2 = dgrad_auto(gs, bp.pw[2], f8, gs_slot)
+            if o2_bits:
+                dpre2 = hip.avgpool2_bwd_bits(dp2, o2_shape, o2)
+            else:
+                dpre2 = hip.avgpool2_bwd(dp2, o2_shape, mask=o2, emit8=d2_slot.emit() if f8 and _fp8_dgrad_wanted(bp.pw[1], o2_shape, 1, f8) else None)
     else:
         e8 = d2_slot.emit() if f8 and _fp8_dgrad_wanted(bp.pw[1], o2_shape, 1, f8) else None
         dpre2 = dgrad_auto(gs, bp.pw[2], f8, gs_slot, emit8=e8, relu_mask=o2)
@@ -703,12 +727,17 @@
         o1[K:].copy_(hip.conv_fwd(extra, w1, s1, b1, relu=True))
         if idn is None:
             px[K:].copy_(hip.avgpool2_fwd(extra))
-    o2 = conv_fwd_auto(o1, bp.pw[1], s2, b2, f8, relu=True, pad=1)
-    o2_shape = tuple(o2.shape)
-    if save and _pool_bits_wanted(bp, o2):
-        p2, o2 = hip.avgpool2_fwd_bits(o2)
+    if _conv2_pool_fused(o1, bp, save):
+        w2 = bp.pw[1].get(T, False)[0]
+        o2_shape = (o1.shape[0], o1.shape[1], o1.shape[2], w2.shape[0])
+        p2, o2 = hip.conv_pool2_fwd(o1, w2, s2, b2, relu=True)
     else:
-        p2 = hip.avgpool2_fwd(o2)
+        o2 = conv_fwd_auto(o1, bp.pw[1], s2, b2, f8, relu=True, pad=1)
+        o2_shape = tuple(o2.shape)
+        if save and _pool_bits_wanted(bp, o2):
+            p2, o2 = hip.avgpool2_fwd_bits(o2)
+        else:
+            p2 = hip.avgpool2_fwd(o2)
     if idn is None:
         idn = conv_fwd_auto(px, bp.pw[3], bnd[0], bnd[1], f8)
     out_shape = (p2.shape[0], p2.shape[1], p2.shape[2], _ohwi(bp.w[2]).shape[0])
@@ -760,7 +789,9 @@
         d2_slot = fp8_slot_of(bp.pw[1], "_fp8_g") if f8 else None
         hip.conv_wgrad(p2, gs, shp(w3p), s3, out=_ohwi(_grad_buf(w3p)))
         if o2.dtype == torch.int32:
-            dpre2 = hip.avgpool2_bwd_bits(dgrad_auto(gs, bp.pw[2], f8, gs_slot), o2_shape, o2)
+            dpre2 = _conv3_dgrad_unpooled(gs, bp, o2, o2_shape)
+            if dpre2 is None:
+                dpre2 = hip.avgpool2_bwd_bits(dgrad_auto(gs, bp.pw[2], f8, gs_slot), o2_shape, o2)
         else:
             e8 = d2_slot.emit() if f8 and _fp8_dgrad_wanted(bp.pw[1], o2_shape, 1, f8) else None
             dpre2 = hip.avgpool2_bwd(dgrad_auto(gs, bp.pw[2], f8, gs_slot), o2_shape, mask=o2, emit8=e8)
diff --git a/include/cddmsl_hip.h b/include/cddmsl_hip.h
--- a/include/cddmsl_hip.h
+++ b/include/cddmsl_hip.h
@@ -13,6 +13,11 @@
                     int pool, int ldy, int ldr, int ldm, int relu, int out_f32, int dtype, void* stream);
 int cddmsl_conv3x3_pool_fwd(const void* x, const void* w, void* y, const float* scale, const float* bias, const void* relu_mask,
                             int Nimg, int Hi, int Wi, int Cin, int Cout, int stride, int dtype, void* stream);
+int cddmsl_conv_pool2_fwd(const void* x, const void* w, void* p2, void* bits, const float* scale, const float* bias,
+                          const void* residual, const void* relu_mask, int Nimg, int Hi, int Wi, int Cin, int Cout, int relu,
+                          int dtype, void* stream);
+int cddmsl_conv_unpool2_fwd(const void* x, const void* w, void* dx, const void* bits, const void* residual, const void* relu_mask,
+                            int Nimg, int H, int W, int Cin, int Cout, int dtype, void* stream);
 int cddmsl_bottleneck64_ok(int Nimg, int H, int W, int dtype);
 int cddmsl_bottleneck64_fwd(const void* o1, const void* w2, const float* s2, const float* b2, const void* w3, const float* s3,
                             const float* b3, const void* residual, const void* x0, const void* wd, const float* sd,
```
